# MCG-NKU/E2FGVI

Hardware: AMD Instinct MI355X
Metric: inpainted frames/sec at 432x240 T=10 (higher is better)
Workload: dtype f32; 1 GPU; BASELINE.json configs[1]: e2fgvi 432x240 T=10 l_t=10, 1 clip(s) per GPU per forward (1 in the job), random-init weights, torch.rand frames + box mask (SURVEY.md 8d); clips_per_gpu=1, precision=fp32, kernel_selection=e2fgvi_amd/tile_table.py (checked in, deterministic: ops.py), hip_graph=True, forwards_in_flight=2

## Files before the change

### e2fgvi_amd/build.py

```python
import os
import subprocess
import sys
from concurrent.futures import ThreadPoolExecutor

HERE = os.path.dirname(os.path.abspath(__file__))
CSRC = os.path.join(HERE, "csrc")
LIB = os.path.join(CSRC, "libe2fgvi_hip.so")
FLAGS = ["--offload-arch=gfx950", "-O3", "-std=c++17", "-fPIC", "-ffp-contract=fast"]
NOPK = ["-Xclang", "-target-feature", "-Xclang", "-packed-fp32-ops"]
UNITS = [("error.hip", "error.o", []), ("conv.hip", "conv.o", []), ("conv.hip", "conv_nopk.o", NOPK + ["-DE2_NOPK_VARIANT"]),
         ("conv_bf16x.hip", "conv_bf16x.o", NOPK), ("conv_wino.hip", "conv_wino.o", NOPK), ("conv_wino.hip", "conv_wino_x3.o", NOPK + ["-DE2_WINO_X3=1"]), ("conv_wino4.hip", "conv_wino4.o", NOPK), ("conv_tail.hip", "conv_tail.o", NOPK),
         ("mdcn.hip", "mdcn.o", NOPK), ("attention.hip", "attention.o", []),
         ("attention_bf16.hip", "attention_bf16.o", NOPK), ("attention_x3.hip", "attention_x3.o", NOPK), ("misc.hip", "misc.o", NOPK),
         ("video.hip", "video.o", NOPK), ("metrics.hip", "metrics.o", NOPK)]
NOPK_OBJECTS = ("conv_nopk.o", "conv_bf16x.o", "conv_wino.o", "conv_wino4.o", "conv_wino_x3.o", "conv_tail.o", "mdcn.o", "attention_bf16.o", "attention_x3.o", "misc.o", "video.o", "metrics.o")
OBJDUMP = "/opt/rocm/lib/llvm/bin/llvm-objdump"


def _hipcc():
    for c in (os.environ.get("HIPCC"), "/opt/rocm/bin/hipcc"):
        if c and os.path.exists(c):
            return c
    return "hipcc"


def _stale(out, deps):
    return (not os.path.exists(out)) or any(os.path.getmtime(d) > os.path.getmtime(out) for d in deps)


def build(force=False, verbose=False, nopk_all=False, lib=None, tag=None, defines=()):
    hipcc = _hipcc()
    if tag:
        nopk_all = False
    objdir = os.path.join(CSRC, ("build_" + tag) if tag else ("build_nopk" if nopk_all else "build"))
    os.makedirs(objdir, exist_ok=True)
    out = lib or (os.path.join(CSRC, "libe2fgvi_hip_%s.so" % tag) if tag else
                  os.path.join(CSRC, "libe2fgvi_hip_nopk.so") if nopk_all else LIB)
    headers = [os.path.join(CSRC, "common.h"), os.path.join(HERE, "..", "include", "e2fgvi_hip.h"), os.path.abspath(__file__)]
    jobs = []
    for src, obj, extra in UNITS:
        sp, op = os.path.join(CSRC, src), os.path.join(objdir, obj)
        if nopk_all and not any(f == "-packed-fp32-ops" for f in extra):
            extra = extra + NOPK
        if force or _stale(op, [sp] + headers):
            jobs.append([hipcc] + FLAGS + extra + list(defines) + ["-c", sp, "-o", op])

    def run(cmd):
        if verbose:
            print(" ".join(cmd), flush=True)
        subprocess.check_call(cmd)

    with ThreadPoolExecutor(max_workers=min(4, max(1, len(jobs)))) as ex:
        list(ex.map(run, jobs))
    objs = [os.path.join(objdir, obj) for _, obj, _ in UNITS]
    if force or jobs or _stale(out, objs):
        run([hipcc, "--offload-arch=gfx950", "-shared", "-fPIC", "-o", out] + objs)
    if jobs:
        verify_isa(objdir)
        if not nopk_all:
            verify_wino_waits(objdir)
            verify_exit_reuse(objdir)
            verify_no_scratch(objdir)
    return out


def build_variant(tag, *defines):
    return build(tag=tag, defines=defines)


def device_isa(obj):
    import shutil
    import tempfile
    d = tempfile.mkdtemp(prefix="e2isa")
    try:
        local = os.path.join(d, os.path.basename(obj))
        shutil.copy(obj, local)
        subprocess.run([OBJDUMP, "--offloading", os.path.basename(obj)], cwd=d, check=True, stdout=subprocess.DEVNULL,
                       stderr=subprocess.DEVNULL)
        dev = [f for f in os.listdir(d) if "gfx950" in f]
        if not dev:
            return ""
        return subprocess.run([OBJDUMP, "-d", os.path.join(d, dev[0])], check=True, capture_output=True, text=True).stdout
    finally:
        shutil.rmtree(d, ignore_errors=True)


def verify_isa(objdir=None):
    import re
    objdir = objdir or os.path.join(CSRC, "build")
    if not os.path.exists(OBJDUMP):
        return
    for obj in NOPK_OBJECTS:
        isa = device_isa(os.path.join(objdir, obj))
        bad = re.findall(r"v_pk_(?:mul|add|fma)_f32", isa)
        if bad or not isa:
            raise RuntimeError("%s: %s" % (obj, "%d packed-fp32 instructions in a unit that must have none" % len(bad) if isa
                                           else "no gfx950 code object found"))


def verify_no_scratch(objdir=None, obj="conv_bf16x.o", marker="ELb0ELi2ELb1EEE"):
    import re
    import shutil
    import tempfile
    objdir = objdir or os.path.join(CSRC, "build")
    readelf = os.path.join(os.path.dirname(OBJDUMP), "llvm-readelf")
    if not (os.path.exists(OBJDUMP) and os.path.exists(readelf)):
        return 0
    d = tempfile.mkdtemp(prefix="e2elf")
    try:
        shutil.copy(os.path.join(objdir, obj), os.path.join(d, obj))
        subprocess.run([OBJDUMP, "--offloading", obj], cwd=d, check=True, stdout=subprocess.DEVNULL, stderr=subprocess.DEVNULL)
        dev = [f for f in os.listdir(d) if "gfx950" in f]
        notes = subprocess.run([readelf, "--notes", os.path.join(d, dev[0])], check=True, capture_output=True, text=True).stdout if dev else ""
    finally:
        shutil.rmtree(d, ignore_errors=True)
    found = 0
    for block in notes.split("  - .agpr_count")[1:]:
        name = re.search(r"\.name:\s+(\S+)", block)
        if not name or marker not in name.group(1):
            continue
        found += 1
        priv = int(re.search(r"\.private_segment_fixed_size:\s+(\d+)", block).group(1))
        spill = int(re.search(r"\.vgpr_spill_count:\s+(\d+)", block).group(1))
        if priv or spill:
            raise RuntimeError("%s: %s: private segment %d bytes, %d spilled VGPRs in a ping-pong kernel" % (obj, name.group(1)[:70], priv, spill))
    if not found:
        raise RuntimeError("verify_no_scratch: no ping-pong instantiation found in %s (mangled-name marker changed?)" % obj)
    return found


def _kernels(isa):
    import re
    out, cur = {}, None
    for line in isa.splitlines():
        m = re.match(r"^[0-9a-f]+ <([^>]+)>:", line)
        if m:
            cur = out.setdefault(m.group(1), [])
            continue
        m = re.match(r"^\s+(\S+)\s*(.*?)\s*//\s*([0-9A-Fa-f]+):", line)
        if m and cur is not None:
            cur.append((int(m.group(3), 16), m.group(1), m.group(2)))
    return out


def check_kernel_waits(obj, name, ins):
# ... 223 lines not shown
```

### e2fgvi_amd/csrc/conv_bf16x.hip

```cpp
#include "common.h"

namespace {

typedef __bf16 bf16x8 __attribute__((ext_vector_type(8)));
typedef unsigned int u32x4 __attribute__((ext_vector_type(4)));
typedef __attribute__((address_space(3))) void lds_void;

struct ConvXParams {
    const void* src[E2FGVI_MAX_SRC];
    int ld[E2FGVI_MAX_SRC];
    int coff[E2FGVI_MAX_SRC];
    int cpg[E2FGVI_MAX_SRC];
    unsigned src_bytes[E2FGVI_MAX_SRC];
    int nsrc;
    int N, H, W, Ho, Wo, KH, KW, stride, pad;
    int padx;
    int osy, osx, opy, opx, oH, oW;
    int res_bcast;
    int Cout, Cout_g, Npad;
    int M;
    int tilesM, tilesN;
    int nsteps;
    unsigned wgroup_bytes;
    long long wgroup_elems;
    const void* w;
    const float* bias;
    const void* res;
    int res_ld, res_coff, res_bf16;
    void* dst;
    int dst_ld, dst_coff, dst_bf16, dst_nchw;
    __bf16* dst2;
    int dst2_ld, dst2_coff;
    int split_from;
    long long split_plane;
    int act;
    float slope;
    int tp_cq;
    unsigned tp_magic;
    unsigned tp_magic_cq;
    int dbg_noload;
};

__device__ __forceinline__ __amdgpu_buffer_rsrc_t make_rsrc(const void* base, unsigned bytes) {
    return __builtin_amdgcn_make_buffer_rsrc(const_cast<void*>(base), 0, (int)bytes, 0x00020000);
}

__device__ __forceinline__ float dcn_post(float v, int co, int C, const f32x4& fl, float max_residue) {
    const int noff = (C / 3) * 2;
    if (co >= noff) return e2_fast_sigmoid(v);
    const int which = (co * 2 >= noff) ? 2 : 0;
    return max_residue * e2_fast_tanh(v) + fl[which + ((co & 1) ? 0 : 1)];
}


__device__ __forceinline__ void split8(const f32x4& v0, const f32x4& v1, bf16x8& hi, bf16x8& mid, bf16x8& lo) {
    e2_split8(v0, v1, hi, mid, lo);
}

typedef int pp_i32x4 __attribute__((ext_vector_type(4)));
__device__ __forceinline__ pp_i32x4 pp_rsrc_words(const void* base, unsigned bytes) {
    const unsigned long long b = (unsigned long long)base;
    pp_i32x4 r;
    r[0] = __builtin_amdgcn_readfirstlane((int)(unsigned)b);
    r[1] = __builtin_amdgcn_readfirstlane((int)((unsigned)(b >> 32) & 0xFFFFu));
    r[2] = __builtin_amdgcn_readfirstlane((int)bytes);
    r[3] = 0x00020000;
    return r;
}
__device__ __forceinline__ void pp_dma16(pp_i32x4 rsrc, unsigned lds_dst, unsigned voff, unsigned soff) {
    unsigned keep;
    asm volatile("s_nop 4\n\ts_mov_b32 %0, m0\n\ts_mov_b32 m0, %3\n\ts_nop 0\n\tbuffer_load_dwordx4 %1, %2, %4 offen lds\n\ts_mov_b32 m0, %0"
                 : "=&s"(keep) : "v"(voff), "s"(rsrc), "s"(lds_dst), "s"(soff) : "memory");
}

template <int BM, int BN, int WGM, int WGN, bool S3, int MODE, bool PP = false>
__global__ __launch_bounds__(64 * WGM * WGN) void conv_bf16x_kernel(const ConvXParams p) {
#if defined(__HIP_DEVICE_COMPILE__)
    constexpr bool F32 = MODE == 1, X3 = MODE == 2, F16 = MODE == 3;
    typedef typename e2_h16<F16>::T E16;
    typedef typename e2_h16<F16>::V8 e16x8;
    static_assert(!PP || (X3 && !S3 && WGM * WGN == 8), "ping-pong halves: split-operand mode, 8 waves, no row-shift stages");
    constexpr int NT = 64 * WGM * WGN;
    constexpr int ESZ = (F32 || X3) ? 4 : 2;
    constexpr int CH = 16 / ESZ;
    constexpr int KC = 8 * CH;
    constexpr int TM = BM / (32 * WGM), TN = BN / (32 * WGN);
    constexpr int AR = S3 ? BM + 2 : BM;
    constexpr int B_CH = X3 ? 12 : 8;
    constexpr int A_BYTES = AR * 128, B_BYTES = BN * B_CH * 16;
    constexpr int A_IT = (AR * 8 + NT - 1) / NT, B_IT = (BN * B_CH + NT - 1) / NT;
    constexpr bool A_PART = (AR * 8) % NT != 0;
    constexpr bool B_PART = (BN * B_CH) % NT != 0;
    constexpr int R = TM * 32, CN = TN * 32;
    constexpr int ES = (WGM * WGN * R * (CN + 4) * 4 <= 150 * 1024) ? 1 : (TN % 2 == 0 ? 2 : TN);
    constexpr int TNH = TN / ES, CNH = CN / ES, LDE = CNH + 4;
    constexpr int EPI = WGM * WGN * R * LDE * 4;
    static_assert(TN % ES == 0 && EPI <= 160 * 1024, "epilogue region");
    constexpr int SMEM = 2 * (A_BYTES + B_BYTES) > EPI ? 2 * (A_BYTES + B_BYTES) : EPI;
    constexpr unsigned OOB = 0xFFFFFFFFu;
    static_assert(TM >= 1 && TN >= 1 && (BM * 8) % NT == 0 && (BN * B_CH) % 64 == 0 && SMEM <= 160 * 1024, "tile");

    __shared__ __attribute__((aligned(1024))) unsigned char smem[SMEM];

    const int tid = threadIdx.x;
    const int lane = tid & 63, wave = __builtin_amdgcn_readfirstlane(tid >> 6);
    const int wm = wave / WGN, wn = wave % WGN;
    const int g = blockIdx.y;
    const int logical = xcd_remap(blockIdx.x, p.tilesM * p.tilesN);
    const int tile_m = logical / p.tilesN, tile_n = logical - tile_m * p.tilesN;
    const int m0 = tile_m * BM, n0 = tile_n * BN;
    const int HoWo = p.Ho * p.Wo;

    int a_pix[A_IT];
    unsigned a_msk[A_IT];
    unsigned a_ch16[A_IT];
#pragma unroll
    for (int it = 0; it < A_IT; ++it) {
        const int item = tid + it * NT;
        const int row = item >> 3, slot = item & 7;
        a_ch16[it] = (unsigned)((slot ^ ((row >> 1) & 7)) * 16);
        const int m = S3 ? m0 + row - 1 : m0 + row;
        const bool ok = m >= 0 && m < p.M;
        const int mm = ok ? m : 0;
        const int img = mm / HoWo;
        const int rem = mm - img * HoWo;
        const int oy = rem / p.Wo, ox = rem - oy * p.Wo;
        const int by = oy * p.stride - p.pad;
        const int bx = S3 ? ox : ox * p.stride - p.padx;
        unsigned msk = 0;
        for (int k = 0; k < p.KH; ++k) msk |= ((unsigned)(by + k) < (unsigned)p.H ? 1u : 0u) << k;
        for (int k = 0; k < (S3 ? 1 : p.KW); ++k) msk |= ((unsigned)(bx + k) < (unsigned)p.W ? 1u : 0u) << (8 + k);
        a_msk[it] = ok ? msk : 0u;
        a_pix[it] = (img * p.H + by) * p.W + bx;
    }
    unsigned b_off[B_IT];
#pragma unroll
    for (int it = 0; it < B_IT; ++it) {
        const int item = tid + it * NT;
        const int koct = item / BN, n = item - koct * BN;
        b_off[it] = ((n0 + n) < p.Npad && koct < B_CH) ? (unsigned)((koct * p.Npad + n0 + n) * 16) : OOB;
    }
    const __amdgpu_buffer_rsrc_t wrsrc = make_rsrc(reinterpret_cast<const char*>(p.w) + (long long)g * p.wgroup_bytes, p.wgroup_bytes);
    const unsigned b_step = (unsigned)B_CH * (unsigned)p.Npad * 16u;

    const void* const sp0 = p.src[0]; const void* const sp1 = p.src[1]; const void* const sp2 = p.src[2]; const void* const sp3 = p.src[3];
    const unsigned sb0 = p.src_bytes[0], sb1 = p.src_bytes[1], sb2 = p.src_bytes[2], sb3 = p.src_bytes[3];
    const unsigned sl0 = (unsigned)p.ld[0] * ESZ, sl1 = (unsigned)p.ld[1] * ESZ, sl2 = (unsigned)p.ld[2] * ESZ, sl3 = (unsigned)p.ld[3] * ESZ;
    const unsigned sc0 = (unsigned)(p.coff[0] + g * p.cpg[0]) * ESZ, sc1 = (unsigned)(p.coff[1] + g * p.cpg[1]) * ESZ,
                   sc2 = (unsigned)(p.coff[2] + g * p.cpg[2]) * ESZ, sc3 = (unsigned)(p.coff[3] + g * p.cpg[3]) * ESZ;
    const int sg0 = p.cpg[0], sg1 = p.cpg[1], sg2 = p.cpg[2], sg3 = p.cpg[3];
    int ky = 0, kx = 0, s = 0, c0 = 0;
    int blk = 0;
    const void* cur_src = sp0;
    unsigned cur_bytes = sb0;
    unsigned cur_ld2 = sl0, cur_chan = sc0;
    int cur_cpg = sg0;
    unsigned a_off[A_IT];
    auto retarget = [&]() {
        if (p.nsrc > 1) {
            cur_src = s == 0 ? sp0 : s == 1 ? sp1 : s == 2 ? sp2 : sp3;
            cur_bytes = s == 0 ? sb0 : s == 1 ? sb1 : s == 2 ? sb2 : sb3;
            cur_ld2 = s == 0 ? sl0 : s == 1 ? sl1 : s == 2 ? sl2 : sl3;
            cur_chan = s == 0 ? sc0 : s == 1 ? sc1 : s == 2 ? sc2 : sc3;
            cur_cpg = s == 0 ? sg0 : s == 1 ? sg1 : s == 2 ? sg2 : sg3;
        }
        const int kxe = S3 ? 0 : kx;
        const int tap = ky * p.W + kxe;
#pragma unroll
        for (int it = 0; it < A_IT; ++it) {
            const bool ok = ((a_msk[it] >> ky) & (a_msk[it] >> (8 + kxe)) & 1u) != 0;
            a_off[it] = ok ? (unsigned)(a_pix[it] + tap) * cur_ld2 + cur_chan + a_ch16[it] : OOB;
        }
    };
    retarget();
    unsigned char* const smem_b = smem + 2 * A_BYTES;
    auto issue_a = [&](int stage) {
        if (p.dbg_noload & 16) return;
        unsigned char* sa = smem + stage * A_BYTES + wave * 1024;
        const __amdgpu_buffer_rsrc_t arsrc = make_rsrc(cur_src, cur_bytes);
        const unsigned soff = (unsigned)c0 * (unsigned)ESZ;
        if (c0 + KC <= cur_cpg) {
#pragma unroll
            for (int it = 0; it < A_IT; ++it)
                if (!A_PART || it + 1 < A_IT || tid + it * NT < AR * 8)
                    __builtin_amdgcn_raw_ptr_buffer_load_lds(arsrc, (lds_void*)(sa + it * NT * 16), 16, a_off[it], soff, 0, 0);
        } else {
#pragma unroll
            for (int it = 0; it < A_IT; ++it)
                if (!A_PART || it + 1 < A_IT || tid + it * NT < AR * 8)
                    __builtin_amdgcn_raw_ptr_buffer_load_lds(arsrc, (lds_void*)(sa + it * NT * 16), 16,
                                                             (c0 + (int)(a_ch16[it] / ESZ) < cur_cpg) ? a_off[it] : OOB, soff, 0, 0);
        }
    };
    auto issue_b = [&](int stage, int step) {
        if (p.dbg_noload & 32) return;
        unsigned char* sb = smem_b + stage * B_BYTES + wave * 1024;
        const unsigned soff = (unsigned)step * b_step;
#pragma unroll
        for (int it = 0; it < B_IT; ++it)
            if (!B_PART || it + 1 < B_IT || tid + it * NT < BN * B_CH)
                __builtin_amdgcn_raw_ptr_buffer_load_lds(wrsrc, (lds_void*)(sb + it * NT * 16), 16, b_off[it], soff, 0, 0);
    };
    auto advance = [&]() -> bool {
        c0 += KC;
        ++blk;
        if (c0 < cur_cpg) return false;
        c0 = 0;
        ++s;
        if (s == p.nsrc) {
            s = 0;
            blk = 0;
            if (S3) ++ky;
            else { ++kx; if (kx == p.KW) { kx = 0; ++ky; } }
        }
        return true;
    };

    f32x16 acc[TM][TN];
#pragma unroll
    for (int tm = 0; tm < TM; ++tm)
#pragma unroll
        for (int tn = 0; tn < TN; ++tn)
#pragma unroll
            for (int r = 0; r < 16; ++r) acc[tm][tn][r] = 0.f;

    const int i = lane & 31, h = lane >> 5;
    int a_row[TM], b_rd[TN];
    bool okl[TM], okr[TM];
#pragma unroll
    for (int tm = 0; tm < TM; ++tm) {
        a_row[tm] = (wm * TM + tm) * 32 + i;
        const int ox = (m0 + a_row[tm]) % p.Wo;
        okl[tm] = ox != 0;
        okr[tm] = ox != p.Wo - 1;
    }
#pragma unroll
    for (int tn = 0; tn < TN; ++tn) b_rd[tn] = ((wn * TN + tn) * 32 + i) * 16;

    auto compute = [&](const unsigned char* st, const unsigned char* stb, int kxs) {
        int a_rd[TM], a_key[TM];
        bool zero[TM];
#pragma unroll
        for (int tm = 0; tm < TM; ++tm) {
            const int row = a_row[tm] + (S3 ? kxs : 0);
            a_rd[tm] = row * 128;
            a_key[tm] = (row >> 1) & 7;
            zero[tm] = S3 && ((kxs == 0 && !okl[tm]) || (kxs == 2 && !okr[tm]));
        }
        if constexpr (X3) {
#pragma unroll
            for (int kk = 0; kk < 2; ++kk) {
                const int q = 2 * kk + h;
                bf16x8 ah[TM], am[TM], al[TM];
#pragma unroll
                for (int tm = 0; tm < TM; ++tm)
                    split8(*reinterpret_cast<const f32x4*>(st + a_rd[tm] + (((2 * q) ^ a_key[tm]) << 4)),
                           *reinterpret_cast<const f32x4*>(st + a_rd[tm] + (((2 * q + 1) ^ a_key[tm]) << 4)), ah[tm], am[tm], al[tm]);
#pragma unroll
                for (int tn = 0; tn < TN; ++tn) {
                    const bf16x8 bh = *reinterpret_cast<const bf16x8*>(stb + b_rd[tn] + q * (BN * 16));
                    const bf16x8 bm = *reinterpret_cast<const bf16x8*>(stb + b_rd[tn] + (4 + q) * (BN * 16));
                    const bf16x8 bl = *reinterpret_cast<const bf16x8*>(stb + b_rd[tn] + (8 + q) * (BN * 16));
#pragma unroll
                    for (int tm = 0; tm < TM; ++tm) acc[tm][tn] = __builtin_amdgcn_mfma_f32_32x32x16_bf16(al[tm], bh, acc[tm][tn], 0, 0, 0);
#pragma unroll
                    for (int tm = 0; tm < TM; ++tm) acc[tm][tn] = __builtin_amdgcn_mfma_f32_32x32x16_bf16(ah[tm], bl, acc[tm][tn], 0, 0, 0);
#pragma unroll
                    for (int tm = 0; tm < TM; ++tm) acc[tm][tn] = __builtin_amdgcn_mfma_f32_32x32x16_bf16(am[tm], bm, acc[tm][tn], 0, 0, 0);
#pragma unroll
                    for (int tm = 0; tm < TM; ++tm) acc[tm][tn] = __builtin_amdgcn_mfma_f32_32x32x16_bf16(am[tm], bh, acc[tm][tn], 0, 0, 0);
#pragma unroll
                    for (int tm = 0; tm < TM; ++tm) acc[tm][tn] = __builtin_amdgcn_mfma_f32_32x32x16_bf16(ah[tm], bm, acc[tm][tn], 0, 0, 0);
#pragma unroll
                    for (int tm = 0; tm < TM; ++tm) acc[tm][tn] = __builtin_amdgcn_mfma_f32_32x32x16_bf16(ah[tm], bh, acc[tm][tn], 0, 0, 0);
                }
            }
        } else {
#pragma unroll
        for (int kk = 0; kk < 4; ++kk) {
            if constexpr (F32) {
                f32x4 a[TM], b[TN];
#pragma unroll
                for (int tm = 0; tm < TM; ++tm)
                    a[tm] = *reinterpret_cast<const f32x4*>(st + a_rd[tm] + (((2 * kk + h) ^ a_key[tm]) << 4));
#pragma unroll
                for (int tn = 0; tn < TN; ++tn)
                    b[tn] = *reinterpret_cast<const f32x4*>(stb + b_rd[tn] + (2 * kk + h) * (BN * 16));
#pragma unroll
                for (int e = 0; e < 4; ++e)
#pragma unroll
                    for (int tm = 0; tm < TM; ++tm)
#pragma unroll
                        for (int tn = 0; tn < TN; ++tn)
                            acc[tm][tn] = __builtin_amdgcn_mfma_f32_32x32x2f32(a[tm][e], b[tn][e], acc[tm][tn], 0, 0, 0);
            } else {
                e16x8 a[TM], b[TN];
#pragma unroll
                for (int tm = 0; tm < TM; ++tm) {
                    a[tm] = *reinterpret_cast<const e16x8*>(st + a_rd[tm] + (((2 * kk + h) ^ a_key[tm]) << 4));
                    if (S3) {
                        u32x4 q = __builtin_bit_cast(u32x4, a[tm]);
#pragma unroll
                        for (int e = 0; e < 4; ++e) q[e] = zero[tm] ? 0u : q[e];
                        a[tm] = __builtin_bit_cast(e16x8, q);
                    }
                }
#pragma unroll
                for (int tn = 0; tn < TN; ++tn)
                    b[tn] = *reinterpret_cast<const e16x8*>(stb + b_rd[tn] + (2 * kk + h) * (BN * 16));
#pragma unroll
                for (int tm = 0; tm < TM; ++tm)
#pragma unroll
                    for (int tn = 0; tn < TN; ++tn)
                        acc[tm][tn] = e2_mfma16(a[tm], b[tn], acc[tm][tn]);
            }
        }
        }
    };
    const bool tap_packed = !S3 && p.tp_cq != 0;
    if (!tap_packed) issue_a(0);
    issue_b(0, 0);
    if (!tap_packed) {
        asm volatile("s_waitcnt vmcnt(0)" ::: "memory");
        __syncthreads();
    }
    if constexpr (PP) {
        const bool trail = wave >= 4;
        bf16x8 fa[TM][3];
        auto pp_bar = [&]() __attribute__((always_inline)) {
            __builtin_amdgcn_sched_barrier(0);
            asm volatile("s_waitcnt lgkmcnt(0)\n\ts_barrier" ::: "memory");
            __builtin_amdgcn_sched_barrier(0);
        };
        auto prep = [&](const unsigned char* st, const int kk) __attribute__((always_inline)) {
            const int q = 2 * kk + h;
#pragma unroll
            for (int tm = 0; tm < TM; ++tm) {
                const int row = a_row[tm];
                const int rd = row * 128, key = (row >> 1) & 7;
                split8(*reinterpret_cast<const f32x4*>(st + rd + (((2 * q) ^ key) << 4)),
                       *reinterpret_cast<const f32x4*>(st + rd + (((2 * q + 1) ^ key) << 4)), fa[tm][0], fa[tm][1], fa[tm][2]);
            }
        };
        auto mma = [&](const unsigned char* stb, const int kk) __attribute__((always_inline)) {
            const int q = 2 * kk + h;
            bf16x8 bq[2][3];
            auto rd = [&](int tn, bf16x8 (&b)[3]) __attribute__((always_inline)) {
                b[0] = *reinterpret_cast<const bf16x8*>(stb + b_rd[tn] + q * (BN * 16));
                b[1] = *reinterpret_cast<const bf16x8*>(stb + b_rd[tn] + (4 + q) * (BN * 16));
                b[2] = *reinterpret_cast<const bf16x8*>(stb + b_rd[tn] + (8 + q) * (BN * 16));
            };
            rd(0, bq[0]);
#pragma unroll
            for (int tn = 0; tn < TN; ++tn) {
                if (tn + 1 < TN) rd(tn + 1, bq[(tn + 1) & 1]);
                __builtin_amdgcn_sched_barrier(0);
                const bf16x8 bh = bq[tn & 1][0], bm = bq[tn & 1][1], bl = bq[tn & 1][2];
#pragma unroll
                for (int tm = 0; tm < TM; ++tm) acc[tm][tn] = __builtin_amdgcn_mfma_f32_32x32x16_bf16(fa[tm][2], bh, acc[tm][tn], 0, 0, 0);
#pragma unroll
                for (int tm = 0; tm < TM; ++tm) acc[tm][tn] = __builtin_amdgcn_mfma_f32_32x32x16_bf16(fa[tm][0], bl, acc[tm][tn], 0, 0, 0);
#pragma unroll
                for (int tm = 0; tm < TM; ++tm) acc[tm][tn] = __builtin_amdgcn_mfma_f32_32x32x16_bf16(fa[tm][1], bm, acc[tm][tn], 0, 0, 0);
#pragma unroll
                for (int tm = 0; tm < TM; ++tm) acc[tm][tn] = __builtin_amdgcn_mfma_f32_32x32x16_bf16(fa[tm][1], bh, acc[tm][tn], 0, 0, 0);
#pragma unroll
                for (int tm = 0; tm < TM; ++tm) acc[tm][tn] = __builtin_amdgcn_mfma_f32_32x32x16_bf16(fa[tm][0], bm, acc[tm][tn], 0, 0, 0);
#pragma unroll
                for (int tm = 0; tm < TM; ++tm) acc[tm][tn] = __builtin_amdgcn_mfma_f32_32x32x16_bf16(fa[tm][0], bh, acc[tm][tn], 0, 0, 0);
                __builtin_amdgcn_sched_barrier(0);
            }
        };
        const unsigned smem_lds = (unsigned)(unsigned long long)(lds_void*)smem;
        const pp_i32x4 wrsrc_w = pp_rsrc_words(reinterpret_cast<const char*>(p.w) + (long long)g * p.wgroup_bytes, p.wgroup_bytes);
        auto pp_issue = [&](int stage, int step) __attribute__((always_inline)) {
            const pp_i32x4 arsrc_w = pp_rsrc_words(cur_src, cur_bytes);
            const unsigned soff = (unsigned)__builtin_amdgcn_readfirstlane(c0 * ESZ);
            const unsigned la = smem_lds + (unsigned)(stage * A_BYTES + wave * 1024);
            const bool whole = c0 + KC <= cur_cpg;
#pragma unroll
            for (int it = 0; it < A_IT; ++it)
                pp_dma16(arsrc_w, (unsigned)__builtin_amdgcn_readfirstlane((int)(la + it * NT * 16)),
                         (whole || c0 + (int)(a_ch16[it] / ESZ) < cur_cpg) ? a_off[it] : OOB, soff);
            const unsigned lb = smem_lds + (unsigned)(2 * A_BYTES + stage * B_BYTES + wave * 1024);
            const unsigned sb = (unsigned)__builtin_amdgcn_readfirstlane((int)((unsigned)step * b_step));
#pragma unroll
            for (int it = 0; it < B_IT; ++it)
                if (!B_PART || it + 1 < B_IT || tid + it * NT < BN * B_CH)
                    pp_dma16(wrsrc_w, (unsigned)__builtin_amdgcn_readfirstlane((int)(lb + it * NT * 16)), b_off[it], sb);
        };
        if (trail) pp_bar();
        for (int step = 0; step < p.nsteps; ++step) {
            const int cur = step & 1;
            const unsigned char* const sA = smem + cur * A_BYTES;
            const unsigned char* const sB = smem_b + cur * B_BYTES;
            if (trail) { if (step + 1 < p.nsteps) { if (advance()) retarget(); pp_issue((step & 1) ^ 1, step + 1); } }
            prep(sA, 0);
            pp_bar();
            mma(sB, 0);
            pp_bar();
            prep(sA, 1);
            if (!trail) { if (step + 1 < p.nsteps) { if (advance()) retarget(); pp_issue((step & 1) ^ 1, step + 1); } }
            if (trail) asm volatile("s_waitcnt vmcnt(0)" ::: "memory");
            pp_bar();
            mma(sB, 1);
            if (!trail) asm volatile("s_waitcnt vmcnt(0)" ::: "memory");
            pp_bar();
        }
        if (!trail) pp_bar();
    } else
    if constexpr (!S3) {
        if (p.tp_cq) {
            const int cq = p.tp_cq, KK = p.KH * p.KW;
            int t_c[A_IT];
#pragma unroll
            for (int it = 0; it < A_IT; ++it) t_c[it] = (int)(a_ch16[it] >> 4);
            const __amdgpu_buffer_rsrc_t arsrc = make_rsrc(sp0, sb0);
            auto issue_a_packed = [&](int stage, int step) {
                unsigned char* sa = smem + stage * A_BYTES + wave * 1024;
#pragma unroll
                for (int it = 0; it < A_IT; ++it) {
                    const int L = 8 * step + t_c[it];
                    const int tap = cq == 1 ? L : (int)__umulhi((unsigned)L, p.tp_magic_cq);
                    const int cc = L - tap * cq;
                    const int tky = (int)__umulhi((unsigned)tap, p.tp_magic), tkx = tap - tky * p.KW;
                    const bool ok = tap < KK && ((a_msk[it] >> tky) & (a_msk[it] >> (8 + tkx)) & 1u) != 0;
                    const unsigned off = ok ? (unsigned)(a_pix[it] + tky * p.W + tkx) * sl0 + sc0 + (unsigned)cc * 16u : OOB;
                    __builtin_amdgcn_raw_ptr_buffer_load_lds(arsrc, (lds_void*)(sa + it * NT * 16), 16, off, 0, 0, 0);
                }
            };
            issue_a_packed(0, 0);
            asm volatile("s_waitcnt vmcnt(0)" ::: "memory");
            __syncthreads();
            for (int step = 0; step < p.nsteps; ++step) {
                const int cur = step & 1;
                if (step + 1 < p.nsteps) {
                    issue_a_packed(cur ^ 1, step + 1);
                    issue_b(cur ^ 1, step + 1);
                }
                compute(smem + cur * A_BYTES, smem_b + cur * B_BYTES, 0);
                asm volatile("s_waitcnt vmcnt(0)" ::: "memory");
                __syncthreads();
            }
        } else
        for (int step = 0; step < p.nsteps; ++step) {
            const int cur = step & 1;
            const bool more = step + 1 < p.nsteps && !(p.dbg_noload & 1);
            if (more) {
                if (advance()) retarget();
                issue_a(cur ^ 1);
                issue_b(cur ^ 1, step + 1);
            }
            compute(smem + cur * A_BYTES, smem_b + cur * B_BYTES, 0);
            asm volatile("s_waitcnt vmcnt(0)" ::: "memory");
            __syncthreads();
        }
    } else if constexpr (!S3) {
        for (int step = 0; step < p.nsteps; ++step) {
            const int cur = step & 1;
            const bool more = step + 1 < p.nsteps && !(p.dbg_noload & 1);
            if (more) {
                if (advance()) retarget();
                issue_a(cur ^ 1);
                issue_b(cur ^ 1, step + 1);
            }
            compute(smem + cur * A_BYTES, smem_b + cur * B_BYTES, 0);
            asm volatile("s_waitcnt vmcnt(0)" ::: "memory");
            __syncthreads();
        }
    } else {
        const int spt = p.nsteps / 9;
        int acur = 0, kxs = 0;
        for (int step = 0; step < p.nsteps; ++step) {
            const bool more = step + 1 < p.nsteps && !(p.dbg_noload & 1);
            int kxn = kxs + 1;
            bool newblk = false;
            if (kxn == 3) {
                kxn = 0;
                if (more) { if (advance()) retarget(); newblk = true; }
            }
            if (more) {
                if (newblk) issue_a(acur ^ 1);
                issue_b((step + 1) & 1, (ky * 3 + kxn) * spt + blk);
            }
            compute(smem + acur * A_BYTES, smem_b + (step & 1) * B_BYTES, kxs);
            asm volatile("s_waitcnt vmcnt(0)" ::: "memory");
            __syncthreads();
            if (kxn == 0) acur ^= 1;
            kxs = kxn;
        }
    }

    if (p.dbg_noload & 2) {
        float sacc = 0.f;
#pragma unroll
        for (int tm = 0; tm < TM; ++tm)
#pragma unroll
            for (int tn = 0; tn < TN; ++tn)
#pragma unroll
                for (int r = 0; r < 16; ++r) sacc += acc[tm][tn][r];
        if (sacc == 123.456f) reinterpret_cast<float*>(p.dst)[0] = sacc;
        return;
    }
    auto out_row = [&](long long m, long long& mr) -> long long {
        long long mo = m;
        mr = m;
        if (p.osy | p.res_bcast) {
            const int img = (int)(m / HoWo);
            const int rem = (int)(m - (long long)img * HoWo);
            if (p.osy) {
                const int oy = rem / p.Wo, ox = rem - oy * p.Wo;
// ... 204 lines not shown
    long long total, wgroup_elems;
};

bool geometry_x(int Cout, int groups, int KH, int KW, int nsrc, const int32_t* cpg, PackX* q, bool f32 = false) {
    q->kc = f32 ? 32 : 64;
    q->ch = f32 ? 4 : 8;
    q->tp_cq = 0;
    if (Cout <= 0 || groups <= 0 || Cout % groups || KH <= 0 || KW <= 0 || nsrc < 1 || nsrc > E2FGVI_MAX_SRC) return false;
    q->Cout = Cout; q->groups = groups; q->KH = KH; q->KW = KW; q->nsrc = nsrc;
    q->Cout_g = Cout / groups;
    q->Npad = round_up(q->Cout_g, 32);
    q->Cin_g = 0;
    q->steps_per_tap = 0;
    for (int s = 0; s < E2FGVI_MAX_SRC; ++s) q->cpg[s] = 0;
    for (int s = 0; s < nsrc; ++s) {
        if (cpg[s] <= 0 || cpg[s] % q->ch) return false;
        q->cpg[s] = cpg[s];
        q->Cin_g += cpg[s];
        q->steps_per_tap += cdiv(cpg[s], q->kc);
    }
    q->wgroup_elems = (long long)KH * KW * q->steps_per_tap * q->kc * q->Npad;
    q->total = q->wgroup_elems * groups;
    return true;
}

__device__ __forceinline__ float pack_value(const float* __restrict__ w, const PackX& p, int g, int step, int koct, int n, int e) {
    if (p.tp_cq) {
        const int L = 8 * step + koct;
        const int tapk = L / p.tp_cq;
        const int chk = (L - tapk * p.tp_cq) * p.ch + e;
        if (tapk < p.KH * p.KW && chk < p.cpg[0] && n < p.Cout_g)
            return w[((long long)n * p.Cin_g + chk) * (p.KH * p.KW) + tapk];
        return 0.f;
    }
    const int tap = step / p.steps_per_tap;
    int blk = step - tap * p.steps_per_tap;
    int s = 0, prefix = 0;
    while (blk >= (p.cpg[s] + p.kc - 1) / p.kc) { blk -= (p.cpg[s] + p.kc - 1) / p.kc; prefix += p.cpg[s]; ++s; }
    const int c = blk * p.kc + koct * p.ch + e;
    if (c < p.cpg[s] && n < p.Cout_g)
        return w[((long long)(g * p.Cout_g + n) * p.Cin_g + prefix + c) * (p.KH * p.KW) + tap];
    return 0.f;
}

template <typename T>
__global__ void pack_conv_weight_x_kernel(const float* __restrict__ w, T* __restrict__ wp, const PackX p) {
    const long long idx = (long long)blockIdx.x * blockDim.x + threadIdx.x;
    if (idx >= p.total) return;
    const int g = (int)(idx / p.wgroup_elems);
    long long rem = idx - (long long)g * p.wgroup_elems;
    const int e = (int)(rem % p.ch);
    rem /= p.ch;
    const int n = (int)(rem % p.Npad);
    rem /= p.Npad;
    const int koct = (int)(rem & 7);
    const int step = (int)(rem >> 3);
    wp[idx] = (T)pack_value(w, p, g, step, koct, n, e);
}

__global__ void pack_conv_weight_x3_kernel(const float* __restrict__ w, unsigned short* __restrict__ wp, const PackX p) {
    const long long idx = (long long)blockIdx.x * blockDim.x + threadIdx.x;
    if (idx >= p.total) return;
    const int g = (int)(idx / p.wgroup_elems);
    long long rem = idx - (long long)g * p.wgroup_elems;
    const int e = (int)(rem & 3);
    rem >>= 2;
    const int n = (int)(rem % p.Npad);
    rem /= p.Npad;
    const int koct = (int)(rem & 7);
    const int step = (int)(rem >> 3);
    const float v = pack_value(w, p, g, step, koct, n, e);
    const unsigned xb = __builtin_bit_cast(unsigned, v);
    const float r = v - __builtin_bit_cast(float, xb & 0xFFFF0000u);
    const unsigned rb = __builtin_bit_cast(unsigned, r);
    const float r2 = r - __builtin_bit_cast(float, rb & 0xFFFF0000u);
    const long long plane = 4LL * p.Npad * 8;
    unsigned short* o = wp + (long long)g * p.wgroup_elems * 3 + (long long)step * 3 * plane +
                        ((long long)(koct >> 1) * p.Npad + n) * 8 + (koct & 1) * 4 + e;
    o[0] = (unsigned short)(xb >> 16);
    o[plane] = (unsigned short)(rb >> 16);
    o[2 * plane] = (unsigned short)(__builtin_bit_cast(unsigned, r2) >> 16);
}

template <int BM, int BN, int WGM, int WGN, bool S3, bool PP = false>
int launch_x(ConvXParams& p, int groups, hipStream_t st, int mode = 0) {
    p.tilesM = cdiv(p.M, BM);
    p.tilesN = cdiv(p.Cout_g, BN);
    if constexpr (PP) {
        if (mode != 2 || p.tp_cq) {
            e2fgvi_set_error("conv2d_x: the ping-pong tiles (107, 108) are for the split-operand mode without tap-packed weights");
            return E2FGVI_EUNSUP;
        }
        hipLaunchKernelGGL((conv_bf16x_kernel<BM, BN, WGM, WGN, false, 2, true>), dim3(p.tilesM * p.tilesN, groups, 1), dim3(64 * WGM * WGN), 0, st, p);
        E2_LAUNCH_CHECK("conv2d_x");
        return 0;
    } else {
    if (S3 && !(p.KH == 3 && p.KW == 3 && p.stride == 1 && p.pad == 1)) {
        e2fgvi_set_error("conv2d_bf16x: the row-shift tiles (11..17) are for 3x3 stride-1 pad-1 layers");
        return E2FGVI_EINVAL;
    }
    if (mode == 1 || mode == 2) {
        if constexpr (!S3) {
            if (mode == 2)
                hipLaunchKernelGGL((conv_bf16x_kernel<BM, BN, WGM, WGN, false, 2>), dim3(p.tilesM * p.tilesN, groups, 1), dim3(64 * WGM * WGN), 0, st, p);
            else
                hipLaunchKernelGGL((conv_bf16x_kernel<BM, BN, WGM, WGN, false, 1>), dim3(p.tilesM * p.tilesN, groups, 1), dim3(64 * WGM * WGN), 0, st, p);
        } else {
            e2fgvi_set_error("conv2d_f32x: the row-shift tiles (11..18) take bf16 operands only");
            return E2FGVI_EUNSUP;
        }
    } else if (mode == 3) {
        hipLaunchKernelGGL((conv_bf16x_kernel<BM, BN, WGM, WGN, S3, 3>), dim3(p.tilesM * p.tilesN, groups, 1), dim3(64 * WGM * WGN), 0, st, p);
    } else {
        hipLaunchKernelGGL((conv_bf16x_kernel<BM, BN, WGM, WGN, S3, 0>), dim3(p.tilesM * p.tilesN, groups, 1), dim3(64 * WGM * WGN), 0, st, p);
    }
    E2_LAUNCH_CHECK("conv2d_x");
    return 0;
    }
}

}

extern "C" int64_t e2fgvi_packed_conv_weight_bf16x_size(int32_t Cout, int32_t groups, int32_t KH, int32_t KW, int32_t nsrc,
                                                        const int32_t* src_cpg) {
    PackX q;
    if (!src_cpg || !geometry_x(Cout, groups, KH, KW, nsrc, src_cpg, &q)) {
        e2fgvi_set_error("packed_conv_weight_bf16x_size: bad geometry (channels per source must be multiples of 8)");
        return E2FGVI_EINVAL;
    }
    return q.total;
}

extern "C" int e2fgvi_pack_conv_weight_bf16x(const float* w, void* wpacked, int32_t Cout, int32_t groups, int32_t KH,
                                             int32_t KW, int32_t nsrc, const int32_t* src_cpg, void* stream) {
    PackX q;
    E2_REQUIRE(w && wpacked && src_cpg, E2FGVI_EINVAL, "pack_conv_weight_bf16x: null pointer");
    E2_REQUIRE(geometry_x(Cout, groups, KH, KW, nsrc, src_cpg, &q), E2FGVI_EINVAL, "pack_conv_weight_bf16x: bad geometry");
    hipLaunchKernelGGL(pack_conv_weight_x_kernel<__bf16>, dim3((unsigned)cdiv64(q.total, 256)), dim3(256), 0, (hipStream_t)stream,
                       w, (__bf16*)wpacked, q);
    E2_LAUNCH_CHECK("pack_conv_weight_bf16x");
    return 0;
}

extern "C" int64_t e2fgvi_packed_conv_weight_f16x_size(int32_t Cout, int32_t groups, int32_t KH, int32_t KW, int32_t nsrc,
                                                       const int32_t* src_cpg) {
    return e2fgvi_packed_conv_weight_bf16x_size(Cout, groups, KH, KW, nsrc, src_cpg);
}
extern "C" int e2fgvi_pack_conv_weight_f16x(const float* w, void* wpacked, int32_t Cout, int32_t groups, int32_t KH,
                                            int32_t KW, int32_t nsrc, const int32_t* src_cpg, void* stream) {
    PackX q;
    E2_REQUIRE(w && wpacked && src_cpg, E2FGVI_EINVAL, "pack_conv_weight_f16x: null pointer");
    E2_REQUIRE(geometry_x(Cout, groups, KH, KW, nsrc, src_cpg, &q), E2FGVI_EINVAL, "pack_conv_weight_f16x: bad geometry");
    hipLaunchKernelGGL(pack_conv_weight_x_kernel<_Float16>, dim3((unsigned)cdiv64(q.total, 256)), dim3(256), 0, (hipStream_t)stream,
                       w, (_Float16*)wpacked, q);
    E2_LAUNCH_CHECK("pack_conv_weight_f16x");
    return 0;
}

extern "C" int64_t e2fgvi_packed_conv_weight_f32x_size(int32_t Cout, int32_t groups, int32_t KH, int32_t KW, int32_t nsrc,
                                                       const int32_t* src_cpg) {
    PackX q;
    if (!src_cpg || !geometry_x(Cout, groups, KH, KW, nsrc, src_cpg, &q, true)) {
        e2fgvi_set_error("packed_conv_weight_f32x_size: bad geometry (channels per source must be multiples of 4)");
        return E2FGVI_EINVAL;
    }
    return q.total;
}

extern "C" int e2fgvi_pack_conv_weight_f32x(const float* w, float* wpacked, int32_t Cout, int32_t groups, int32_t KH,
                                            int32_t KW, int32_t nsrc, const int32_t* src_cpg, void* stream) {
// ... 64 lines not shown
                                                 void* stream) {
    PackX q;
    E2_REQUIRE(w && wpacked, E2FGVI_EINVAL, "pack_conv_weight_f16x_taps: null pointer");
    E2_REQUIRE(geometry_taps(Cout, KH, KW, cin, &q), E2FGVI_EINVAL, "pack_conv_weight_f16x_taps: bad geometry");
    hipLaunchKernelGGL(pack_conv_weight_x_kernel<_Float16>, dim3((unsigned)cdiv64(q.total, 256)), dim3(256), 0, (hipStream_t)stream,
                       w, (_Float16*)wpacked, q);
    E2_LAUNCH_CHECK("pack_conv_weight_f16x_taps");
    return 0;
}

extern "C" int64_t e2fgvi_packed_conv_weight_f32x_taps_size(int32_t Cout, int32_t KH, int32_t KW, int32_t cin) {
    PackX q;
    if (!geometry_taps(Cout, KH, KW, cin, &q, true)) {
        e2fgvi_set_error("packed_conv_weight_f32x_taps_size: one source of 4 ... 56 channels (multiple of 4), KW >= 2");
        return E2FGVI_EINVAL;
    }
    return q.total;
}

extern "C" int e2fgvi_pack_conv_weight_f32x_taps(const float* w, float* wpacked, int32_t Cout, int32_t KH, int32_t KW, int32_t cin,
                                                 void* stream) {
    PackX q;
    E2_REQUIRE(w && wpacked, E2FGVI_EINVAL, "pack_conv_weight_f32x_taps: null pointer");
    E2_REQUIRE(geometry_taps(Cout, KH, KW, cin, &q, true), E2FGVI_EINVAL, "pack_conv_weight_f32x_taps: bad geometry");
    hipLaunchKernelGGL(pack_conv_weight_x_kernel<float>, dim3((unsigned)cdiv64(q.total, 256)), dim3(256), 0, (hipStream_t)stream,
                       w, wpacked, q);
    E2_LAUNCH_CHECK("pack_conv_weight_f32x_taps");
    return 0;
}

extern "C" int64_t e2fgvi_packed_conv_weight_f32x3_taps_size(int32_t Cout, int32_t KH, int32_t KW, int32_t cin) {
    PackX q;
    if (!geometry_taps(Cout, KH, KW, cin, &q, true)) {
        e2fgvi_set_error("packed_conv_weight_f32x3_taps_size: one source of 4 ... 56 channels (multiple of 4), KW >= 2");
        return E2FGVI_EINVAL;
    }
    return 3 * q.total;
}

extern "C" int e2fgvi_pack_conv_weight_f32x3_taps(const float* w, void* wpacked, int32_t Cout, int32_t KH, int32_t KW, int32_t cin,
                                                  void* stream) {
    PackX q;
    E2_REQUIRE(w && wpacked, E2FGVI_EINVAL, "pack_conv_weight_f32x3_taps: null pointer");
    E2_REQUIRE(geometry_taps(Cout, KH, KW, cin, &q, true), E2FGVI_EINVAL, "pack_conv_weight_f32x3_taps: bad geometry");
    hipLaunchKernelGGL(pack_conv_weight_x3_kernel, dim3((unsigned)cdiv64(q.total, 256)), dim3(256), 0, (hipStream_t)stream,
                       w, (unsigned short*)wpacked, q);
    E2_LAUNCH_CHECK("pack_conv_weight_f32x3_taps");
    return 0;
}

static int conv2d_x(const e2fgvi_convx_desc* d, void* stream, int mode) {
    const bool f32 = mode == 1 || mode == 2;
    const int dt16 = mode == 3 ? E2FGVI_F16 : E2FGVI_BF16;
    E2_REQUIRE(d, E2FGVI_EINVAL, "conv2d_bf16x: null descriptor");
    PackX q;
    const int esz = f32 ? 4 : 2;
    const int wbytes_num = mode == 2 ? 6 : esz;
    E2_REQUIRE(geometry_x(d->Cout, d->groups, d->KH, d->KW, d->nsrc, d->src_cpg, &q, f32), E2FGVI_EINVAL,
               "conv2d_bf16x: bad geometry (channels per source must be multiples of 8 bf16 / 4 fp32)");
    E2_REQUIRE(d->N > 0 && d->H > 0 && d->W > 0 && d->Ho > 0 && d->Wo > 0 && d->stride > 0 && d->pad >= 0, E2FGVI_EINVAL,
               "conv2d_bf16x: bad sizes");
    if (d->out_grid) {
        E2_REQUIRE(d->pad_left >= 0 && d->act != E2FGVI_ACT_DCNPOST && !d->dst_nchw && !d->tap_packed && (d->tile < 10 || d->tile > 20),
                   E2FGVI_EINVAL, "conv2d_bf16x: explicit output grids take plain NHWC tiles only");
        if (d->out_sy || d->out_sx)
            E2_REQUIRE(d->out_sy > 0 && d->out_sx > 0 && d->out_py >= 0 && d->out_px >= 0 && d->out_H > 0 && d->out_W > 0 &&
                       (d->Ho - 1) * d->out_sy + d->out_py < d->out_H && (d->Wo - 1) * d->out_sx + d->out_px < d->out_W &&
                       (long long)d->N * d->out_H * d->out_W < 2147483647LL,
                       E2FGVI_EINVAL, "conv2d_bf16x: the output scatter leaves the [N, out_H, out_W] image");
    } else {
        E2_REQUIRE(d->Ho == (d->H + 2 * d->pad - d->KH) / d->stride + 1 && d->Wo == (d->W + 2 * d->pad - d->KW) / d->stride + 1,
                   E2FGVI_EINVAL, "conv2d_bf16x: Ho/Wo inconsistent with H/W/k/stride/pad");
        E2_REQUIRE(!d->out_sy && !d->out_sx && !d->pad_left, E2FGVI_EINVAL, "conv2d_bf16x: pad_left / out_s* need out_grid = 1");
    }
    E2_REQUIRE(!d->res_bcast || (d->residual && d->act != E2FGVI_ACT_DCNPOST), E2FGVI_EINVAL, "conv2d_bf16x: res_bcast without a residual");
    E2_REQUIRE((long long)d->N * d->Ho * d->Wo < 2147483647LL, E2FGVI_EUNSUP, "conv2d_bf16x: more than 2^31 output pixels");
    E2_REQUIRE(d->KH <= 8 && d->KW <= 8, E2FGVI_EUNSUP, "conv2d_bf16x: kernels larger than 8x8 are not supported");
    E2_REQUIRE(d->wpacked && d->dst, E2FGVI_EINVAL, "conv2d_bf16x: null weight/dst");
    E2_REQUIRE((d->dst_dtype == E2FGVI_F32 || d->dst_dtype == dt16) && (d->res_dtype == E2FGVI_F32 || d->res_dtype == dt16),
               E2FGVI_EINVAL, mode == 3 ? "conv2d_f16x: dtype must be E2FGVI_F32 or E2FGVI_F16"
                                        : "conv2d_bf16x: dtype must be E2FGVI_F32 or E2FGVI_BF16");
    ConvXParams p;
    for (int s = 0; s < E2FGVI_MAX_SRC; ++s) { p.src[s] = nullptr; p.ld[s] = 0; p.coff[s] = 0; p.cpg[s] = 0; p.src_bytes[s] = 0; }
    for (int s = 0; s < d->nsrc; ++s) {
        E2_REQUIRE(d->src[s], E2FGVI_EINVAL, "conv2d_bf16x: null source %d", s);
        E2_REQUIRE(d->src_ld[s] % q.ch == 0 && d->src_coff[s] % q.ch == 0 && ((uintptr_t)d->src[s] & 15) == 0, E2FGVI_EINVAL,
                   "conv2d_bf16x: source %d not 16-byte addressable (ld / coff multiples of 8 bf16 / 4 fp32)", s);
        E2_REQUIRE(d->src_coff[s] + d->groups * d->src_cpg[s] <= d->src_ld[s], E2FGVI_EINVAL,
                   "conv2d_bf16x: source %d channel range exceeds its pixel stride", s);
        const long long bytes = (long long)d->N * d->H * d->W * d->src_ld[s] * esz;
        E2_REQUIRE(bytes < 4294967295LL, E2FGVI_EUNSUP, "conv2d_bf16x: source %d spans >= 4 GiB (split the batch)", s);
        p.src[s] = d->src[s]; p.ld[s] = d->src_ld[s]; p.coff[s] = d->src_coff[s]; p.cpg[s] = d->src_cpg[s];
        p.src_bytes[s] = (unsigned)bytes;
    }
    E2_REQUIRE(q.wgroup_elems * wbytes_num < 4294967295LL, E2FGVI_EUNSUP, "conv2d_bf16x: packed weight group >= 4 GiB");
    E2_REQUIRE(((uintptr_t)d->wpacked & 15) == 0, E2FGVI_EINVAL, "conv2d_bf16x: packed weight not 16-byte aligned");
    if (d->dst_nchw)
        E2_REQUIRE(d->dst_dtype == E2FGVI_F32 && !d->dst2, E2FGVI_EINVAL, "conv2d_bf16x: the NCHW destination is fp32, without a second copy");
    else
        E2_REQUIRE(d->dst_coff >= 0 && d->dst_coff + d->Cout <= d->dst_ld, E2FGVI_EINVAL, "conv2d_bf16x: dst slice exceeds dst_ld");
    E2_REQUIRE(((uintptr_t)d->dst & 15) == 0 && (!d->dst2 || ((uintptr_t)d->dst2 & 15) == 0) &&
               (!d->residual || ((uintptr_t)d->residual & 15) == 0), E2FGVI_EINVAL, "conv2d_bf16x: dst / dst2 / residual not 16-byte aligned");
    E2_REQUIRE(mode != 3 || !d->dst2_plane_stride, E2FGVI_EINVAL, "conv2d_f16x: no split planes (dst2 is an fp16 copy)");
    if (d->dst2_plane_stride) {
        E2_REQUIRE(d->dst2 && d->dst2_plane_stride > 0 && d->dst_dtype == E2FGVI_F32 && !d->dst_nchw && d->groups == 1 &&
                       !(d->out_grid && d->out_sy), E2FGVI_EINVAL,
                   "conv2d_bf16x: split planes need dst2, an fp32 NHWC dst, groups = 1 and no output scatter");
        E2_REQUIRE(d->Cout % 8 == 0 && d->dst2_split_from >= 0 && d->dst2_split_from <= d->Cout && d->dst2_split_from % 8 == 0 &&
                       d->dst2_ld % 8 == 0 && d->dst2_coff % 8 == 0 && d->dst2_plane_stride % 8 == 0 && d->dst2_coff >= 0 &&
                       d->dst2_coff + d->Cout - d->dst2_split_from <= d->dst2_ld, E2FGVI_EINVAL,
                   "conv2d_bf16x: split planes: Cout, dst2_split_from, dst2_ld, dst2_coff and dst2_plane_stride in multiples of 8, "
                   "the split channels inside dst2_ld");
    } else if (d->dst2)
        E2_REQUIRE(d->dst2_coff >= 0 && d->dst2_coff + d->Cout <= d->dst2_ld, E2FGVI_EINVAL, "conv2d_bf16x: dst2 slice exceeds dst2_ld");
    if (d->act == E2FGVI_ACT_DCNPOST)
        E2_REQUIRE(d->residual && d->res_dtype == E2FGVI_F32 && d->Cout % 3 == 0 && d->groups == 1, E2FGVI_EINVAL,
                   "conv2d_bf16x: ACT_DCNPOST needs the fp32 [pixel][4] flows as residual, Cout %% 3 == 0, groups == 1");
    p.nsrc = d->nsrc;
    p.N = d->N; p.H = d->H; p.W = d->W; p.Ho = d->Ho; p.Wo = d->Wo;
    p.KH = d->KH; p.KW = d->KW; p.stride = d->stride; p.pad = d->pad;
    p.padx = d->out_grid ? d->pad_left : d->pad;
    p.osy = d->out_grid ? d->out_sy : 0; p.osx = d->out_sx; p.opy = d->out_py; p.opx = d->out_px; p.oH = d->out_H; p.oW = d->out_W;
    p.res_bcast = d->res_bcast;
    p.Cout = d->Cout; p.Cout_g = q.Cout_g; p.Npad = q.Npad;
    p.M = d->N * d->Ho * d->Wo;
    p.nsteps = d->KH * d->KW * q.steps_per_tap;
    p.tp_cq = 0; p.tp_magic = 0; p.tp_magic_cq = 0;
    if (d->tap_packed) {
        PackX qt;
        E2_REQUIRE(d->nsrc == 1 && d->groups == 1 && geometry_taps(d->Cout, d->KH, d->KW, d->src_cpg[0], &qt, f32), E2FGVI_EINVAL,
                   "conv2d_bf16x: tap-packed weights are for one source of <= 56 channels, no groups, KW >= 2");
        E2_REQUIRE(d->tile < 10 || d->tile > 20, E2FGVI_EUNSUP, "conv2d_bf16x: the row-shift tiles do not take tap-packed weights");
        q.wgroup_elems = qt.wgroup_elems;
        p.tp_cq = qt.tp_cq;
        p.tp_magic = 0xFFFFFFFFu / (unsigned)d->KW + 1u;
        p.tp_magic_cq = qt.tp_cq > 1 ? 0xFFFFFFFFu / (unsigned)qt.tp_cq + 1u : 0u;
        p.nsteps = cdiv(d->KH * d->KW * qt.tp_cq, 8);
    }
    p.wgroup_elems = q.wgroup_elems; p.wgroup_bytes = (unsigned)(q.wgroup_elems * wbytes_num);
    p.w = d->wpacked; p.bias = d->bias;
    p.res = d->residual; p.res_ld = d->res_ld; p.res_coff = d->res_coff; p.res_bf16 = d->res_dtype == dt16;
    p.dst = d->dst; p.dst_ld = d->dst_ld; p.dst_coff = d->dst_coff; p.dst_bf16 = d->dst_dtype == dt16;
    p.dst_nchw = d->dst_nchw;
    p.dst2 = (__bf16*)d->dst2; p.dst2_ld = d->dst2_ld; p.dst2_coff = d->dst2_coff;
    p.split_from = d->dst2_split_from; p.split_plane = d->dst2_plane_stride;
    p.act = d->act; p.slope = d->slope;
    hipStream_t st = (hipStream_t)stream;
    int tile = d->tile;
    p.dbg_noload = 0;
    if (tile == 21 || tile == 24 || tile == 26 || tile == 27) { p.dbg_noload = 1; tile -= 20; }
    if (tile == 31 || tile == 34 || tile == 36) { p.dbg_noload = 2; tile -= 30; }
    if (tile == 41 || tile == 44 || tile == 46) { p.dbg_noload = 3; tile -= 40; }
    if (tile == 61 || tile == 66) { p.dbg_noload = 8; tile -= 60; }
    if (tile == 71 || tile == 74 || tile == 76 || tile == 77) { p.dbg_noload = 16; tile -= 70; }
    if (tile == 81 || tile == 84 || tile == 86 || tile == 87) { p.dbg_noload = 32; tile -= 80; }
    if (!tile) {
        if (p.Cout_g <= 32) tile = 3;
        else if (p.Cout_g <= 64) tile = 2;
        else tile = ((long long)cdiv(p.M, 128) * cdiv(p.Cout_g, 128) * d->groups >= 384) ? 1 : 4;
    }
    switch (tile) {
        case 1: return launch_x<128, 128, 2, 2, false>(p, d->groups, st, mode);
        case 2: return launch_x<128, 64, 2, 2, false>(p, d->groups, st, mode);
        case 3: return launch_x<128, 32, 4, 1, false>(p, d->groups, st, mode);
        case 4: return launch_x<64, 128, 2, 2, false>(p, d->groups, st, mode);
        case 5: return launch_x<64, 64, 2, 2, false>(p, d->groups, st, mode);
        case 6: return launch_x<256, 128, 4, 2, false>(p, d->groups, st, mode);
        case 7: return launch_x<256, 256, 4, 2, false>(p, d->groups, st, mode);
        case 8: return launch_x<256, 192, 4, 2, false>(p, d->groups, st, mode);
        case 107: return launch_x<256, 256, 4, 2, false, true>(p, d->groups, st, mode);
        case 108: return launch_x<256, 192, 4, 2, false, true>(p, d->groups, st, mode);
        case 11: return launch_x<128, 128, 2, 2, true>(p, d->groups, st, mode);
        case 12: return launch_x<128, 64, 2, 2, true>(p, d->groups, st, mode);
        case 13: return launch_x<128, 32, 4, 1, true>(p, d->groups, st, mode);
        case 14: return launch_x<64, 128, 2, 2, true>(p, d->groups, st, mode);
        case 16: return launch_x<256, 128, 4, 2, true>(p, d->groups, st, mode);
        case 17: return launch_x<256, 256, 4, 2, true>(p, d->groups, st, mode);
        case 18: return launch_x<256, 64, 4, 2, true>(p, d->groups, st, mode);
        default: break;
    }
    e2fgvi_set_error("conv2d_bf16x: unknown tile %d", tile);
    return E2FGVI_EINVAL;
}

extern "C" int e2fgvi_conv2d_bf16x(const e2fgvi_convx_desc* d, void* stream) { return conv2d_x(d, stream, 0); }
extern "C" int e2fgvi_conv2d_f32x(const e2fgvi_convx_desc* d, void* stream) { return conv2d_x(d, stream, 1); }
extern "C" int e2fgvi_conv2d_f32x3(const e2fgvi_convx_desc* d, void* stream) { return conv2d_x(d, stream, 2); }
extern "C" int e2fgvi_conv2d_f16x(const e2fgvi_convx_desc* d, void* stream) { return conv2d_x(d, stream, 3); }
```

### e2fgvi_amd/csrc/misc.hip

```cpp
#include "common.h"

#include <type_traits>

namespace {

constexpr int NTH = 256;

typedef unsigned int u32x2 __attribute__((ext_vector_type(2)));
typedef __bf16 bf16x4 __attribute__((ext_vector_type(4)));
typedef _Float16 f16x4 __attribute__((ext_vector_type(4)));
typedef _Float16 f16x8 __attribute__((ext_vector_type(8)));
template <typename T> __device__ __forceinline__ f32x4 ld4(const T* p);
template <> __device__ __forceinline__ f32x4 ld4<float>(const float* p) { return *reinterpret_cast<const f32x4*>(p); }
template <> __device__ __forceinline__ f32x4 ld4<__bf16>(const __bf16* p) {
    const u32x2 q = *reinterpret_cast<const u32x2*>(p);
    f32x4 v = {__builtin_bit_cast(float, q[0] << 16), __builtin_bit_cast(float, q[0] & 0xFFFF0000u),
               __builtin_bit_cast(float, q[1] << 16), __builtin_bit_cast(float, q[1] & 0xFFFF0000u)};
    return v;
}
template <> __device__ __forceinline__ f32x4 ld4<_Float16>(const _Float16* p) {
    const f16x4 h = *reinterpret_cast<const f16x4*>(p);
    f32x4 v = {(float)h[0], (float)h[1], (float)h[2], (float)h[3]};
    return v;
}
// ... 342 lines not shown
    stv(co + C + c4 * NV, c2);
    if (c4 == 0) {
        f32x4 fo = {f1.x, f1.y, fl2.x, fl2.y};
        *reinterpret_cast<f32x4*>(flows + pix * 4) = fo;
        if (flows8) {
            const f32x4 z4 = {0.f, 0.f, 0.f, 0.f};
            st4(flows8 + pix * 8, fo);
            st4(flows8 + pix * 8 + 4, z4);
        }
    }
}

template <int VPL, typename TO>
__global__ void layernorm_kernel(const float* __restrict__ x, const float* __restrict__ gamma,
                                 const float* __restrict__ beta, TO* __restrict__ y, long long rows, int C) {
    const long long row = (long long)blockIdx.x * (blockDim.x >> 6) + (threadIdx.x >> 6);
    if (row >= rows) return;
    const int lane = threadIdx.x & 63;
    const float* xr = x + row * C;
    f32x4 v[VPL];
    float s = 0.f;
#pragma unroll
    for (int i = 0; i < VPL; ++i) {
        v[i] = *reinterpret_cast<const f32x4*>(xr + (i * 64 + lane) * 4);
        s += v[i][0] + v[i][1] + v[i][2] + v[i][3];
    }
#pragma unroll
    for (int o = 32; o > 0; o >>= 1) s += __shfl_xor(s, o);
    const float mean = s / (float)C;
    float q = 0.f;
#pragma unroll
    for (int i = 0; i < VPL; ++i) {
        v[i] = v[i] - mean;
        q += v[i][0] * v[i][0] + v[i][1] * v[i][1] + v[i][2] * v[i][2] + v[i][3] * v[i][3];
    }
#pragma unroll
    for (int o = 32; o > 0; o >>= 1) q += __shfl_xor(q, o);
    const float rstd = 1.f / sqrtf(q / (float)C + 1e-5f);
    TO* yr = y + row * C;
#pragma unroll
    for (int i = 0; i < VPL; ++i) {
        const f32x4 g = *reinterpret_cast<const f32x4*>(gamma + (i * 64 + lane) * 4);
        const f32x4 bb = *reinterpret_cast<const f32x4*>(beta + (i * 64 + lane) * 4);
        st4(yr + (i * 64 + lane) * 4, v[i] * rstd * g + bb);
    }
}

template <typename T>
__global__ void window_pool_kernel(const T* __restrict__ x, const float* __restrict__ w45,
                                   const float* __restrict__ bias1, T* __restrict__ pooled, int BT, int fh, int fw,
                                   int C) {
    constexpr int NV = VT<T>::N, Q = VT<T>::Q;
    const int cq = C / NV;
    const int nWw = fw / 9, nWh = fh / 5;
    const long long idx = (long long)blockIdx.x * blockDim.x + threadIdx.x;
    if (idx >= (long long)BT * nWh * nWw * cq) return;
    FlatIdx fi(idx, (long long)BT * nWh * nWw * cq);
    const int c4 = fi.pop(cq);
    const int wx = fi.pop(nWw);
    const int wy = fi.pop(nWh);
    const long long bt = fi.rest();
    const float b = bias1[0];
    f32x4 acc[Q];
#pragma unroll
    for (int q = 0; q < Q; ++q) acc[q] = f32x4{b, b, b, b};
    for (int py = 0; py < 5; ++py)
        for (int px = 0; px < 9; ++px) {
            f32x4 v[Q];
            ldv(x + ((bt * fh + wy * 5 + py) * fw + wx * 9 + px) * C + c4 * NV, v);
#pragma unroll
            for (int q = 0; q < Q; ++q) acc[q] = acc[q] + v[q] * w45[py * 9 + px];
        }
    stv(pooled + idx * NV, acc);
}

__device__ __forceinline__ void fold_range(int Y, int L, int& l_lo, int& l_hi) {
    const int lo = Y - 3;
    l_lo = lo <= 0 ? 0 : (lo + 2) / 3;
    l_hi = min((Y + 3) / 3, L - 1);
}

__device__ __forceinline__ float gelu_exact(float x) { return 0.5f * x * (1.f + erff(x * 0.70710678118654752f)); }

template <bool NORMALISE, typename TE, typename TR, typename TD, bool GELU_OUT = false>
__global__ void fold_kernel(const TE* __restrict__ emb, const float* __restrict__ bias_hwc,
                            const TR* __restrict__ residual, TD* __restrict__ dst, int F, int fh, int fw, int H,
                            int W, int C) {
    static_assert(VT<TE>::N == VT<TD>::N && VT<TR>::N == VT<TD>::N, "fold: one element class per instantiation");
    constexpr int NV = VT<TD>::N, Q = VT<TD>::Q;
    const int cq = C / NV;
    const long long idx = (long long)blockIdx.x * blockDim.x + threadIdx.x;
    if (idx >= (long long)F * H * W * cq) return;
    FlatIdx fi(idx, (long long)F * H * W * cq);
    const int c4 = fi.pop(cq);
    const int X = fi.pop(W);
    const int Y = fi.pop(H);
    const long long f = fi.rest();
    int ly0, ly1, lx0, lx1;
    fold_range(Y, fh, ly0, ly1);
    fold_range(X, fw, lx0, lx1);
    f32x4 acc[Q];
#pragma unroll
    for (int q = 0; q < Q; ++q) acc[q] = f32x4{0.f, 0.f, 0.f, 0.f};
    const int row_len = 49 * C;
    for (int ly = ly0; ly <= ly1; ++ly) {
        const int ki = Y + 3 - 3 * ly;
        for (int lx = lx0; lx <= lx1; ++lx) {
            const int kj = X + 3 - 3 * lx;
            f32x4 v[Q];
            ldv(emb + ((f * fh + ly) * fw + lx) * row_len + (ki * 7 + kj) * C + c4 * NV, v);
#pragma unroll
            for (int q = 0; q < Q; ++q) acc[q] = acc[q] + v[q];
        }
    }
    if (NORMALISE) {
        const float cnt = (float)((ly1 - ly0 + 1) * (lx1 - lx0 + 1));
#pragma unroll
        for (int q = 0; q < Q; ++q) acc[q] = acc[q] / cnt;
    }
    if (GELU_OUT) {
#pragma unroll
        for (int q = 0; q < Q; ++q)
#pragma unroll
            for (int e = 0; e < 4; ++e) acc[q][e] = gelu_exact(acc[q][e]);
    }
    const long long o = ((f * H + Y) * W + X) * C + c4 * NV;
    if (bias_hwc) {
        f32x4 bq[Q];
        ldf<Q>(bias_hwc + ((long long)Y * W + X) * C + c4 * NV, bq);
#pragma unroll
        for (int q = 0; q < Q; ++q) acc[q] = acc[q] + bq[q];
    }
    if (residual) {
        f32x4 rq[Q];
        ldv(residual + o, rq);
#pragma unroll
        for (int q = 0; q < Q; ++q) acc[q] = acc[q] + rq[q];
    }
    stv(dst + o, acc);
}

template <typename T, bool GELU = true>
__global__ void unfold_gelu_kernel(const T* __restrict__ folded, T* __restrict__ out, int F, int fh, int fw,
                                   int H, int W, int C) {
    constexpr int NV = VT<T>::N, Q = VT<T>::Q;
    const int cq = C / NV;
    const long long idx = (long long)blockIdx.x * blockDim.x + threadIdx.x;
    if (idx >= (long long)F * fh * fw * 49 * cq) return;
    FlatIdx fi(idx, (long long)F * fh * fw * 49 * cq);
    const int c4 = fi.pop(cq);
    const int tap = fi.pop(49);
    const int lx = fi.pop(fw);
    const int ly = fi.pop(fh);
    const long long f = fi.rest();
    const int Y = 3 * ly - 3 + tap / 7, X = 3 * lx - 3 + tap % 7;
    f32x4 v[Q];
#pragma unroll
    for (int q = 0; q < Q; ++q) v[q] = f32x4{0.f, 0.f, 0.f, 0.f};
    if (Y >= 0 && Y < H && X >= 0 && X < W) {
        ldv(folded + ((f * H + Y) * W + X) * C + c4 * NV, v);
        if (GELU) {
#pragma unroll
            for (int q = 0; q < Q; ++q)
#pragma unroll
                for (int e = 0; e < 4; ++e) v[q][e] = gelu_exact(v[q][e]);
        }
    }
    stv(out + idx * NV, v);
}

template <typename TI, typename TO>
__global__ void cast_kernel(const TI* __restrict__ src, TO* __restrict__ dst, long long n4) {
    const long long idx = (long long)blockIdx.x * blockDim.x + threadIdx.x;
    if (idx < n4) st4(dst + idx * 4, ld4(src + idx * 4));
}

inline unsigned blocks_for(long long total) { return (unsigned)cdiv64(total, NTH); }

template <typename Fn> void with_dtype(int dt, Fn&& f) {
    if (dt == E2FGVI_BF16) f((__bf16*)nullptr);
    else if (dt == E2FGVI_F16) f((_Float16*)nullptr);
    else f((float*)nullptr);
}
#define E2_ELEM(z) std::remove_pointer_t<decltype(z)>

}

#define E2_DT_OK(dt) ((dt) == E2FGVI_F32 || (dt) == E2FGVI_BF16 || (dt) == E2FGVI_F16)
#define E2_DT16(dt) ((dt) == E2FGVI_BF16 || (dt) == E2FGVI_F16)

extern "C" int e2fgvi_nchw_to_nhwc_x(const float* src, void* dst, int32_t dst_dtype, int32_t N, int32_t C, int32_t H, int32_t W,
                                     int32_t ld, float scale, float shift, void* stream) {
    E2_REQUIRE(src && dst && N > 0 && C > 0 && H > 0 && W > 0 && ld >= C && E2_DT_OK(dst_dtype), E2FGVI_EINVAL,
               "nchw_to_nhwc: bad arguments");
    if (ld == 8 && C <= 8 && ((uintptr_t)dst & 15) == 0) {
        const long long total = (long long)N * H * W;
        with_dtype(dst_dtype, [&](auto z) {
            hipLaunchKernelGGL(nchw_small_to_nhwc8_kernel<E2_ELEM(z)>, dim3(blocks_for(total)), dim3(NTH), 0, (hipStream_t)stream, src,
                               (E2_ELEM(z)*)dst, C, H * W, scale, shift, total);
        });
        E2_LAUNCH_CHECK("nchw_to_nhwc8");
        return 0;
    }
    if (ld == 4 && C <= 4 && ((uintptr_t)dst & 15) == 0) {
        const long long total = (long long)N * H * W;
        with_dtype(dst_dtype, [&](auto z) {
            hipLaunchKernelGGL(nchw_small_to_nhwc4_kernel<E2_ELEM(z)>, dim3(blocks_for(total)), dim3(NTH), 0, (hipStream_t)stream, src,
                               (E2_ELEM(z)*)dst, C, H * W, scale, shift, total);
        });
        E2_LAUNCH_CHECK("nchw_to_nhwc4");
        return 0;
    }
    dim3 grid(cdiv(H * W, 32), cdiv(ld, 32), N), block(32, 8);
    with_dtype(dst_dtype, [&](auto z) {
        hipLaunchKernelGGL(nchw_to_nhwc_kernel<E2_ELEM(z)>, grid, block, 0, (hipStream_t)stream, src, (E2_ELEM(z)*)dst, C, H * W, ld,
                           scale, shift);
    });
    E2_LAUNCH_CHECK("nchw_to_nhwc");
    return 0;
}
extern "C" int e2fgvi_nchw_to_nhwc(const float* src, float* dst, int32_t N, int32_t C, int32_t H, int32_t W, int32_t ld,
// ... 188 lines not shown
                                void* stream) {
    return e2fgvi_layernorm_x(x, gamma, beta, y, E2FGVI_F32, rows, C, stream);
}

extern "C" int e2fgvi_window_pool_x(const void* x, int32_t dtype, const float* w45, const float* bias1, void* pooled,
                                    int32_t BT, int32_t fh, int32_t fw, int32_t C, void* stream) {
    E2_REQUIRE(x && w45 && bias1 && pooled && BT > 0 && fh > 0 && fw > 0 && fh % 5 == 0 && fw % 9 == 0 && C % 4 == 0 &&
                   E2_DT_OK(dtype),
               E2FGVI_EINVAL, "window_pool: bad arguments");
    E2_REQUIRE(dtype == E2FGVI_F32 || C % 8 == 0, E2FGVI_EINVAL, "window_pool: 16-bit needs C %% 8 == 0");
    const long long total = (long long)BT * (fh / 5) * (fw / 9) * (C / (E2_DT16(dtype) ? 8 : 4));
    with_dtype(dtype, [&](auto z) {
        using T = E2_ELEM(z);
        hipLaunchKernelGGL(window_pool_kernel<T>, dim3(blocks_for(total)), dim3(NTH), 0, (hipStream_t)stream,
                           (const T*)x, w45, bias1, (T*)pooled, BT, fh, fw, C);
    });
    E2_LAUNCH_CHECK("window_pool");
    return 0;
}
extern "C" int e2fgvi_window_pool(const float* x, const float* w45, const float* bias1, float* pooled, int32_t BT,
                                  int32_t fh, int32_t fw, int32_t C, void* stream) {
    return e2fgvi_window_pool_x(x, E2FGVI_F32, w45, bias1, pooled, BT, fh, fw, C, stream);
}

static int check_fold(const char* name, int F, int fh, int fw, int H, int W, int C) {
    E2_REQUIRE(F > 0 && C > 0 && C % 4 == 0, E2FGVI_EINVAL, "%s: bad arguments", name);
    E2_REQUIRE(fh == (H + 6 - 7) / 3 + 1 && fw == (W + 6 - 7) / 3 + 1, E2FGVI_EINVAL,
               "%s: token grid %dx%d inconsistent with %dx%d", name, fh, fw, H, W);
    return 0;
}

extern "C" int e2fgvi_ffn_fold_x(const void* hid, void* folded, int32_t dtype, int32_t F, int32_t fh, int32_t fw, int32_t H,
                                 int32_t W, int32_t C, void* stream) {
    E2_REQUIRE(hid && folded && E2_DT_OK(dtype), E2FGVI_EINVAL, "ffn_fold: bad arguments");
    if (int rc = check_fold("ffn_fold", F, fh, fw, H, W, C)) return rc;
    E2_REQUIRE(dtype == E2FGVI_F32 || C % 8 == 0, E2FGVI_EINVAL, "ffn_fold: 16-bit needs C %% 8 == 0");
    const long long total = (long long)F * H * W * (C / (E2_DT16(dtype) ? 8 : 4));
    with_dtype(dtype, [&](auto z) {
        using T = E2_ELEM(z);
        hipLaunchKernelGGL((fold_kernel<true, T, T, T>), dim3(blocks_for(total)), dim3(NTH), 0, (hipStream_t)stream,
                           (const T*)hid, (const float*)nullptr, (const T*)nullptr, (T*)folded, F, fh, fw, H, W, C);
    });
    E2_LAUNCH_CHECK("ffn_fold");
    return 0;
}
extern "C" int e2fgvi_ffn_fold(const float* hid, float* folded, int32_t F, int32_t fh, int32_t fw, int32_t H, int32_t W,
                               int32_t C, void* stream) {
    return e2fgvi_ffn_fold_x(hid, folded, E2FGVI_F32, F, fh, fw, H, W, C, stream);
}

extern "C" int e2fgvi_ffn_unfold_gelu_x(const void* folded, void* out, int32_t dtype, int32_t F, int32_t fh, int32_t fw,
                                        int32_t H, int32_t W, int32_t C, void* stream) {
    E2_REQUIRE(folded && out && E2_DT_OK(dtype), E2FGVI_EINVAL, "ffn_unfold_gelu: bad arguments");
    if (int rc = check_fold("ffn_unfold_gelu", F, fh, fw, H, W, C)) return rc;
    E2_REQUIRE(dtype == E2FGVI_F32 || C % 8 == 0, E2FGVI_EINVAL, "ffn_unfold_gelu: 16-bit needs C %% 8 == 0");
    const long long total = (long long)F * fh * fw * 49 * (C / (E2_DT16(dtype) ? 8 : 4));
    with_dtype(dtype, [&](auto z) {
        using T = E2_ELEM(z);
        hipLaunchKernelGGL(unfold_gelu_kernel<T>, dim3(blocks_for(total)), dim3(NTH), 0, (hipStream_t)stream,
                           (const T*)folded, (T*)out, F, fh, fw, H, W, C);
    });
    E2_LAUNCH_CHECK("ffn_unfold_gelu");
    return 0;
}
extern "C" int e2fgvi_ffn_unfold_gelu(const float* folded, float* out, int32_t F, int32_t fh, int32_t fw, int32_t H,
                                      int32_t W, int32_t C, void* stream) {
    return e2fgvi_ffn_unfold_gelu_x(folded, out, E2FGVI_F32, F, fh, fw, H, W, C, stream);
}

extern "C" int e2fgvi_ffn_fold_gelu_x(const void* hid, void* folded, int32_t dtype, int32_t F, int32_t fh, int32_t fw, int32_t H,
                                      int32_t W, int32_t C, void* stream) {
    E2_REQUIRE(hid && folded && E2_DT_OK(dtype), E2FGVI_EINVAL, "ffn_fold_gelu: bad arguments");
    if (int rc = check_fold("ffn_fold_gelu", F, fh, fw, H, W, C)) return rc;
    E2_REQUIRE(dtype == E2FGVI_F32 || C % 8 == 0, E2FGVI_EINVAL, "ffn_fold_gelu: 16-bit needs C %% 8 == 0");
    const long long total = (long long)F * H * W * (C / (E2_DT16(dtype) ? 8 : 4));
    with_dtype(dtype, [&](auto z) {
        using T = E2_ELEM(z);
        hipLaunchKernelGGL((fold_kernel<true, T, T, T, true>), dim3(blocks_for(total)), dim3(NTH), 0, (hipStream_t)stream,
                           (const T*)hid, (const float*)nullptr, (const T*)nullptr, (T*)folded, F, fh, fw, H, W, C);
    });
    E2_LAUNCH_CHECK("ffn_fold_gelu");
    return 0;
}
extern "C" int e2fgvi_ffn_unfold_x(const void* folded, void* out, int32_t dtype, int32_t F, int32_t fh, int32_t fw, int32_t H,
                                   int32_t W, int32_t C, void* stream) {
    E2_REQUIRE(folded && out && E2_DT_OK(dtype), E2FGVI_EINVAL, "ffn_unfold: bad arguments");
    if (int rc = check_fold("ffn_unfold", F, fh, fw, H, W, C)) return rc;
    E2_REQUIRE(dtype == E2FGVI_F32 || C % 8 == 0, E2FGVI_EINVAL, "ffn_unfold: 16-bit needs C %% 8 == 0");
    const long long total = (long long)F * fh * fw * 49 * (C / (E2_DT16(dtype) ? 8 : 4));
    with_dtype(dtype, [&](auto z) {
        using T = E2_ELEM(z);
        hipLaunchKernelGGL((unfold_gelu_kernel<T, false>), dim3(blocks_for(total)), dim3(NTH), 0, (hipStream_t)stream,
                           (const T*)folded, (T*)out, F, fh, fw, H, W, C);
    });
    E2_LAUNCH_CHECK("ffn_unfold");
    return 0;
}

extern "C" int e2fgvi_softcomp_fold(const float* emb, const float* bias_hwc, const float* residual, float* dst, int32_t F,
                                    int32_t fh, int32_t fw, int32_t H, int32_t W, int32_t C, void* stream) {
    E2_REQUIRE(emb && dst, E2FGVI_EINVAL, "softcomp_fold: null pointer");
    if (int rc = check_fold("softcomp_fold", F, fh, fw, H, W, C)) return rc;
    const long long total = (long long)F * H * W * (C / 4);
    hipLaunchKernelGGL((fold_kernel<false, float, float, float>), dim3(blocks_for(total)), dim3(NTH), 0, (hipStream_t)stream, emb,
                       bias_hwc, residual, dst, F, fh, fw, H, W, C);
    E2_LAUNCH_CHECK("softcomp_fold");
    return 0;
}
template <typename T>
static int softcomp_fold_16(const char* name, const void* emb, const float* bias_hwc, const void* residual, void* dst, int32_t F,
                            int32_t fh, int32_t fw, int32_t H, int32_t W, int32_t C, void* stream) {
    E2_REQUIRE(emb && dst, E2FGVI_EINVAL, "%s: null pointer", name);
    if (int rc = check_fold(name, F, fh, fw, H, W, C)) return rc;
    E2_REQUIRE(C % 8 == 0, E2FGVI_EINVAL, "%s: C %% 8 != 0", name);
    const long long total = (long long)F * H * W * (C / 8);
    hipLaunchKernelGGL((fold_kernel<false, T, T, T>), dim3(blocks_for(total)), dim3(NTH), 0, (hipStream_t)stream,
                       (const T*)emb, bias_hwc, (const T*)residual, (T*)dst, F, fh, fw, H, W, C);
    E2_LAUNCH_CHECK(name);
    return 0;
}
extern "C" int e2fgvi_softcomp_fold_bf16(const void* emb, const float* bias_hwc, const void* residual, void* dst, int32_t F,
                                         int32_t fh, int32_t fw, int32_t H, int32_t W, int32_t C, void* stream) {
    return softcomp_fold_16<__bf16>("softcomp_fold_bf16", emb, bias_hwc, residual, dst, F, fh, fw, H, W, C, stream);
}
extern "C" int e2fgvi_softcomp_fold_f16(const void* emb, const float* bias_hwc, const void* residual, void* dst, int32_t F,
                                        int32_t fh, int32_t fw, int32_t H, int32_t W, int32_t C, void* stream) {
    return softcomp_fold_16<_Float16>("softcomp_fold_f16", emb, bias_hwc, residual, dst, F, fh, fw, H, W, C, stream);
}

extern "C" int e2fgvi_cast(const void* src, int32_t src_dtype, void* dst, int32_t dst_dtype, int64_t n, void* stream) {
    E2_REQUIRE(src && dst && n > 0 && n % 4 == 0 && E2_DT_OK(src_dtype) && E2_DT_OK(dst_dtype) &&
                   (src_dtype == E2FGVI_F32) != (dst_dtype == E2FGVI_F32) && (((uintptr_t)src | (uintptr_t)dst) & 7) == 0,
               E2FGVI_EINVAL, "cast: bad arguments (n must be a multiple of 4, one side fp32, the other bf16 / fp16)");
    if (src_dtype == E2FGVI_F32)
        with_dtype(dst_dtype, [&](auto z) {
            using T = E2_ELEM(z);
            if constexpr (!std::is_same_v<T, float>)
                hipLaunchKernelGGL((cast_kernel<float, T>), dim3(blocks_for(n / 4)), dim3(NTH), 0, (hipStream_t)stream,
                                   (const float*)src, (T*)dst, (long long)(n / 4));
        });
    else
        with_dtype(src_dtype, [&](auto z) {
            using T = E2_ELEM(z);
            if constexpr (!std::is_same_v<T, float>)
                hipLaunchKernelGGL((cast_kernel<T, float>), dim3(blocks_for(n / 4)), dim3(NTH), 0, (hipStream_t)stream,
                                   (const T*)src, (float*)dst, (long long)(n / 4));
        });
    E2_LAUNCH_CHECK("cast");
    return 0;
}

namespace {
__global__ void nhwc_to_planar16_kernel(const uint4* __restrict__ src, uint4* __restrict__ dst, long long P, int C8) {
    const long long idx = (long long)blockIdx.x * blockDim.x + threadIdx.x;
    if (idx >= P * C8) return;
    const long long pix = idx / C8;
    const int o = (int)(idx - pix * C8);
    dst[((long long)(o >> 1) * P + pix) * 2 + (o & 1)] = src[idx];
}
}

extern "C" int e2fgvi_nhwc_to_planar16(const void* src, void* dst, int64_t P, int32_t C, void* stream) {
    E2_REQUIRE(src && dst, E2FGVI_EINVAL, "nhwc_to_planar16: null pointer");
    E2_REQUIRE(P > 0 && C > 0 && C % 16 == 0 && ((uintptr_t)src & 15) == 0 && ((uintptr_t)dst & 15) == 0, E2FGVI_EINVAL,
               "nhwc_to_planar16: C must be a multiple of 16, buffers 16-byte aligned");
    const long long n = (long long)P * (C / 8);
// ... 6 lines not shown
```

### e2fgvi_amd/engine.py

```python
import numpy as np
import os

import torch

from . import ops
from .ops import ACT_DCNPOST, ACT_LRELU, ACT_RELU, ACT_TANH, PackedConvX

BF16 = torch.bfloat16
F16 = torch.float16
FC2_CONV = ops.X3_ENABLED
WIN = (5, 9)
JOIN_AT = int(os.environ.get("E2FGVI_JOIN_AT", "0") or 0)
if JOIN_AT not in (0, 10, 12, 14, 16, 18):
    raise ValueError("E2FGVI_JOIN_AT=%d: the join sits in front of encoder.layers.10 / 12 / 14 / 16 or behind the encoder (18)" % JOIN_AT)
PROP_SPLIT = os.environ.get("E2FGVI_PROP_SPLIT", "1") != "0"


def token_grid(h, w):
    return (h + 6 - 7) // 3 + 1, (w + 6 - 7) // 3 + 1


def build_key_table(fh, fw, valid_ind_rolled):
    nwh, nww = fh // WIN[0], fw // WIN[1]
    ex = (WIN[0] // 2, WIN[1] // 2)
# ... 61 lines not shown
            return c

        cin0 = 8 if x16 else 4
        w0 = torch.zeros(64, cin0, 3, 3, device=self.device)
        w0[:, :3] = f("encoder.layers.0.weight")
        self.enc = [layer("encoder.layers.0", "encoder.layers.0", [cin0], w=w0, stride=2, pad=1)]
        for i, (cpg, g, s) in zip((2, 4, 6, 8, 10, 12, 14, 16),
                                  (([64], 1, 1), ([64], 1, 2), ([128], 1, 1), ([256], 1, 1), ([128, 192], 2, 1),
                                   ([64, 128], 4, 1), ([32, 48], 8, 1), ([256, 256], 1, 1))):
            self.enc.append(layer("encoder.layers.%d" % i, "encoder.layers.%d" % i, cpg, groups=g, stride=s, pad=1))

        self.dec = [layer(n, n, [c], pad=1) for n, c in (("decoder.0.conv", 128), ("decoder.2", 128), ("decoder.4.conv", 64))]
        tail = ops.PackedTailConv(f("decoder.6.weight"), f("decoder.6.bias"), dtype=self.dtype)
        tail.name = "decoder.6"
        if x16 and autotune:
            tail.tune = True
        self.dec.append(tail)

        self.prop = {}
        self.prop_split = {}
        for d, nparts in (("backward_", 2), ("forward_", 3)):
            p = "feat_prop_module.deform_align.%s." % d
            b = "feat_prop_module.backbone.%s." % d
            w_off0 = f(p + "conv_offset.0.weight")
            if x16:
                w_off0 = torch.cat([w_off0, w_off0.new_zeros(128, 4, 3, 3)], 1)
            off = [layer("deform_align.%sconv_offset.0" % d, p + "conv_offset.0", [128, 128, 128, 8 if x16 else 4], w=w_off0, pad=1)]
            off += [layer("deform_align.%sconv_offset.%d" % (d, k), p + "conv_offset.%d" % k, [128], pad=1) for k in (2, 4, 6)]
            dcn = ops.PackedDcn(f(p + "weight"), f(p + "bias"), 16, pad=1, mfma=precision if x16 else ("x3" if x3 else "fp32"))
            dcn.name = "deform_align.%sdcn" % d
            bb = [layer("backbone.%s0" % d, b + "0", [128] * nparts, pad=1), layer("backbone.%s2" % d, b + "2", [128], pad=1)]
            self.prop[d] = (off, dcn, bb)
            if PROP_SPLIT and not x16:
                ws = split_prop_weights(f(p + "conv_offset.0.weight"), f(b + "0.weight"))
                self.prop_split[d] = dict(
                    off_rec=layer("deform_align.%sconv_offset.0 (recurrent part)" % d, None, [128, 128, 4], w=ws["off_rec"],
                                  b=f(p + "conv_offset.0.bias"), pad=1),
                    off_cur=layer("deform_align.%sconv_offset.0 (current-frame part)" % d, None, [128], w=ws["off_cur"], pad=1),
                    bb_rec=layer("backbone.%s0 (recurrent part)" % d, None, [128], w=ws["bb_rec"], b=f(b + "0.bias"), pad=1),
                    bb_pre=layer("backbone.%s0 (non-recurrent part)" % d, None, [128] * (nparts - 1), w=ws["bb_pre"], pad=1))
        self.fusion = layer("fusion", "feat_prop_module.fusion", [128, 128], tune=True)

        self.ss = layer("ss.embedding", "ss.embedding", [128], w=f("ss.embedding.weight").view(512, 128, 7, 7), stride=3, pad=3,
                        tune=True)
        wsc = f("sc.embedding.weight").view(128, 49, 512).permute(1, 0, 2).reshape(6272, 512).contiguous()
        bsc = f("sc.embedding.bias").view(128, 49).t().reshape(6272).contiguous()
        self.sc = layer("sc.embedding", None, w=wsc, b=bsc, tune=True)
        self.sc_bias_conv = layer("sc.bias_conv", "sc.bias_conv", [128], pad=1) if self.hq else None
        self.sc_bias_hwc = None if self.hq else f("sc.bias").permute(1, 2, 0).contiguous()
        self.sc_gather = (ops.SoftCompGather(f("sc.embedding.weight"), f("sc.embedding.bias"), 128, dtype=self.dtype)
                          if x16 and self.hq else None)

        self.blocks = []
        for i in range(8):
            p = "transformer.%d." % i
            w1 = f(p + "mlp.conv1.0.weight").view(40, 49, 512).permute(1, 0, 2).reshape(1960, 512).contiguous()
            b1 = f(p + "mlp.conv1.0.bias").view(40, 49).t().reshape(1960).contiguous()
            if FC2_CONV or x16:
                fc2 = layer(p + "fc2", p + "mlp.conv2.1", [40], w=f(p + "mlp.conv2.1.weight").view(512, 40, 7, 7), stride=3, pad=3,
                            taps=True, tune=True)
            else:
                w2 = f(p + "mlp.conv2.1.weight").view(512, 40, 49).permute(0, 2, 1).reshape(512, 1960).contiguous()
                fc2 = layer(p + "fc2", p + "mlp.conv2.1", w=w2, tune=True)
            self.blocks.append(dict(
                pool_w=f(p + "pool_layers.0.weight").view(45), pool_b=f(p + "pool_layers.0.bias"),
                n1w=f(p + "norm1.weight"), n1b=f(p + "norm1.bias"), n2w=f(p + "norm2.weight"), n2b=f(p + "norm2.bias"),
                qkv=layer(p + "qkv", p + "attn.qkv", tune=True),
                proj=layer(p + "proj", p + "attn.proj", tune=True),
                fc1=layer(p + "fc1", None, w=w1, b=b1, tune=True),
                fc2=fc2,
                valid=sd[p + "attn.valid_ind_rolled"].cpu().tolist()))

        self.spy = [[layer("spynet.%d.%d" % (lv, j), "update_spynet.basic_module.%d.basic_module.%d.conv" % (lv, j), [cin], pad=3,
                           nopk=True)
                     for j, cin in enumerate((8, 32, 64, 32, 16))] for lv in range(6)]
        mean = f("update_spynet.mean").view(3)
        std = f("update_spynet.std").view(3)
        one = torch.ones(1, device=self.device)
        self.spy_scale = torch.cat([1.0 / std, one]).contiguous()
        self.spy_shift = torch.cat([-mean / std, 0 * one]).contiguous()
        self.half = torch.full((4,), 0.5, device=self.device)
        self._tables = {}
        self._zeros = {}
        self.overlap_flows = True
        self._side = None
        self._given = None
        torch.cuda.synchronize(self.device)

    def weight_bytes(self):
        seen, total = set(), 0

        def walk(o):
            nonlocal total
            if id(o) in seen:
                return
            seen.add(id(o))
            if isinstance(o, (list, tuple)):
                for v in o:
                    walk(v)
            elif isinstance(o, dict):
                for v in o.values():
                    walk(v)
            elif hasattr(o, "weight_bytes") and o is not self:
                total += o.weight_bytes()
            elif isinstance(getattr(o, "wpacked", None), torch.Tensor):
                total += o.wpacked.numel() * o.wpacked.element_size()
            elif hasattr(o, "__dict__") and type(o).__module__.startswith("e2fgvi_amd") and o is not self:
                walk(list(vars(o).values()))
        walk(list(vars(self).values()))
        return total

    def _fork_ok(self):
        return self.overlap_flows and not torch.cuda.is_current_stream_capturing()

    def _side_stream(self):
        if self._side is None:
            self._side = {}
        key = torch.cuda.current_stream(self.device).cuda_stream
        if key not in self._side:
            self._side[key] = torch.cuda.Stream(device=self.device)
        return self._side[key]

    def _zero(self, shape, dtype=torch.float32):
        key = (dtype,) + tuple(shape)
        if key not in self._zeros:
            self._zeros[key] = torch.zeros(tuple(shape), dtype=dtype, device=self.device)
        return self._zeros[key]

    def _table(self, fh, fw, blk):
        key = (fh, fw, tuple(blk["valid"]))
        if key not in self._tables:
            tab, nk = build_key_table(fh, fw, blk["valid"])
            self._tables[key] = (torch.from_numpy(tab).to(self.device), torch.from_numpy(nk).to(self.device))
        return self._tables[key]

    def flows(self, frames, l_t):
        b, t, c, H, W = frames.shape
        h, w = H // 4, W // 4
        local = frames[:, :l_t].reshape(b * l_t, c, H, W)
        if not local.is_contiguous():
            local = local.contiguous()
        small = ops.resize_bilinear(local, (h, w), True, src_nchw=True, out_ld=4, scale=self.half, shift=self.half)
        w_up = w if w % 32 == 0 else 32 * (w // 32 + 1)
        h_up = h if h % 32 == 0 else 32 * (h // 32 + 1)
        pyr = [ops.resize_bilinear(small, (h_up, w_up), False, channels=3, out_ld=4, scale=self.spy_scale,
                                   shift=self.spy_shift)]
        for _ in range(5):
            pyr.append(ops.avgpool2(pyr[-1]))
        pyr = pyr[::-1]
        nf = b * (l_t - 1)
        key = ("pairs", b, l_t, h, w)
        if key not in self._tables:
            ref, supp = [], []
            for bi in range(b):
                for i in range(l_t - 1):
                    ref.append(bi * l_t + i); supp.append(bi * l_t + i + 1)
            ref, supp = ref + supp, supp + ref
            self._tables[key] = (torch.tensor(ref, dtype=torch.int32, device=self.device),
                                 torch.tensor(supp, dtype=torch.int32, device=self.device),
                                 torch.tensor([float(w) / float(w_up), float(h) / float(h_up)], dtype=torch.float32,
                                              device=self.device))
        ref_idx, supp_idx, sc = self._tables[key]
        flow = None
        for lv in range(6):
            if self.x16:
                inp, x = ops.spynet_level_input(pyr[lv], ref_idx, supp_idx, flow, copy_dtype=self.dtype)
            else:
                inp = x = ops.spynet_level_input(pyr[lv], ref_idx, supp_idx, flow)
            cv = self.spy[lv]
            x = cv[0]([x], act=ACT_RELU)
            x = cv[1]([x], act=ACT_RELU)
            x = cv[2]([x], act=ACT_RELU)
            x = cv[3]([x], act=ACT_RELU)
            flow = cv[4]([x], out_dtype=torch.float32, residual=inp, res_coff=6)
        flow = ops.resize_bilinear(flow, (h, w), False, scale=sc)
        fwd = flow[:nf].view(b, l_t - 1, h, w, 2)
        bwd = flow[nf:].view(b, l_t - 1, h, w, 2)
        return fwd, bwd

    def encode(self, frames, join=None):
        b, t, c, H, W = frames.shape
        x = ops.nchw_to_nhwc(frames.reshape(b * t, c, H, W).contiguous(), ld=8 if self.x16 else 4, out_dtype=self.dtype)
        e = self.enc
        lr = dict(act=ACT_LRELU, slope=0.2)
        x = e[0]([x], **lr)
        x = e[1]([x], **lr)
        x = e[2]([x], **lr)
        x0 = e[3]([x], **lr)
        x = e[4]([x0], **lr)
        join_at = 18 if self.x16 else (JOIN_AT or (16 if b == 1 else 10))
        joined = join is None
        if not joined and join_at <= 10:
            join()
            joined = True
        for k in (5, 6, 7, 8):
            x = e[k]([x0, x], **lr)
            if not joined and (join_at <= 2 * k + 2 or k == 8):
                join()
                joined = True
        return x

    def propagate(self, loc, flows_a, flows_b, inplace=False):
        l_t, b, h, w, ch = loc.shape
        dev = loc.device
        x16 = self.x16
        feats = {}
        zero = self._zero((b, h, w, ch), self.dtype)
        zero_dcn = self._zero((ch // 16, b, h, w, 16), self.dtype) if x16 else zero
        lk = dict(act=ACT_LRELU, slope=0.1)
        split = bool(self.prop_split) and b == 1 and l_t >= 3
        main = torch.cuda.current_stream()
        side = self._side_stream() if (split and self._fork_ok()) else None
        pre, ready = {}, {}
        if split:
            n1 = (l_t - 1) * b
            for k in ("off backward_", "bb backward_", "off forward_", "bb forward_"):
                pre[k] = torch.empty((l_t - 1, b, h, w, ch), dtype=torch.float32, device=dev)
# ... 10 lines not shown
                    with torch.cuda.stream(side):
                        layer(srcs, out=flat(pre[key]))
                        ready[key] = torch.cuda.Event()
                        ready[key].record(side)
            sb, sf = self.prop_split["backward_"], self.prop_split["forward_"]
            beside([("off backward_", sb["off_cur"], [lb]), ("bb backward_", sb["bb_pre"], [lb]), ("off forward_", sf["off_cur"], [lf])])

        def partial(key, slot):
            ev = ready.pop(key, None)
            if ev is not None:
                main.wait_event(ev)
            return pre[key][slot]
        for name, flows in (("backward_", flows_a), ("forward_", flows_b)):
            off_convs, dcn, bb = self.prop[name]
            sp = self.prop_split.get(name) if split else None
            if sp is not None and name == "forward_":
                beside([("bb forward_", sp["bb_pre"], [lf, flat(feats["backward_"][1:])])])
            store = torch.empty((l_t, b, h, w, ch), dtype=self.dtype, device=dev)
            order = list(range(l_t))
            if name == "backward_":
                order = order[::-1]
            img_stride = (l_t - 1) * h * w * 2
            hist = []
            hist_dcn = [] if x16 else hist
            aligned = zero
            for i, idx in enumerate(order):
                cur = loc[idx]
                if i > 0:
                    flow_a = flows[0, i - 1]
                    flow_b = flows[0, i - 2] if i > 1 else None
                    feat_n2 = hist[-2] if i > 1 else None
                    if x16:
                        cond, fl, fl_src = ops.prop_cond(hist[-1], feat_n2, flow_a, flow_b, img_stride, cond_dtype=self.dtype, flows8=True)
                    else:
                        cond, fl = ops.prop_cond(hist[-1], feat_n2, flow_a, flow_b, img_stride)
                        fl_src = fl
                    if sp is not None:
                        slot = idx if name == "backward_" else idx - 1
                        x = sp["off_rec"]([(cond, 0), (cond, ch), fl], residual=partial("off " + name, slot), **lk)
                    else:
                        x = off_convs[0]([(cond, 0), cur, (cond, ch), fl_src], **lk)
                    x = off_convs[1]([x], **lk)
                    x = off_convs[2]([x], **lk)
                    offs = off_convs[3]([x], out_dtype=torch.float32, residual=fl, act=ACT_DCNPOST, slope=10.0)
                    aligned = dcn([hist_dcn[-1], hist_dcn[-2] if i > 1 else zero_dcn], offs, out_dtype=self.dtype, planar=x16)
                if sp is not None and i > 0:
                    y = sp["bb_rec"]([aligned], residual=partial("bb " + name, idx if name == "backward_" else idx - 1), **lk)
                else:
                    srcs = [cur, feats["backward_"][idx], aligned] if name == "forward_" else [cur, aligned]
                    y = bb[0](srcs, **lk)
                hist.append(bb[1]([y], residual=aligned, out=store[idx]))
                if x16 and i + 1 < l_t:
                    hist_dcn.append(ops.to_planar16(store[idx]))
            feats[name] = store
        out = self.fusion([feats["backward_"].view(l_t * b, h, w, ch), feats["forward_"].view(l_t * b, h, w, ch)],
                          residual=loc.view(l_t * b, h, w, ch), out=loc.view(l_t * b, h, w, ch) if inplace else None)
        return out.view(l_t, b, h, w, ch)

    def soft_split(self, feat):
        return self.ss([feat], out_dtype=torch.float32)

    def block(self, i, x, b, t, fh, fw, hw, out2=None):
        blk = self.blocks[i]
        H, W = hw
        tab, nk = self._table(fh, fw, blk)
        rows = x.shape[0]
        prow = b * t * (fh // 5) * (fw // 9)
        nbuf = torch.empty((rows + prow, 512), dtype=self.dtype, device=x.device)
        n1 = ops.layernorm(x, blk["n1w"], blk["n1b"], out=nbuf[:rows])
        ops.window_pool(n1, blk["pool_w"], blk["pool_b"], b * t, fh, fw, out=nbuf[rows:])
        if self.x16:
            both = blk["qkv"](nbuf)
            att = ops.focal_attention_bf16(both[:rows], both[rows:], tab, nk, b, t, fh, fw)
        elif ops.attention_x3_applies(b, t, fh, fw):
            planes = torch.empty((3, rows + prow, 1024), dtype=torch.bfloat16, device=x.device)
            both = blk["qkv"](nbuf, kv_planes=planes)
            att = ops.focal_attention_x3(both[:rows], planes, tab, nk, b, t, fh, fw)
        else:
            both = blk["qkv"](nbuf)
            att = ops.focal_attention(both[:rows], both[rows:], tab, nk, b, t, fh, fw)
        x1 = blk["proj"](att, out_dtype=torch.float32, residual=x)
        n2 = ops.layernorm(x1, blk["n2w"], blk["n2b"], out_dtype=self.dtype)
        hid = blk["fc1"](n2)
        folded = ops.ffn_fold_gelu(hid, b * t, fh, fw, H, W, 40)
        if isinstance(blk["fc2"], PackedConvX):
            y = torch.empty((rows, 512), dtype=torch.float32, device=x.device)
            blk["fc2"]([folded], out=y.view(b * t, fh, fw, 512), residual=x1.view(b * t, fh, fw, 512),
                       out2=None if out2 is None else out2.view(b * t, fh, fw, 512))
            return y, x1
        unf = ops.ffn_unfold(folded, fh, fw, out=hid)
        return blk["fc2"](unf, residual=x1), x1

    def compose(self, tokens, enc, b, t, fh, fw):
        _, h, w, ch = enc.shape
        if self.sc_gather is not None and (h, w) == (3 * fh, 3 * fw):
            folded = self.sc_gather(tokens.view(b * t, fh, fw, 512))
            return self.sc_bias_conv([folded], residual=enc)
        emb = self.sc(tokens)
        if self.hq:
            folded = ops.softcomp_fold(emb, b * t, fh, fw, h, w, ch)
            return self.sc_bias_conv([folded], residual=enc)
        return ops.softcomp_fold(emb, b * t, fh, fw, h, w, ch, bias_hwc=self.sc_bias_hwc, residual=enc)

    def decode(self, x):
        n, h, w, _ = x.shape
        lr = dict(act=ACT_LRELU, slope=0.2)
        d = self.dec
        x = ops.resize_bilinear(x, (2 * h, 2 * w), True)
        x = d[0]([x], **lr)
        x = d[1]([x], **lr)
        x = ops.resize_bilinear(x, (4 * h, 4 * w), True)
        x = d[2]([x], **lr)
        return d[3]([x], act=ACT_TANH, out_nchw=True)

    def forward(self, frames, l_t, trace=None):
        b, t, c, H, W = frames.shape
        if H % 4 or W % 4:
            raise ValueError("H and W must be multiples of 4")
        h, w = H // 4, W // 4
        fh, fw = token_grid(h, w)
        if fh % 5 or fw % 9:
            raise ValueError("token grid %dx%d is not a multiple of (5,9): pad H to a multiple of 60 and W to a "
                             "multiple of 108 (reference test.py:156-165)" % (fh, fw))
        if not self.hq and (h, w) != (60, 108):
            raise ValueError("model 'e2fgvi' is fixed to 432x240 inputs (sc.bias is [128,60,108]); use e2fgvi_hq")
        if not (1 <= l_t <= t):
            raise ValueError("num_local_frames must be in [1, t]")
        frames = ops._chk(frames.float().contiguous(), "masked_frames")
        if self._given is not None:
            (fwd, bwd), enc = self._given
        elif l_t == 1:
            fwd = bwd = torch.empty((b, 0, h, w, 2), dtype=torch.float32, device=frames.device)
            enc = self.encode(frames)
        elif self._fork_ok():
            main = torch.cuda.current_stream()
            side = self._side_stream()
            side.wait_stream(main)
            with torch.cuda.stream(side):
                fwd, bwd = self.flows(frames, l_t)
            enc = self.encode(frames, join=lambda: main.wait_stream(side))
        else:
            fwd, bwd = self.flows(frames, l_t)
            enc = self.encode(frames)
        ch = enc.shape[3]
        if trace is not None:
            trace["flow_fwd"], trace["flow_bwd"], trace["enc"] = fwd, bwd, enc.to(torch.float32, copy=True)
        enc5 = enc.view(b, t, h, w, ch)
        if b == 1:
            loc = enc5[0, :l_t].unsqueeze(1)
            inplace = not (ops.AUTOTUNE or self.x16)
            prop = self.propagate(loc, fwd, bwd, inplace=inplace)
            if not inplace:
                enc5[0, :l_t].copy_(prop[:, 0])
        else:
            loc = enc5[:, :l_t].permute(1, 0, 2, 3, 4).contiguous()
            prop = self.propagate(loc, fwd, bwd)
            enc5[:, :l_t].copy_(prop.permute(1, 0, 2, 3, 4))
        if trace is not None:
            trace["prop"] = enc.to(torch.float32, copy=True)
        tok = self.soft_split(enc).view(b * t * fh * fw, 512)
        if trace is not None:
            trace["tokens0"] = tok.clone()
        tok16 = None
        for i in range(8):
            if self.x16 and i == 7:
                tok16 = torch.empty((b * t * fh * fw, 512), dtype=self.dtype, device=tok.device)
            tok, x1 = self.block(i, tok, b, t, fh, fw, (h, w), out2=tok16)
# ... 14 lines not shown
```

### e2fgvi_amd/lib.py

```python
import ctypes as C
import os

_HERE = os.path.dirname(os.path.abspath(__file__))
LIB_PATH = os.environ.get("E2FGVI_LIB") or os.path.join(_HERE, "csrc", "libe2fgvi_hip.so")

ABI_VERSION = 8
MAX_SRC = 4
ACT_NONE, ACT_RELU, ACT_LRELU, ACT_TANH, ACT_DCNPOST = 0, 1, 2, 3, 4
DT_F32, DT_BF16 = 0, 1
DT_F16 = 3

_fp = C.c_void_p


class ConvDesc(C.Structure):
    _fields_ = [
        ("src", _fp * MAX_SRC), ("src_ld", C.c_int32 * MAX_SRC), ("src_coff", C.c_int32 * MAX_SRC),
        ("src_cpg", C.c_int32 * MAX_SRC), ("nsrc", C.c_int32),
        ("N", C.c_int32), ("H", C.c_int32), ("W", C.c_int32), ("Ho", C.c_int32), ("Wo", C.c_int32),
        ("KH", C.c_int32), ("KW", C.c_int32), ("stride", C.c_int32), ("pad", C.c_int32),
        ("groups", C.c_int32), ("Cout", C.c_int32), ("bk", C.c_int32),
        ("wpacked", _fp), ("bias", _fp), ("residual", _fp), ("res_ld", C.c_int32), ("res_coff", C.c_int32),
        ("dst", _fp), ("dst_ld", C.c_int32), ("dst_coff", C.c_int32), ("dst_nchw", C.c_int32),
        ("act", C.c_int32), ("slope", C.c_float), ("tile", C.c_int32),
# ... 37 lines not shown
SYMBOLS = {
    "e2fgvi_last_error": (C.c_char_p, []),
    "e2fgvi_abi_version": (C.c_int, []),
    "e2fgvi_nhwc_to_planar16": (C.c_int, [_fp, _fp, _i64, _i32, _fp]),
    "e2fgvi_conv2d_nhwc": (C.c_int, [C.POINTER(ConvDesc), _fp]),
    "e2fgvi_conv2d_nhwc_nopk": (C.c_int, [C.POINTER(ConvDesc), _fp]),
    "e2fgvi_packed_conv_weight_size": (_i64, [_i32, _i32, _i32, _i32, _i32, C.POINTER(_i32), _i32]),
    "e2fgvi_pack_conv_weight": (C.c_int, [_fp, _fp, _i32, _i32, _i32, _i32, _i32, C.POINTER(_i32), _i32, _fp]),
    "e2fgvi_conv2d_bf16x": (C.c_int, [C.POINTER(ConvXDesc), _fp]),
    "e2fgvi_packed_conv_weight_bf16x_size": (_i64, [_i32, _i32, _i32, _i32, _i32, C.POINTER(_i32)]),
    "e2fgvi_pack_conv_weight_bf16x": (C.c_int, [_fp, _fp, _i32, _i32, _i32, _i32, _i32, C.POINTER(_i32), _fp]),
    "e2fgvi_packed_conv_weight_bf16x_taps_size": (_i64, [_i32, _i32, _i32, _i32]),
    "e2fgvi_pack_conv_weight_bf16x_taps": (C.c_int, [_fp, _fp, _i32, _i32, _i32, _i32, _fp]),
    "e2fgvi_conv2d_f16x": (C.c_int, [C.POINTER(ConvXDesc), _fp]),
    "e2fgvi_packed_conv_weight_f16x_size": (_i64, [_i32, _i32, _i32, _i32, _i32, C.POINTER(_i32)]),
    "e2fgvi_pack_conv_weight_f16x": (C.c_int, [_fp, _fp, _i32, _i32, _i32, _i32, _i32, C.POINTER(_i32), _fp]),
    "e2fgvi_packed_conv_weight_f16x_taps_size": (_i64, [_i32, _i32, _i32, _i32]),
    "e2fgvi_pack_conv_weight_f16x_taps": (C.c_int, [_fp, _fp, _i32, _i32, _i32, _i32, _fp]),
    "e2fgvi_packed_conv_weight_f32x_taps_size": (_i64, [_i32, _i32, _i32, _i32]),
    "e2fgvi_pack_conv_weight_f32x_taps": (C.c_int, [_fp, _fp, _i32, _i32, _i32, _i32, _fp]),
    "e2fgvi_conv2d_f32x": (C.c_int, [C.POINTER(ConvXDesc), _fp]),
    "e2fgvi_packed_conv_weight_f32x_size": (_i64, [_i32, _i32, _i32, _i32, _i32, C.POINTER(_i32)]),
    "e2fgvi_pack_conv_weight_f32x": (C.c_int, [_fp, _fp, _i32, _i32, _i32, _i32, _i32, C.POINTER(_i32), _fp]),
    "e2fgvi_conv2d_f32x3": (C.c_int, [C.POINTER(ConvXDesc), _fp]),
    "e2fgvi_packed_conv_weight_f32x3_size": (_i64, [_i32, _i32, _i32, _i32, _i32, C.POINTER(_i32)]),
    "e2fgvi_pack_conv_weight_f32x3": (C.c_int, [_fp, _fp, _i32, _i32, _i32, _i32, _i32, C.POINTER(_i32), _fp]),
    "e2fgvi_packed_conv_weight_f32x3_taps_size": (_i64, [_i32, _i32, _i32, _i32]),
    "e2fgvi_pack_conv_weight_f32x3_taps": (C.c_int, [_fp, _fp, _i32, _i32, _i32, _i32, _fp]),
    "e2fgvi_packed_winograd_weight_size": (_i64, [_i32, _i32, _i32, C.POINTER(_i32)]),
    "e2fgvi_pack_winograd_weight": (C.c_int, [_fp, _fp, _i32, _i32, _i32, C.POINTER(_i32), _fp]),
    "e2fgvi_conv3x3_winograd": (C.c_int, [C.POINTER(ConvDesc), _fp]),
    "e2fgvi_packed_winograd_weight_x3_size": (_i64, [_i32, _i32, _i32, C.POINTER(_i32)]),
    "e2fgvi_pack_winograd_weight_x3": (C.c_int, [_fp, _fp, _i32, _i32, _i32, C.POINTER(_i32), _fp]),
    "e2fgvi_conv3x3_winograd_x3": (C.c_int, [C.POINTER(ConvDesc), _fp]),
    "e2fgvi_packed_winograd4_weight_size": (_i64, [_i32, _i32, _i32, C.POINTER(_i32), _i32]),
    "e2fgvi_pack_winograd4_weight": (C.c_int, [_fp, _fp, _i32, _i32, _i32, C.POINTER(_i32), _i32, _fp]),
    "e2fgvi_conv3x3_winograd4": (C.c_int, [C.POINTER(ConvDesc), _i32, _fp]),
    "e2fgvi_packed_tail_weight_size": (_i64, [_i32, _i32]),
    "e2fgvi_pack_tail_weight": (C.c_int, [_fp, _fp, _i32, _i32, _i32, _fp]),
    "e2fgvi_conv3x3_tail": (C.c_int, [_fp, _i32, _i32, _fp, _fp, _fp, _i32, _i32, _i32, _i32, C.c_float, _fp]),
    "e2fgvi_mdcn_nhwc": (C.c_int, [C.POINTER(MdcnDesc), _fp]),
    "e2fgvi_packed_dcn_weight_size": (_i64, [_i32, _i32, _i32, _i32]),
    "e2fgvi_pack_dcn_weight": (C.c_int, [_fp, _fp, _i32, _i32, _i32, _i32, _i32, _fp]),
    "e2fgvi_pack_dcn_weight_bf16": (C.c_int, [_fp, _fp, _i32, _i32, _i32, _i32, _i32, _fp]),
    "e2fgvi_pack_dcn_weight_f16": (C.c_int, [_fp, _fp, _i32, _i32, _i32, _i32, _i32, _fp]),
    "e2fgvi_pack_dcn_weight_x3": (C.c_int, [_fp, _fp, _i32, _i32, _i32, _i32, _i32, _fp]),
    "e2fgvi_focal_attention": (C.c_int, [_fp, _fp, _fp, _i32, _fp, _fp, _i32, _i32, _i32, _i32, _i32, _fp]),
    "e2fgvi_split3_kv": (C.c_int, [_fp, _fp, _i64, _fp]),
    "e2fgvi_focal_attention_x3": (C.c_int, [_fp, _fp, _fp, _i32, _fp, _fp, _i32, _i32, _i32, _i32, _i32, _fp]),
    "e2fgvi_nchw_to_nhwc": (C.c_int, [_fp, _fp, _i32, _i32, _i32, _i32, _i32, _f, _f, _fp]),
    "e2fgvi_nhwc_to_nchw": (C.c_int, [_fp, _i32, _fp, _i32, _i32, _i32, _i32, _fp]),
    "e2fgvi_resize_bilinear": (C.c_int, [_fp, _i32, _i32, _fp, _i32, _i32, _i32, _i32, _i32, _i32, _i32, _i32, _fp, _fp, _fp]),
    "e2fgvi_avgpool2_nhwc": (C.c_int, [_fp, _fp, _i32, _i32, _i32, _i32, _fp]),
    "e2fgvi_spynet_level_input": (C.c_int, [_fp, _fp, _fp, _fp, _fp, _i32, _i32, _i32, _fp]),
    "e2fgvi_prop_cond": (C.c_int, [_fp, _i32, _fp, _i32, _fp, _fp, _i64, _fp, _fp, _i32, _i32, _i32, _i32, _fp]),
    "e2fgvi_layernorm": (C.c_int, [_fp, _fp, _fp, _fp, _i64, _i32, _fp]),
    "e2fgvi_window_pool": (C.c_int, [_fp, _fp, _fp, _fp, _i32, _i32, _i32, _i32, _fp]),
    "e2fgvi_ffn_fold": (C.c_int, [_fp, _fp, _i32, _i32, _i32, _i32, _i32, _i32, _fp]),
    "e2fgvi_ffn_unfold_gelu": (C.c_int, [_fp, _fp, _i32, _i32, _i32, _i32, _i32, _i32, _fp]),
    "e2fgvi_mask_prepare": (C.c_int, [_fp, _i32, _i32, _i32, _fp, _fp, _fp, _i32, _i32, _i32, _fp]),
    "e2fgvi_masked_clip": (C.c_int, [_fp, _fp, _fp, _i32, _i32, _i32, _fp, _i32, _i32, _fp]),
    "e2fgvi_composite": (C.c_int, [_fp, _fp, _fp, _i32, _fp, _fp, _fp, _i32, _i32, _i32, _i32, _fp]),
    "e2fgvi_resample_u8": (C.c_int, [_fp, _fp, _i32, _i32, _i32, _i32, _i32, _fp, _fp, _i32, _fp]),
    "e2fgvi_float_to_u8": (C.c_int, [_fp, _fp, _i64, _fp]),
    "e2fgvi_pred_to_u8": (C.c_int, [_fp, _fp, _i32, _i32, _i32, _i32, _i32, _fp]),
    "e2fgvi_psnr_ssim_workspace": (_i64, [_i32, _i32, _i32]),
    "e2fgvi_psnr_ssim": (C.c_int, [_fp, _fp, _i32, _i32, _i32, _i32, _fp, _fp, _fp]),
    "e2fgvi_softcomp_fold": (C.c_int, [_fp, _fp, _fp, _fp, _i32, _i32, _i32, _i32, _i32, _i32, _fp]),
    "e2fgvi_focal_attention_bf16": (C.c_int, [_fp, _fp, _fp, _i32, _fp, _fp, _i32, _i32, _i32, _i32, _fp]),
    "e2fgvi_focal_attention_bf16_variant": (C.c_int, [C.c_int]),
    "e2fgvi_focal_attention_f16": (C.c_int, [_fp, _fp, _fp, _i32, _fp, _fp, _i32, _i32, _i32, _i32, _fp]),
    "e2fgvi_nchw_to_nhwc_x": (C.c_int, [_fp, _fp, _i32, _i32, _i32, _i32, _i32, _i32, _f, _f, _fp]),
    "e2fgvi_resize_bilinear_bf16": (C.c_int, [_fp, _i32, _fp, _i32, _i32, _i32, _i32, _i32, _i32, _i32, _i32, _fp]),
    "e2fgvi_resize_bilinear_f16": (C.c_int, [_fp, _i32, _fp, _i32, _i32, _i32, _i32, _i32, _i32, _i32, _i32, _fp]),
    "e2fgvi_prop_cond_x": (C.c_int, [_fp, _i32, _fp, _i32, _fp, _fp, _i64, _fp, _i32, _fp, _fp, _i32, _i32, _i32, _i32, _fp]),
    "e2fgvi_prop_cond_xs": (C.c_int, [_fp, _i32, _fp, _i32, _i32, _fp, _fp, _i64, _fp, _i32, _fp, _fp, _i32, _i32, _i32, _i32, _fp]),
    "e2fgvi_spynet_level_input_x": (C.c_int, [_fp, _fp, _fp, _fp, _fp, _fp, _i32, _i32, _i32, _fp]),
    "e2fgvi_spynet_level_input_x_f16": (C.c_int, [_fp, _fp, _fp, _fp, _fp, _fp, _i32, _i32, _i32, _fp]),
    "e2fgvi_layernorm_x": (C.c_int, [_fp, _fp, _fp, _fp, _i32, _i64, _i32, _fp]),
    "e2fgvi_window_pool_x": (C.c_int, [_fp, _i32, _fp, _fp, _fp, _i32, _i32, _i32, _i32, _fp]),
    "e2fgvi_ffn_fold_x": (C.c_int, [_fp, _fp, _i32, _i32, _i32, _i32, _i32, _i32, _i32, _fp]),
    "e2fgvi_ffn_unfold_gelu_x": (C.c_int, [_fp, _fp, _i32, _i32, _i32, _i32, _i32, _i32, _i32, _fp]),
    "e2fgvi_ffn_fold_gelu_x": (C.c_int, [_fp, _fp, _i32, _i32, _i32, _i32, _i32, _i32, _i32, _fp]),
    "e2fgvi_ffn_unfold_x": (C.c_int, [_fp, _fp, _i32, _i32, _i32, _i32, _i32, _i32, _i32, _fp]),
    "e2fgvi_softcomp_fold_bf16": (C.c_int, [_fp, _fp, _fp, _fp, _i32, _i32, _i32, _i32, _i32, _i32, _fp]),
    "e2fgvi_softcomp_fold_f16": (C.c_int, [_fp, _fp, _fp, _fp, _i32, _i32, _i32, _i32, _i32, _i32, _fp]),
    "e2fgvi_cast": (C.c_int, [_fp, _i32, _fp, _i32, _i64, _fp]),
}

_lib = None

TRACE = None
NEXT_META = None


X3_PIPE = 6 * 157.3 / 2500.0


def useful_macs(kernel, macs, issued):
    import re
    k = str(kernel)
    f = 1.0
    m = re.match(r"conv_wino4<F\((\d)x4\)", k)
    if m:
        fy = int(m.group(1))
        f = (fy + 2) * 6 / (fy * 4 * 9.0)
    elif k.startswith("conv_wino"):
        f = 16 / 36.0
    if "x3" in k:
        f *= X3_PIPE
    return min(int(issued), int(macs * f))


def annotate(**meta):
    global NEXT_META
    if TRACE is not None:
        if "macs" in meta and "issued" in meta and "useful" not in meta:
            meta["useful"] = useful_macs(meta.get("kernel", ""), meta["macs"], meta["issued"])
        NEXT_META = meta


def _traced(name, fn):
    def call(*args):
        global NEXT_META
        if TRACE is None:
            return fn(*args)
        import torch
        e0, e1 = torch.cuda.Event(enable_timing=True), torch.cuda.Event(enable_timing=True)
        e0.record()
        rc = fn(*args)
        e1.record()
        TRACE.append({"symbol": name, "e0": e0, "e1": e1, "meta": NEXT_META})
        NEXT_META = None
        return rc
    call.__name__ = name
    return call


class HipLibraryMissing(ImportError):
    pass


def load():
    global _lib
    if _lib is not None:
        return _lib
    if not os.path.exists(LIB_PATH):
        raise HipLibraryMissing(
            "libe2fgvi_hip.so not found at %s -- the MI355X kernels are mandatory (no CPU / eager "
            "fallback exists).  Build them: python -m e2fgvi_amd.build" % LIB_PATH)
    lib = C.CDLL(LIB_PATH)
    for name, (res, args) in SYMBOLS.items():
        fn = getattr(lib, name)
        fn.restype = res
        fn.argtypes = args
        if args and args[-1] is _fp and res is C.c_int:
            setattr(lib, name, _traced(name, fn))
    have = int(lib.e2fgvi_abi_version())
    if have != ABI_VERSION:
        raise HipLibraryMissing("%s implements ABI version %d, this binding is version %d: rebuild it (python -m e2fgvi_amd.build)"
                                % (LIB_PATH, have, ABI_VERSION))
    _lib = lib
    return lib


class HipError(RuntimeError):
# ... 17 lines not shown
```

### e2fgvi_amd/ops.py

```python
import ctypes as C
import math
import os

import torch

from . import lib as _L

ACT_NONE, ACT_RELU, ACT_LRELU, ACT_TANH, ACT_DCNPOST = _L.ACT_NONE, _L.ACT_RELU, _L.ACT_LRELU, _L.ACT_TANH, _L.ACT_DCNPOST


def _stream():
    return C.c_void_p(torch.cuda.current_stream().cuda_stream)


def _chk(t, name, dtype=torch.float32):
    if not isinstance(t, torch.Tensor) or not t.is_cuda:
        raise TypeError("%s must be a CUDA (ROCm) tensor -- the HIP path has no CPU fallback" % name)
    if t.dtype != dtype:
        raise TypeError("%s must be %s, got %s" % (name, dtype, t.dtype))
    if not t.is_contiguous():
        raise ValueError("%s must be contiguous" % name)
    return t


def _ptr(t):
    return C.c_void_p(t.data_ptr()) if t is not None else C.c_void_p(0)


def empty_nhwc(n, h, w, c, device):
    return torch.empty((n, h, w, c), dtype=torch.float32, device=device)


TUNE_CANDIDATES = (0, 213, 223, 211, 219, 216)
WINO_CANDIDATES = (64, 132, 164, 32)
W4_CODES = {2464: (2, 64)}
_W4_MINPIX = 20000
XTUNE_CANDIDATES = (1, 4, 6, 7, 8, 2, 5, 3, 107, 108)
XTUNE_ROWSHIFT = (11, 16, 17, 12, 13, 18)
X3_ENABLED = os.environ.get("E2FGVI_X3", "1") != "0"
X3_MARGIN = 0.97
X3_BASE = 30000
W3_BASE = 40000
W3_CANDIDATES = (132, 164, 32, 5132, 6064)
W3_WIDE = 6064
W3_WIDE_FALLBACK = 164
_TUNED = {}
AUTOTUNE = os.environ.get("E2FGVI_AUTOTUNE", "0") == "1"
TUNE_REPS = max(1, int(os.environ.get("E2FGVI_TUNE_REPS", "1") or 1))
TABLE_FORMAT = 2
_SIZE_FIELD = 8


def _default_tune_file():
    try:
        st = os.stat(_L.LIB_PATH)
        d = os.environ.get("E2FGVI_CACHE_DIR") or os.path.join(os.path.dirname(os.path.abspath(__file__)), ".tile_cache")
        os.makedirs(d, exist_ok=True)
        dev = "gpu"
        if torch.cuda.is_available():
            dev = "".join(ch for ch in torch.cuda.get_device_properties(0).gcnArchName.split(":")[0] if ch.isalnum())
        return os.path.join(d, "tiles_v%d_%s_%x_%x.txt" % (TABLE_FORMAT, dev, st.st_size, int(st.st_mtime)))
    except (OSError, RuntimeError):
        return None


_TUNE_FILE = None
if AUTOTUNE:
    _TUNE_FILE = os.environ.get("E2FGVI_TUNE_FILE")
    if _TUNE_FILE is None:
        _TUNE_FILE = _default_tune_file()
    elif _TUNE_FILE in ("", "0"):
        _TUNE_FILE = None
    if _TUNE_FILE and os.path.exists(_TUNE_FILE):
        import ast
        for _line in open(_TUNE_FILE):
            try:
                _k, _v = ast.literal_eval(_line)
                _TUNED[_k] = _v
            except Exception:
                pass
elif os.environ.get("E2FGVI_TILE_TABLE", "1") != "0":
    try:
        if os.environ.get("E2FGVI_TILE_TABLE", "1").endswith(".py"):
            import importlib.util
            _spec = importlib.util.spec_from_file_location("e2fgvi_tile_table_override", os.environ["E2FGVI_TILE_TABLE"])
            _tt = importlib.util.module_from_spec(_spec)
            _spec.loader.exec_module(_tt)
        else:
            from . import tile_table as _tt
        if getattr(_tt, "TABLE_FORMAT", None) == TABLE_FORMAT:
            _TUNED.update(_tt.TILES)
    except ImportError:
        pass


def _remember(key, tile):
    _TUNED[key] = tile
    if _TUNE_FILE:
        try:
            with open(_TUNE_FILE, "a") as fh:
                fh.write(repr((key, tile)) + "\n")
        except OSError:
            pass
    return tile


def _decision(key):
    best = _TUNED.get(key)
    if best is not None or AUTOTUNE:
        return best
    hit = _NEAREST.get(key)
    if hit is None:
        sc = key[_SIZE_FIELD]
        cands = [(abs(k[_SIZE_FIELD] - sc), k[_SIZE_FIELD], v) for k, v in _TUNED.items()
                 if len(k) == len(key) and k[:_SIZE_FIELD] == key[:_SIZE_FIELD] and k[_SIZE_FIELD + 1:] == key[_SIZE_FIELD + 1:]]
        hit = _NEAREST[key] = (min(cands)[2] if cands else -1)
    return None if hit < 0 else hit


_NEAREST = {}


def sync_tile_decisions(group=None, src=0):
    import torch.distributed as dist
# ... 327 lines not shown
                        for _ in range(3):
                            launch()
                        e1.record()
                        e1.synchronize()
                        t = min(t, e0.elapsed_time(e1) / 3)
                    return t
                if self.tune and not use_wino and not self.nopk and self._alt() is not None:
                    d.tile = best
                    mine = time_mine()
                    res = self.alt._time_tiles(self.alt._desc(srcs, out, out_coff, residual, res_coff, act, slope, None, out_nchw))
                    if res and min(res.values()) < mine:
                        best, mine = 2000 + min(res, key=res.get), min(res.values())
                if x3 and self._alt3() is not None:
                    if mine is None:
                        d.tile = best
                        mine = time_mine()
                    d3 = self.alt3._desc(srcs, out, out_coff, residual, res_coff, act, slope, None, out_nchw)
                    if kv_planes is not None:
                        self.alt3._set_planes(d3, kv_planes, self.Cout - kv_planes.shape[2], N * Ho * Wo)
                    res = self.alt3._time_tiles(d3)
                    if res and min(res.values()) < X3_MARGIN * mine:
                        best, mine = X3_BASE + min(res, key=res.get), min(res.values())
                if x3 and use_wino and self._wino_x3() is not None:
                    w3 = {}
                    for shape in W3_CANDIDATES:
                        if launch_w3(shape)[0] != 0:
                            continue
                        e0, e1 = torch.cuda.Event(enable_timing=True), torch.cuda.Event(enable_timing=True)
                        w3[shape] = float("inf")
                        for _ in range(TUNE_REPS):
                            e0.record()
                            for _ in range(3):
                                launch_w3(shape)
                            e1.record()
                            e1.synchronize()
                            w3[shape] = min(w3[shape], e0.elapsed_time(e1) / 3)
                    if w3 and min(w3.values()) < X3_MARGIN * mine:
                        best, mine = W3_BASE + min(w3, key=w3.get), min(w3.values())
                best = _remember(key, best)
            try:
                if best and best >= W3_BASE and self._wino_x3() is not None:
                    w3_tile = best - W3_BASE
                elif best and X3_BASE <= best < W3_BASE and self._alt3() is not None:
                    return self.alt3(srcs, out=out, out_coff=out_coff, residual=residual, res_coff=res_coff, act=act, slope=slope,
                                     tile=best - X3_BASE, out_nchw=out_nchw, planes=kv_planes,
                                     split_from=(self.Cout - kv_planes.shape[2]) if kv_planes is not None else 0)
                elif best and self.tune and 2000 <= best < 2100 and self._alt() is not None:
                    r = self.alt(srcs, out=out, out_coff=out_coff, residual=residual, res_coff=res_coff, act=act, slope=slope,
                                 tile=best - 2000, out_nchw=out_nchw)
                    if kv_planes is not None:
                        split3_kv(out.view(-1, out.shape[-1]), out=kv_planes)
                    return r
                elif self.tune and best is not None and best < 2000:
                    d.tile = best
            except _L.HipError:
                if not from_table:
                    raise
                w3_tile = None
        if _L.TRACE is not None:
            _L.annotate(**self._work(N, H, W, Ho, Wo, use_wino, d.tile if w3_tile is None else W3_BASE + w3_tile))
        rc, what = launch()
        if rc != 0 and (w3_tile is not None or d.tile != tile0):
            w3_tile, d.tile = None, tile0
            rc, what = launch()
        _L.check(rc, what)
        if kv_planes is not None:
            split3_kv(out.view(-1, out.shape[-1]), out=kv_planes)
        return out


HALF16 = (torch.bfloat16, torch.float16)


def _dt(t):
    if t.dtype == torch.float32:
        return _L.DT_F32
    if t.dtype == torch.bfloat16:
        return _L.DT_BF16
    if t.dtype == torch.float16:
        return _L.DT_F16
    raise TypeError("tensor must be float32, bfloat16 or float16, got %s" % t.dtype)


def _dt_key(t):
    return _L.DT_BF16 if t.dtype == torch.float16 else _dt(t)


def _chk_any(t, name):
    if not isinstance(t, torch.Tensor) or not t.is_cuda:
        raise TypeError("%s must be a CUDA (ROCm) tensor -- the HIP path has no CPU fallback" % name)
    if not t.is_contiguous():
        raise ValueError("%s must be contiguous" % name)
    _dt(t)
    return t


class PackedConvX:

    def __init__(self, weight, bias, cpg, groups=1, stride=1, pad=0, dtype=torch.bfloat16, taps=None, x3=False):
        lib = _L.load()
        if weight.dim() == 2:
            weight = weight[:, :, None, None]
        w = _chk(weight.detach().float().contiguous(), "weight")
        self.Cout, cin_g, self.KH, self.KW = w.shape
        self.cpg = [int(c) for c in cpg]
        if sum(self.cpg) != cin_g:
            raise ValueError("sum(cpg)=%d != weight input channels %d" % (sum(self.cpg), cin_g))
        self.groups, self.stride, self.pad = groups, stride, pad
        self.dtype = dtype
        self.f32 = dtype == torch.float32
        self.x3 = bool(x3)
        if self.x3 and not self.f32:
            raise ValueError("x3 splitting is for fp32 sources")
        self.f16 = dtype == torch.float16
        if not self.f32 and dtype not in HALF16:
            raise TypeError("PackedConvX: dtype must be float32, bfloat16 or float16")
        self._fn = ((lib.e2fgvi_conv2d_f32x3 if self.x3 else lib.e2fgvi_conv2d_f32x) if self.f32 else
                    lib.e2fgvi_conv2d_f16x if self.f16 else lib.e2fgvi_conv2d_bf16x)
        wdtype = torch.bfloat16 if self.x3 else dtype
        self.name = "conv"
        self.tune = False
        self.try_x3 = False
        self.alt3 = None
        self._w_raw = w if (self.f32 and not self.x3) else None
        self._taps_arg = taps
        arr = (C.c_int32 * len(self.cpg))(*self.cpg)
        self.taps = (len(self.cpg) == 1 and groups == 1 and self.cpg[0] <= 56 and self.KW > 1
                     and (taps is True if self.f32 else taps is not False))
        self._wdtype = wdtype
        self._wp = None
        self.bias = None if bias is None else _chk(bias.detach().float().contiguous(), "bias")
        if self._w_raw is None:
            self._wp = self._pack(w)
        else:
            self._pack(w, dry=True)

    @property
    def wpacked(self):
        if self._wp is None:
            _no_capture(self.name + " (LDS-DMA GEMM weights)")
            self._wp = self._pack(self._w_raw)
        return self._wp

    def weight_bytes(self):
        return (0 if self._wp is None else self._wp.numel() * self._wp.element_size()) + (self.alt3.weight_bytes() if self.alt3 is not None else 0)

    def _pack(self, w, dry=False):
        lib = _L.load()
        wdtype = self._wdtype
        arr = (C.c_int32 * len(self.cpg))(*self.cpg)
        if self.taps:
            size_fn = ((lib.e2fgvi_packed_conv_weight_f32x3_taps_size if self.x3 else lib.e2fgvi_packed_conv_weight_f32x_taps_size)
                       if self.f32 else lib.e2fgvi_packed_conv_weight_f16x_taps_size if self.f16
                       else lib.e2fgvi_packed_conv_weight_bf16x_taps_size)
            pack_fn = ((lib.e2fgvi_pack_conv_weight_f32x3_taps if self.x3 else lib.e2fgvi_pack_conv_weight_f32x_taps)
                       if self.f32 else lib.e2fgvi_pack_conv_weight_f16x_taps if self.f16 else lib.e2fgvi_pack_conv_weight_bf16x_taps)
            n = size_fn(self.Cout, self.KH, self.KW, self.cpg[0])
            if n < 0:
                _L.check(int(n), "packed_conv_weight_x_taps_size")
            if dry:
                return None
            t = torch.empty(int(n), dtype=wdtype, device=w.device)
            _L.check(pack_fn(_ptr(w), _ptr(t), self.Cout, self.KH, self.KW, self.cpg[0], _stream()),
                     "pack_conv_weight_x_taps")
        else:
            size_fn = ((lib.e2fgvi_packed_conv_weight_f32x3_size if self.x3 else lib.e2fgvi_packed_conv_weight_f32x_size)
                       if self.f32 else lib.e2fgvi_packed_conv_weight_f16x_size if self.f16 else lib.e2fgvi_packed_conv_weight_bf16x_size)
            pack_fn = ((lib.e2fgvi_pack_conv_weight_f32x3 if self.x3 else lib.e2fgvi_pack_conv_weight_f32x)
                       if self.f32 else lib.e2fgvi_pack_conv_weight_f16x if self.f16 else lib.e2fgvi_pack_conv_weight_bf16x)
            n = size_fn(self.Cout, self.groups, self.KH, self.KW, len(self.cpg), arr)
            if n < 0:
                _L.check(int(n), "packed_conv_weight_x_size")
            if dry:
                return None
            t = torch.empty(int(n), dtype=wdtype, device=w.device)
            _L.check(pack_fn(_ptr(w), _ptr(t), self.Cout, self.groups, self.KH, self.KW, len(self.cpg), arr, _stream()),
                     "pack_conv_weight_x")
        return t

    def out_hw(self, H, W):
        return ((H + 2 * self.pad - self.KH) // self.stride + 1, (W + 2 * self.pad - self.KW) // self.stride + 1)

    def _alt3(self):
        if self.alt3 is None and self._w_raw is not None:
            _no_capture(self.name + " (split-operand GEMM alternative)")
            self.alt3 = PackedConvX(self._w_raw, self.bias, self.cpg, groups=self.groups, stride=self.stride, pad=self.pad,
                                    dtype=torch.float32, taps=self._taps_arg, x3=True)
            self.alt3.name = self.name
        return self.alt3

    def _desc(self, srcs, out, out_coff, residual, res_coff, act, slope, out2, out_nchw):
        d = _L.ConvXDesc()
        N, H, W, _ = srcs[0][0].shape
        Ho, Wo = self.out_hw(H, W)
        for i, (t, coff) in enumerate(srcs):
            _chk(t, "source %d" % i, self.dtype)
            if t.dim() != 4 or tuple(t.shape[:3]) != (N, H, W):
                raise ValueError("source %d shape %s does not match [%d,%d,%d,*]" % (i, tuple(t.shape), N, H, W))
            d.src[i], d.src_ld[i], d.src_coff[i], d.src_cpg[i] = t.data_ptr(), t.shape[3], coff, self.cpg[i]
        d.nsrc = len(srcs)
        d.N, d.H, d.W, d.Ho, d.Wo = N, H, W, Ho, Wo
        d.KH, d.KW, d.stride, d.pad = self.KH, self.KW, self.stride, self.pad
        d.groups, d.Cout = self.groups, self.Cout
        d.wpacked = None if self._wp is None else self._wp.data_ptr()
        d.bias = self.bias.data_ptr() if self.bias is not None else None
        _chk_any(out, "out")
        if out_nchw:
            if tuple(out.shape) != (N, self.Cout, Ho, Wo) or out.dtype != torch.float32:
                raise ValueError("NCHW out must be fp32 %s" % ((N, self.Cout, Ho, Wo),))
            d.dst, d.dst_ld, d.dst_coff, d.dst_dtype, d.dst_nchw = out.data_ptr(), 0, 0, _L.DT_F32, 1
        else:
            if out.dim() != 4 or tuple(out.shape[:3]) != (N, Ho, Wo):
                raise ValueError("out shape %s != [%d,%d,%d,*]" % (tuple(out.shape), N, Ho, Wo))
            d.dst, d.dst_ld, d.dst_coff, d.dst_dtype = out.data_ptr(), out.shape[3], out_coff, _dt(out)
        if out2 is not None:
            _chk(out2, "out2", torch.float16 if self.f16 else torch.bfloat16)
            if out2.dim() != 4 or tuple(out2.shape[:3]) != (N, Ho, Wo):
                raise ValueError("out2 shape %s != [%d,%d,%d,*]" % (tuple(out2.shape), N, Ho, Wo))
            d.dst2, d.dst2_ld, d.dst2_coff = out2.data_ptr(), out2.shape[3], 0
        if residual is not None:
            _chk_any(residual, "residual")
            if residual.dim() != 4 or tuple(residual.shape[:3]) != (N, Ho, Wo):
                raise ValueError("residual shape %s != [%d,%d,%d,*]" % (tuple(residual.shape), N, Ho, Wo))
            d.residual, d.res_ld, d.res_coff, d.res_dtype = residual.data_ptr(), residual.shape[3], res_coff, _dt(residual)
        d.act, d.slope, d.tile = act, slope, 0
        d.tap_packed = 1 if self.taps else 0
        return d

    @staticmethod
    def _set_planes(d, planes, split_from, rows):
        _chk(planes, "planes", torch.bfloat16)
        if planes.dim() != 3 or planes.shape[0] != 3 or planes.shape[1] != rows or planes.shape[2] != d.Cout - split_from:
            raise ValueError("planes must be [3, %d, %d] bf16, got %s" % (rows, d.Cout - split_from, tuple(planes.shape)))
        d.dst2, d.dst2_ld, d.dst2_coff = planes.data_ptr(), planes.shape[2], 0
        d.dst2_split_from, d.dst2_plane_stride = split_from, planes.shape[1] * planes.shape[2]

    def __call__(self, sources, out=None, out_dtype=None, out_coff=0, residual=None, res_coff=0, act=ACT_NONE,
                 slope=0.0, out2=None, tile=0, out_nchw=False, planes=None, split_from=0):
        if out_dtype is None:
            out_dtype = self.dtype
        srcs = [(s, 0) if isinstance(s, torch.Tensor) else s for s in sources]
        if len(srcs) != len(self.cpg):
            raise ValueError("expected %d sources, got %d" % (len(self.cpg), len(srcs)))
        N, H, W, _ = srcs[0][0].shape
        Ho, Wo = self.out_hw(H, W)
        dev = srcs[0][0].device
        if out is None:
            out = (torch.empty((N, self.Cout, Ho, Wo), dtype=torch.float32, device=dev) if out_nchw else
                   torch.empty((N, Ho, Wo, self.Cout), dtype=out_dtype, device=dev))
        per_img = max(H * W * t.shape[3] * (4 if self.f32 else 2) for t, _ in srcs)
        if N > 1 and N * per_img >= (1 << 32) - 1:
            if planes is not None:
                raise ValueError("split planes: the batch spans >= 4 GiB (call in chunks)")
            step = max(1, ((1 << 32) - 2) // per_img)
            for n0 in range(0, N, step):
                n1 = min(N, n0 + step)
                self([(t[n0:n1], c) for t, c in srcs], out=out[n0:n1], out_coff=out_coff,
                     residual=None if residual is None else residual[n0:n1], res_coff=res_coff, act=act, slope=slope,
                     out2=None if out2 is None else out2[n0:n1], tile=tile, out_nchw=out_nchw)
            return out
        d = self._desc(srcs, out, out_coff, residual, res_coff, act, slope, out2, out_nchw)
        if planes is not None:
            self._set_planes(d, planes, split_from, N * Ho * Wo)
        d.tile = tile
        x3 = self.try_x3 and X3_ENABLED and self.f32 and not self.x3
        if tile == 0 and self.tune and N * Ho * Wo >= 2048:
            key = (("x3" if self.x3 else ("x32+3" if x3 else "x32")) if self.f32 else "x", self.Cout, tuple(self.cpg), self.KH, self.KW, self.stride, self.pad, self.groups,
                   int(4.0 * math.log2(N * Ho * Wo)), _dt_key(out), out_nchw, self.taps)
            best = _decision(key)
            if best is None and AUTOTUNE and not torch.cuda.is_current_stream_capturing() and (
                    residual is None or residual.data_ptr() != out.data_ptr()):
                res = self._time_tiles(d)
                best = min(res, key=res.get) if res else 0
                if x3 and self._alt3() is not None:
                    res3 = self.alt3._time_tiles(self.alt3._desc(srcs, out, out_coff, residual, res_coff, act, slope, out2, out_nchw))
                    if res3 and (not res or min(res3.values()) < X3_MARGIN * min(res.values())):
                        best = X3_BASE + min(res3, key=res3.get)
                best = _remember(key, best)
            if best and best >= X3_BASE and self._alt3() is not None:
                try:
                    return self.alt3(srcs, out=out, out_dtype=out_dtype, out_coff=out_coff, residual=residual, res_coff=res_coff, act=act,
                                     slope=slope, out2=out2, tile=best - X3_BASE, out_nchw=out_nchw, planes=planes, split_from=split_from)
                except _L.HipError:
                    best = 0
            d.tile = tile = (best or 0) if (best or 0) < X3_BASE else 0
        if _L.TRACE is not None:
            cin_g, cout_g, K2 = sum(self.cpg), self.Cout // self.groups, self.KH * self.KW
            kc = 32 if self.f32 else 64
            cin_p = sum(-(-c // kc) * kc for c in self.cpg)
            if self.taps:
                cin_p = -(-K2 * (self.cpg[0] // (4 if self.f32 else 8)) // 8) * kc / K2
            _L.annotate(layer=self.name, kernel="conv_%s tile=%d%s" % (("f32x3" if self.x3 else "f32x") if self.f32 else
                                                                      "f16x" if self.f16 else "bf16x", tile,
                                                                      " taps" if self.taps else ""),
                        shape="N%d %dx%d %d->%d k%d s%d g%d" % (N, H, W, cin_g * self.groups, self.Cout, self.KH, self.stride, self.groups),
                        macs=N * Ho * Wo * self.Cout * cin_g * K2,
                        issued=int(N * Ho * Wo * (-(-cout_g // 32) * 32) * self.groups * cin_p * K2 * (6 * 157.3 / 2500.0 if self.x3 else 1)))
        d.wpacked = self.wpacked.data_ptr()
        rc = self._fn(C.byref(d), _stream())
        if rc != 0 and d.tile and self.tune:
            d.tile = 0
            rc = self._fn(C.byref(d), _stream())
        _L.check(rc, "conv2d_x")
        return out

    def _time_tiles(self, d, reps=3, rounds=2):
        st = _stream()
        res = {}
        d.tile = 0
        d.wpacked = self.wpacked.data_ptr()
        for _ in range(2):
            self._fn(C.byref(d), st)
        for _ in range(rounds * TUNE_REPS):
            rowshift = (self.KH, self.KW, self.stride, self.pad) == (3, 3, 1, 1) and not self.f32 and not self.taps
            for code in XTUNE_CANDIDATES + (XTUNE_ROWSHIFT if rowshift else ()):
                if code % 10 == 3 and self.Cout // self.groups > 64:
                    continue
                if code in (12, 18) and self.Cout // self.groups > 64:
                    continue
                d.tile = code
                if self._fn(C.byref(d), st) != 0:
                    continue
                e0, e1 = torch.cuda.Event(enable_timing=True), torch.cuda.Event(enable_timing=True)
                e0.record()
                for _ in range(reps):
                    self._fn(C.byref(d), st)
                e1.record()
                e1.synchronize()
                res[code] = min(res.get(code, float("inf")), e0.elapsed_time(e1) / reps)
        d.tile = 0
        return res


class SoftCompGather:

    def __init__(self, weight, bias, channels=128, dtype=torch.bfloat16):
        w = _chk(weight.detach().float().contiguous(), "weight")
        if w.dim() != 2 or w.shape[0] != 49 * channels:
            raise ValueError("SoftComp embedding weight must be [%d, hidden]" % (49 * channels))
        self.C, self.hidden, self.dtype = channels, w.shape[1], dtype
        w4 = w.view(channels, 7, 7, self.hidden)
        self.phases = []
        for py in range(3):
            ky_taps = [6, 3, 0] if py == 0 else [py + 3, py]
            for px in range(3):
                kx_taps = [6, 3, 0] if px == 0 else [px + 3, px]
                wp = w4[:, ky_taps][:, :, kx_taps].permute(0, 3, 1, 2).contiguous()
                layer = PackedConvX(wp, None, [self.hidden], dtype=dtype)
                layer.name = "sc.embedding phase (%d,%d)" % (py, px)
                self.phases.append((py, px, 1 if py == 0 else 0, 1 if px == 0 else 0, layer))
        self.bias = None if bias is None else _chk(bias.detach().float().contiguous(), "bias")
        self._bias_img = {}
        self.tile = 0

    def bias_image(self, fh, fw):
        key = (fh, fw)
        if key not in self._bias_img and self.bias is not None:
            rows = self.bias.view(self.C, 49).t().reshape(1, 49 * self.C).expand(fh * fw, 49 * self.C).contiguous()
            self._bias_img[key] = softcomp_fold(rows, 1, fh, fw, 3 * fh, 3 * fw, self.C)[0].contiguous()
        return self._bias_img.get(key)

    def __call__(self, tokens, out=None, out_dtype=None):
        _chk(tokens, "tokens", self.dtype)
        F_, fh, fw, hid = tokens.shape
        if hid != self.hidden:
            raise ValueError("tokens must be [F, fh, fw, %d]" % self.hidden)
        H, W = 3 * fh, 3 * fw
        if out is None:
            out = torch.empty((F_, H, W, self.C), dtype=out_dtype or self.dtype, device=tokens.device)
        if tuple(out.shape) != (F_, H, W, self.C):
            raise ValueError("out must be [%d,%d,%d,%d]" % (F_, H, W, self.C))
        per_img = fh * fw * hid * tokens.element_size()
        if F_ > 1 and F_ * per_img >= (1 << 32) - 1:
            step = max(1, ((1 << 32) - 2) // per_img)
            for n0 in range(0, F_, step):
                self(tokens[n0:n0 + step], out=out[n0:n0 + step])
            return out
        bimg = self.bias_image(fh, fw)
        for py, px, pad_y, pad_x, layer in self.phases:
            d = _L.ConvXDesc()
            d.src[0], d.src_ld[0], d.src_coff[0], d.src_cpg[0], d.nsrc = tokens.data_ptr(), hid, 0, hid, 1
            d.N, d.H, d.W, d.Ho, d.Wo = F_, fh, fw, fh, fw
            d.KH, d.KW, d.stride, d.pad = layer.KH, layer.KW, 1, pad_y
            d.groups, d.Cout = 1, self.C
            d.wpacked = layer.wpacked.data_ptr()
            d.dst, d.dst_ld, d.dst_coff, d.dst_dtype = out.data_ptr(), self.C, 0, _dt(out)
            if bimg is not None:
# ... 392 lines not shown
    _chk_any(feat_prop, "feat_prop")
    N, H, W, Cc = feat_prop.shape
    if cond is None:
        cond = torch.empty((N, H, W, 2 * Cc), dtype=cond_dtype, device=feat_prop.device)
    if flows is None:
        flows = empty_nhwc(N, H, W, 4, feat_prop.device)
    fl8 = (torch.empty((N, H, W, 8), dtype=cond.dtype if cond.dtype == torch.float16 else torch.bfloat16, device=feat_prop.device)
           if flows8 else None)
    f2_ld = 0
    if flow_b is not None:
        _chk(feat_n2, "feat_n2", feat_prop.dtype)
        f2_ld = feat_n2.shape[3]
    _L.check(lib.e2fgvi_prop_cond_xs(_ptr(feat_prop), Cc, _ptr(feat_n2) if flow_b is not None else None, f2_ld, _dt(feat_prop),
                                    C.c_void_p(flow_a.data_ptr()),
                                    C.c_void_p(flow_b.data_ptr()) if flow_b is not None else None,
                                    flow_img_stride, _ptr(cond), _dt(cond), _ptr(flows), _ptr(fl8), N, H, W, Cc, _stream()),
             "prop_cond")
    return (cond, flows, fl8) if flows8 else (cond, flows)


def layernorm(x, gamma, beta, out=None, out_dtype=torch.float32):
    lib = _L.load()
    _chk(x, "x"); _chk(gamma, "gamma"); _chk(beta, "beta")
    Cc = x.shape[-1]
    rows = x.numel() // Cc
    if out is None:
        out = torch.empty(x.shape, dtype=out_dtype, device=x.device)
    _chk_any(out, "out")
    _L.check(lib.e2fgvi_layernorm_x(_ptr(x), _ptr(gamma), _ptr(beta), _ptr(out), _dt(out), rows, Cc, _stream()), "layernorm")
    return out


def window_pool(x, w45, bias1, BT, fh, fw, out=None):
    lib = _L.load()
    _chk_any(x, "x"); _chk(w45, "w45"); _chk(bias1, "bias1")
    Cc = x.shape[-1]
    rows = BT * (fh // 5) * (fw // 9)
    if out is None:
        out = torch.empty((rows, Cc), dtype=x.dtype, device=x.device)
    elif tuple(_chk(out, "out", x.dtype).shape) != (rows, Cc):
        raise ValueError("window_pool out must be [%d,%d]" % (rows, Cc))
    _L.check(lib.e2fgvi_window_pool_x(_ptr(x), _dt(x), _ptr(w45), _ptr(bias1), _ptr(out), BT, fh, fw, Cc, _stream()), "window_pool")
    return out


def ffn_fold(hid, F_, fh, fw, H, W, Cc):
    lib = _L.load()
    _chk_any(hid, "hid")
    out = torch.empty((F_, H, W, Cc), dtype=hid.dtype, device=hid.device)
    _L.check(lib.e2fgvi_ffn_fold_x(_ptr(hid), _ptr(out), _dt(hid), F_, fh, fw, H, W, Cc, _stream()), "ffn_fold")
    return out


def to_planar16(x, out=None):
    dt = x.dtype if isinstance(x, torch.Tensor) and x.dtype == torch.float16 else torch.bfloat16
    _chk(x, "x", dt)
    N, H, W, Cc = x.shape
    if out is None:
        out = torch.empty((Cc // 16, N, H, W, 16), dtype=dt, device=x.device)
    _chk(out, "out", dt)
    _L.check(_L.load().e2fgvi_nhwc_to_planar16(_ptr(x), _ptr(out), N * H * W, Cc, _stream()), "nhwc_to_planar16")
    return out


def ffn_unfold_gelu(folded, fh, fw, out=None):
    lib = _L.load()
    _chk_any(folded, "folded")
    F_, H, W, Cc = folded.shape
    if out is None:
        out = torch.empty((F_ * fh * fw, 49 * Cc), dtype=folded.dtype, device=folded.device)
    _chk(out, "out", folded.dtype)
    _L.check(lib.e2fgvi_ffn_unfold_gelu_x(_ptr(folded), _ptr(out), _dt(folded), F_, fh, fw, H, W, Cc, _stream()), "ffn_unfold_gelu")
    return out


def ffn_fold_gelu(hid, F_, fh, fw, H, W, Cc):
    lib = _L.load()
    _chk_any(hid, "hid")
    out = torch.empty((F_, H, W, Cc), dtype=hid.dtype, device=hid.device)
    _L.check(lib.e2fgvi_ffn_fold_gelu_x(_ptr(hid), _ptr(out), _dt(hid), F_, fh, fw, H, W, Cc, _stream()), "ffn_fold_gelu")
    return out


def ffn_unfold(folded, fh, fw, out=None):
    lib = _L.load()
    _chk_any(folded, "folded")
    F_, H, W, Cc = folded.shape
    if out is None:
        out = torch.empty((F_ * fh * fw, 49 * Cc), dtype=folded.dtype, device=folded.device)
    _chk(out, "out", folded.dtype)
    _L.check(lib.e2fgvi_ffn_unfold_x(_ptr(folded), _ptr(out), _dt(folded), F_, fh, fw, H, W, Cc, _stream()), "ffn_unfold")
    return out


def softcomp_fold(emb, F_, fh, fw, H, W, Cc, bias_hwc=None, residual=None):
    lib = _L.load()
    if isinstance(emb, torch.Tensor) and emb.dtype in HALF16:
        _chk(emb, "emb", emb.dtype)
        out = torch.empty((F_, H, W, Cc), dtype=emb.dtype, device=emb.device)
        if bias_hwc is not None:
            _chk(bias_hwc, "bias_hwc")
        if residual is not None:
            _chk(residual, "residual", emb.dtype)
        fn = lib.e2fgvi_softcomp_fold_f16 if emb.dtype == torch.float16 else lib.e2fgvi_softcomp_fold_bf16
        _L.check(fn(_ptr(emb), _ptr(bias_hwc), _ptr(residual), _ptr(out), F_, fh, fw, H, W, Cc, _stream()), "softcomp_fold_16")
        return out
    _chk(emb, "emb")
    out = empty_nhwc(F_, H, W, Cc, emb.device)
    if bias_hwc is not None:
        _chk(bias_hwc, "bias_hwc")
    if residual is not None:
        _chk(residual, "residual")
    _L.check(lib.e2fgvi_softcomp_fold(_ptr(emb), _ptr(bias_hwc), _ptr(residual), _ptr(out), F_, fh, fw, H, W, Cc,
                                      _stream()), "softcomp_fold")
    return out


def _u8(t, name):
    return _chk(t, name, torch.uint8)


def mask_prepare(masks_u8, ytab, xtab, H, W, iterations=4):
    lib = _L.load()
    _u8(masks_u8, "masks")
    _chk(ytab, "ytab", torch.int32); _chk(xtab, "xtab", torch.int32)
    L, Hin, Win = masks_u8.shape
    if ytab.numel() != H or xtab.numel() != W:
        raise ValueError("ytab / xtab must have H / W entries")
    out = torch.empty((L, H, W), dtype=torch.uint8, device=masks_u8.device)
    _L.check(lib.e2fgvi_mask_prepare(_ptr(masks_u8), L, Hin, Win, _ptr(ytab), _ptr(xtab), _ptr(out), H, W, iterations, _stream()),
             "mask_prepare")
    return out


def masked_clip(frames_u8, masks01, ids, Hp, Wp):
    lib = _L.load()
    _u8(frames_u8, "frames"); _u8(masks01, "masks"); _chk(ids, "ids", torch.int32)
    L, H, W, _ = frames_u8.shape
    t = ids.numel()
    out = torch.empty((1, t, 3, Hp, Wp), dtype=torch.float32, device=frames_u8.device)
    _L.check(lib.e2fgvi_masked_clip(_ptr(frames_u8), _ptr(masks01), _ptr(ids), t, H, W, _ptr(out), Hp, Wp, _stream()), "masked_clip")
    return out


def composite(pred, ids, first, frames_u8, masks01, comp):
    lib = _L.load()
    _chk(pred, "pred"); _chk(ids, "ids", torch.int32); _u8(first, "first"); _u8(frames_u8, "frames"); _u8(masks01, "masks")
    _chk(comp, "comp")
    L, H, W, _ = frames_u8.shape
    n = ids.numel()
    if pred.shape[0] < n or pred.shape[1] != 3:
        raise ValueError("pred must hold at least %d frames of 3 channels" % n)
    _L.check(lib.e2fgvi_composite(_ptr(pred), _ptr(ids), _ptr(first), n, _ptr(frames_u8), _ptr(masks01), _ptr(comp), H, W,
                                  pred.shape[2], pred.shape[3], _stream()), "composite")
    return comp


def resample_u8(frames_u8, n_out, axis, bounds, coeffs):
    lib = _L.load()
    _u8(frames_u8, "frames"); _chk(bounds, "bounds", torch.int32); _chk(coeffs, "coeffs", torch.int32)
    if frames_u8.dim() != 4 or frames_u8.shape[3] != 3:
        raise ValueError("frames must be [L,H,W,3], got %s" % (tuple(frames_u8.shape),))
    if axis not in (1, 2):
        raise ValueError("axis must be 1 (H) or 2 (W), got %r" % (axis,))
    if bounds.device != frames_u8.device or coeffs.device != frames_u8.device:
        raise ValueError("frames, bounds and coeffs must be on one device")
# ... 33 lines not shown
```

### e2fgvi_amd/tile_table.py

```python
TABLE_FORMAT = 2
TILES = {
    ('x', 128, (128, 128), 1, 1, 1, 0, 1, 63, 1, False, False): 1,
    ('x', 128, (128, 128), 1, 1, 1, 0, 1, 76, 1, False, False): 4,
    ('x', 128, (128, 128), 1, 1, 1, 0, 1, 85, 1, False, False): 4,
    ('x', 128, (128, 128), 3, 3, 1, 1, 1, 50, 1, False, False): 5,
    ('x', 128, (128, 128), 3, 3, 1, 1, 1, 63, 1, False, False): 1,
    ('x', 128, (128, 128), 3, 3, 1, 1, 1, 68, 1, False, False): 4,
    ('x', 128, (128, 128, 128), 3, 3, 1, 1, 1, 50, 1, False, False): 5,
    ('x', 128, (128, 128, 128), 3, 3, 1, 1, 1, 63, 1, False, False): 11,
    ('x', 128, (128, 128, 128), 3, 3, 1, 1, 1, 68, 1, False, False): 4,
    ('x', 128, (128, 128, 128, 8), 3, 3, 1, 1, 1, 50, 1, False, False): 5,
    ('x', 128, (128, 128, 128, 8), 3, 3, 1, 1, 1, 63, 1, False, False): 11,
    ('x', 128, (128, 128, 128, 8), 3, 3, 1, 1, 1, 68, 1, False, False): 11,
    ('x', 128, (128,), 3, 3, 1, 1, 1, 50, 1, False, False): 5,
    ('x', 128, (128,), 3, 3, 1, 1, 1, 63, 1, False, False): 6,
    ('x', 128, (128,), 3, 3, 1, 1, 1, 68, 1, False, False): 4,
    ('x', 128, (128,), 3, 3, 1, 1, 1, 71, 1, False, False): 1,
    ('x', 128, (128,), 3, 3, 1, 1, 1, 76, 1, False, False): 1,
    ('x', 128, (128,), 3, 3, 1, 1, 1, 84, 1, False, False): 1,
    ('x', 128, (128,), 3, 3, 1, 1, 1, 85, 1, False, False): 6,
    ('x', 128, (128,), 3, 3, 1, 1, 1, 93, 1, False, False): 6,
    ('x', 128, (256, 256), 3, 3, 1, 1, 1, 63, 1, False, False): 16,
    ('x', 128, (256, 256), 3, 3, 1, 1, 1, 76, 1, False, False): 11,
    ('x', 128, (256, 256), 3, 3, 1, 1, 1, 85, 1, False, False): 11,
# ... 42 lines not shown
    ('x', 256, (32, 48), 3, 3, 1, 1, 8, 63, 1, False, False): 13,
    ('x', 256, (32, 48), 3, 3, 1, 1, 8, 76, 1, False, False): 13,
    ('x', 256, (32, 48), 3, 3, 1, 1, 8, 85, 1, False, False): 13,
    ('x', 32, (64,), 7, 7, 1, 3, 1, 44, 1, False, False): 5,
    ('x', 32, (64,), 7, 7, 1, 3, 1, 48, 1, False, False): 5,
    ('x', 32, (64,), 7, 7, 1, 3, 1, 49, 1, False, False): 5,
    ('x', 32, (64,), 7, 7, 1, 3, 1, 52, 1, False, False): 5,
    ('x', 32, (64,), 7, 7, 1, 3, 1, 56, 1, False, False): 5,
    ('x', 32, (64,), 7, 7, 1, 3, 1, 57, 1, False, False): 5,
    ('x', 32, (64,), 7, 7, 1, 3, 1, 60, 1, False, False): 3,
    ('x', 32, (64,), 7, 7, 1, 3, 1, 64, 1, False, False): 3,
    ('x', 32, (64,), 7, 7, 1, 3, 1, 65, 1, False, False): 3,
    ('x', 32, (64,), 7, 7, 1, 3, 1, 68, 1, False, False): 3,
    ('x', 32, (64,), 7, 7, 1, 3, 1, 72, 1, False, False): 3,
    ('x', 32, (64,), 7, 7, 1, 3, 1, 73, 1, False, False): 3,
    ('x', 32, (64,), 7, 7, 1, 3, 1, 80, 1, False, False): 3,
    ('x', 32, (64,), 7, 7, 1, 3, 1, 81, 1, False, False): 3,
    ('x', 32, (64,), 7, 7, 1, 3, 1, 89, 1, False, False): 3,
    ('x', 32, (8,), 7, 7, 1, 3, 1, 44, 1, False, True): 5,
    ('x', 32, (8,), 7, 7, 1, 3, 1, 48, 1, False, True): 5,
    ('x', 32, (8,), 7, 7, 1, 3, 1, 49, 1, False, True): 5,
    ('x', 32, (8,), 7, 7, 1, 3, 1, 52, 1, False, True): 5,
    ('x', 32, (8,), 7, 7, 1, 3, 1, 56, 1, False, True): 5,
    ('x', 32, (8,), 7, 7, 1, 3, 1, 57, 1, False, True): 5,
    ('x', 32, (8,), 7, 7, 1, 3, 1, 60, 1, False, True): 5,
    ('x', 32, (8,), 7, 7, 1, 3, 1, 64, 1, False, True): 3,
    ('x', 32, (8,), 7, 7, 1, 3, 1, 65, 1, False, True): 3,
    ('x', 32, (8,), 7, 7, 1, 3, 1, 68, 1, False, True): 3,
    ('x', 32, (8,), 7, 7, 1, 3, 1, 72, 1, False, True): 3,
    ('x', 32, (8,), 7, 7, 1, 3, 1, 73, 1, False, True): 3,
    ('x', 32, (8,), 7, 7, 1, 3, 1, 80, 1, False, True): 3,
    ('x', 32, (8,), 7, 7, 1, 3, 1, 81, 1, False, True): 3,
    ('x', 32, (8,), 7, 7, 1, 3, 1, 89, 1, False, True): 3,
    ('x', 384, (256,), 3, 3, 1, 1, 1, 63, 1, False, False): 8,
    ('x', 384, (256,), 3, 3, 1, 1, 1, 76, 1, False, False): 8,
    ('x', 384, (256,), 3, 3, 1, 1, 1, 85, 1, False, False): 8,
    ('x', 384, (64, 128), 3, 3, 1, 1, 4, 63, 1, False, False): 11,
    ('x', 384, (64, 128), 3, 3, 1, 1, 4, 76, 1, False, False): 11,
    ('x', 384, (64, 128), 3, 3, 1, 1, 4, 85, 1, False, False): 11,
    ('x', 432, (128,), 3, 3, 1, 1, 1, 50, 0, False, False): 5,
    ('x', 432, (128,), 3, 3, 1, 1, 1, 63, 0, False, False): 2,
    ('x', 432, (128,), 3, 3, 1, 1, 1, 68, 0, False, False): 2,
    ('x', 512, (128, 192), 3, 3, 1, 1, 2, 63, 1, False, False): 7,
    ('x', 512, (128, 192), 3, 3, 1, 1, 2, 76, 1, False, False): 17,
    ('x', 512, (128, 192), 3, 3, 1, 1, 2, 85, 1, False, False): 7,
    ('x', 512, (128,), 7, 7, 3, 3, 1, 51, 0, False, False): 4,
    ('x', 512, (128,), 7, 7, 3, 3, 1, 63, 0, False, False): 7,
    ('x', 512, (128,), 7, 7, 3, 3, 1, 72, 0, False, False): 7,
    ('x', 512, (40,), 7, 7, 3, 3, 1, 51, 0, False, True): 4,
    ('x', 512, (40,), 7, 7, 3, 3, 1, 63, 0, False, True): 7,
    ('x', 512, (40,), 7, 7, 3, 3, 1, 72, 0, False, True): 7,
    ('x', 512, (512,), 1, 1, 1, 0, 1, 51, 0, False, False): 4,
    ('x', 512, (512,), 1, 1, 1, 0, 1, 63, 0, False, False): 7,
    ('x', 512, (512,), 1, 1, 1, 0, 1, 72, 0, False, False): 7,
    ('x', 6272, (512,), 1, 1, 1, 0, 1, 51, 1, False, False): 7,
    ('x', 64, (128,), 3, 3, 1, 1, 1, 71, 1, False, False): 2,
    ('x', 64, (128,), 3, 3, 1, 1, 1, 84, 1, False, False): 2,
    ('x', 64, (128,), 3, 3, 1, 1, 1, 93, 1, False, False): 2,
    ('x', 64, (32,), 7, 7, 1, 3, 1, 44, 1, False, True): 5,
    ('x', 64, (32,), 7, 7, 1, 3, 1, 48, 1, False, True): 5,
    ('x', 64, (32,), 7, 7, 1, 3, 1, 49, 1, False, True): 5,
    ('x', 64, (32,), 7, 7, 1, 3, 1, 52, 1, False, True): 5,
    ('x', 64, (32,), 7, 7, 1, 3, 1, 56, 1, False, True): 5,
    ('x', 64, (32,), 7, 7, 1, 3, 1, 57, 1, False, True): 5,
    ('x', 64, (32,), 7, 7, 1, 3, 1, 60, 1, False, True): 5,
    ('x', 64, (32,), 7, 7, 1, 3, 1, 64, 1, False, True): 2,
    ('x', 64, (32,), 7, 7, 1, 3, 1, 65, 1, False, True): 2,
    ('x', 64, (32,), 7, 7, 1, 3, 1, 68, 1, False, True): 5,
    ('x', 64, (32,), 7, 7, 1, 3, 1, 72, 1, False, True): 2,
    ('x', 64, (32,), 7, 7, 1, 3, 1, 73, 1, False, True): 2,
    ('x', 64, (32,), 7, 7, 1, 3, 1, 80, 1, False, True): 2,
    ('x', 64, (32,), 7, 7, 1, 3, 1, 81, 1, False, True): 2,
    ('x', 64, (32,), 7, 7, 1, 3, 1, 89, 1, False, True): 2,
    ('x', 64, (64,), 3, 3, 1, 1, 1, 71, 1, False, False): 2,
    ('x', 64, (64,), 3, 3, 1, 1, 1, 79, 1, False, False): 2,
    ('x', 64, (64,), 3, 3, 1, 1, 1, 84, 1, False, False): 2,
    ('x', 64, (64,), 3, 3, 1, 1, 1, 92, 1, False, False): 2,
    ('x', 64, (64,), 3, 3, 1, 1, 1, 93, 1, False, False): 2,
    ('x', 64, (64,), 3, 3, 1, 1, 1, 99, 1, False, False): 2,
    ('x', 64, (8,), 3, 3, 2, 1, 1, 71, 1, False, True): 2,
    ('x', 64, (8,), 3, 3, 2, 1, 1, 84, 1, False, True): 2,
    ('x', 64, (8,), 3, 3, 2, 1, 1, 93, 1, False, True): 2,
    ('x32+3', 512, (40,), 7, 7, 3, 3, 1, 47, 0, False, True): 30005,
    ('x32+3', 512, (40,), 7, 7, 3, 3, 1, 51, 0, False, True): 30004,
    ('x32+3', 512, (40,), 7, 7, 3, 3, 1, 54, 0, False, True): 30001,
    ('x32+3', 512, (40,), 7, 7, 3, 3, 1, 55, 0, False, True): 30001,
    ('x32+3', 512, (40,), 7, 7, 3, 3, 1, 63, 0, False, True): 30007,
    (128, (128, 128), 1, 1, 1, 0, 1, 32, 59, True, 0, False, True, 0): 2005,
    (128, (128, 128), 1, 1, 1, 0, 1, 32, 59, True, 0, False, True, 0, 'x3'): 30005,
    (128, (128, 128), 1, 1, 1, 0, 1, 32, 63, True, 0, False, True, 0): 2005,
    (128, (128, 128), 1, 1, 1, 0, 1, 32, 63, True, 0, False, True, 0, 'x3'): 30001,
    (128, (128, 128), 1, 1, 1, 0, 1, 32, 64, True, 0, False, True, 0): 2005,
    (128, (128, 128), 1, 1, 1, 0, 1, 32, 64, True, 0, False, True, 0, 'x3'): 30005,
    (128, (128, 128), 1, 1, 1, 0, 1, 32, 67, True, 0, False, True, 0): 2005,
    (128, (128, 128), 1, 1, 1, 0, 1, 32, 67, True, 0, False, True, 0, 'x3'): 30005,
    (128, (128, 128), 1, 1, 1, 0, 1, 32, 68, True, 0, False, True, 0): 2005,
    (128, (128, 128), 1, 1, 1, 0, 1, 32, 68, True, 0, False, True, 0, 'x3'): 30005,
    (128, (128, 128), 1, 1, 1, 0, 1, 32, 75, True, 0, False, True, 0): 2002,
    (128, (128, 128), 1, 1, 1, 0, 1, 32, 75, True, 0, False, True, 0, 'x3'): 30005,
    (128, (128, 128), 3, 3, 1, 1, 1, 32, 50, False, 2, True, False, 0, 'x3'): 40132,
    (128, (128, 128), 3, 3, 1, 1, 1, 32, 54, False, 2, True, False, 0, 'x3'): 40164,
    (128, (128, 128), 3, 3, 1, 1, 1, 32, 55, False, 2, True, False, 0, 'x3'): 46064,
    (128, (128, 128), 3, 3, 1, 1, 1, 32, 58, False, 0, True, False, 0, 'x3'): 46064,
    (128, (128, 128), 3, 3, 1, 1, 1, 32, 62, False, 2, True, False, 0, 'x3'): 46064,
    (128, (128, 128), 3, 3, 1, 1, 1, 32, 63, False, 0, True, False, 0, 'x3'): 46064,
    (128, (128, 128), 3, 3, 1, 1, 1, 32, 68, False, 0, True, False, 0, 'x3'): 46064,
    (128, (128, 128, 128), 3, 3, 1, 1, 1, 32, 50, False, 2, True, False, 0, 'x3'): 40132,
    (128, (128, 128, 128), 3, 3, 1, 1, 1, 32, 54, False, 2, True, False, 0, 'x3'): 40164,
    (128, (128, 128, 128), 3, 3, 1, 1, 1, 32, 55, False, 2, True, False, 0, 'x3'): 46064,
    (128, (128, 128, 128), 3, 3, 1, 1, 1, 32, 62, False, 2, True, False, 0, 'x3'): 46064,
    (128, (128, 128, 128, 4), 3, 3, 1, 1, 1, 32, 54, False, 2, True, False, 0, 'x3'): 40164,
    (128, (128, 128, 128, 4), 3, 3, 1, 1, 1, 32, 62, False, 2, True, False, 0, 'x3'): 46064,
    (128, (128, 128, 4), 3, 3, 1, 1, 1, 16, 50, True, 2, True, False, 0, 'x3'): 40132,
    (128, (128, 128, 4), 3, 3, 1, 1, 1, 16, 55, True, 2, True, False, 0, 'x3'): 46064,
    (128, (128,), 3, 3, 1, 1, 1, 32, 50, False, 2, True, False, 0, 'x3'): 40132,
    (128, (128,), 3, 3, 1, 1, 1, 32, 50, True, 0, True, False, 0, 'x3'): 40132,
    (128, (128,), 3, 3, 1, 1, 1, 32, 50, True, 2, True, False, 0, 'x3'): 40132,
    (128, (128,), 3, 3, 1, 1, 1, 32, 54, False, 2, True, False, 0, 'x3'): 40164,
    (128, (128,), 3, 3, 1, 1, 1, 32, 54, True, 0, True, False, 0, 'x3'): 45132,
    (128, (128,), 3, 3, 1, 1, 1, 32, 55, False, 2, True, False, 0, 'x3'): 46064,
    (128, (128,), 3, 3, 1, 1, 1, 32, 55, True, 0, True, False, 0, 'x3'): 46064,
    (128, (128,), 3, 3, 1, 1, 1, 32, 55, True, 2, True, False, 0, 'x3'): 46064,
    (128, (128,), 3, 3, 1, 1, 1, 32, 58, False, 0, True, False, 0, 'x3'): 46064,
    (128, (128,), 3, 3, 1, 1, 1, 32, 62, False, 2, True, False, 0, 'x3'): 46064,
    (128, (128,), 3, 3, 1, 1, 1, 32, 62, True, 0, True, False, 0, 'x3'): 46064,
    (128, (128,), 3, 3, 1, 1, 1, 32, 63, False, 0, True, False, 0, 'x3'): 46064,
    (128, (128,), 3, 3, 1, 1, 1, 32, 63, True, 0, True, False, 0, 'x3'): 45132,
    (128, (128,), 3, 3, 1, 1, 1, 32, 67, False, 2, True, False, 0, 'x3'): 46064,
    (128, (128,), 3, 3, 1, 1, 1, 32, 68, False, 0, True, False, 0, 'x3'): 46064,
    (128, (128,), 3, 3, 1, 1, 1, 32, 68, True, 0, True, False, 0, 'x3'): 46064,
    (128, (128,), 3, 3, 1, 1, 1, 32, 71, False, 2, True, False, 0, 'x3'): 46064,
    (128, (128,), 3, 3, 1, 1, 1, 32, 75, False, 2, True, False, 0, 'x3'): 46064,
    (128, (128,), 3, 3, 1, 1, 1, 32, 76, False, 2, True, False, 0, 'x3'): 46064,
    (128, (128,), 3, 3, 1, 1, 1, 32, 83, False, 2, True, False, 0, 'x3'): 46064,
    (128, (256, 256), 3, 3, 1, 1, 1, 32, 59, False, 2, True, False, 0, 'x3'): 45132,
    (128, (256, 256), 3, 3, 1, 1, 1, 32, 63, False, 2, True, False, 0, 'x3'): 46064,
    (128, (256, 256), 3, 3, 1, 1, 1, 32, 67, False, 2, True, False, 0, 'x3'): 46064,
    (128, (256, 256), 3, 3, 1, 1, 1, 32, 68, False, 2, True, False, 0, 'x3'): 46064,
    (128, (256, 256), 3, 3, 1, 1, 1, 32, 75, False, 2, True, False, 0, 'x3'): 46064,
    (128, (64,), 3, 3, 2, 1, 1, 32, 59, False, 2, False, False, 0, 'x3'): 30004,
    (128, (64,), 3, 3, 2, 1, 1, 32, 63, False, 2, False, False, 0, 'x3'): 30001,
    (128, (64,), 3, 3, 2, 1, 1, 32, 67, False, 2, False, False, 0, 'x3'): 30001,
    (128, (64,), 3, 3, 2, 1, 1, 32, 68, False, 2, False, False, 0, 'x3'): 30001,
    (128, (64,), 3, 3, 2, 1, 1, 32, 75, False, 2, False, False, 0, 'x3'): 30001,
    (1536, (512,), 1, 1, 1, 0, 1, 32, 47, False, 0, False, True, 0): 2004,
    (1536, (512,), 1, 1, 1, 0, 1, 32, 47, False, 0, False, True, 0, 'x3'): 30001,
    (1536, (512,), 1, 1, 1, 0, 1, 32, 51, False, 0, False, True, 0): 2005,
    (1536, (512,), 1, 1, 1, 0, 1, 32, 51, False, 0, False, True, 0, 'x3'): 30108,
    (1536, (512,), 1, 1, 1, 0, 1, 32, 54, False, 0, False, True, 0): 2004,
    (1536, (512,), 1, 1, 1, 0, 1, 32, 54, False, 0, False, True, 0, 'x3'): 30001,
    (1536, (512,), 1, 1, 1, 0, 1, 32, 55, False, 0, False, True, 0): 2004,
    (1536, (512,), 1, 1, 1, 0, 1, 32, 55, False, 0, False, True, 0, 'x3'): 30108,
    (1536, (512,), 1, 1, 1, 0, 1, 32, 56, False, 0, False, True, 0): 2005,
    (1536, (512,), 1, 1, 1, 0, 1, 32, 56, False, 0, False, True, 0, 'x3'): 30107,
    (1536, (512,), 1, 1, 1, 0, 1, 32, 63, False, 0, False, True, 0): 2004,
    (1536, (512,), 1, 1, 1, 0, 1, 32, 63, False, 0, False, True, 0, 'x3'): 30107,
    (16, (32,), 7, 7, 1, 3, 1, 32, 44, False, 1, False, False, 0, 'x3'): 0,
    (16, (32,), 7, 7, 1, 3, 1, 32, 45, False, 1, False, False, 0, 'x3'): 0,
    (16, (32,), 7, 7, 1, 3, 1, 32, 48, False, 1, False, False, 0, 'x3'): 0,
    (16, (32,), 7, 7, 1, 3, 1, 32, 49, False, 1, False, False, 0, 'x3'): 0,
    (16, (32,), 7, 7, 1, 3, 1, 32, 52, False, 1, False, False, 0, 'x3'): 0,
    (16, (32,), 7, 7, 1, 3, 1, 32, 53, False, 1, False, False, 0, 'x3'): 0,
    (16, (32,), 7, 7, 1, 3, 1, 32, 56, False, 1, False, False, 0, 'x3'): 0,
    (16, (32,), 7, 7, 1, 3, 1, 32, 57, False, 1, False, False, 0, 'x3'): 0,
    (16, (32,), 7, 7, 1, 3, 1, 32, 60, False, 1, False, False, 0, 'x3'): 0,
    (16, (32,), 7, 7, 1, 3, 1, 32, 61, False, 1, False, False, 0, 'x3'): 0,
    (16, (32,), 7, 7, 1, 3, 1, 32, 64, False, 1, False, False, 0, 'x3'): 0,
# ... 168 lines not shown
```

### include/e2fgvi_hip.h

```cpp
#ifndef E2FGVI_HIP_H
#define E2FGVI_HIP_H

#include <stdint.h>

#ifdef __cplusplus
extern "C" {
#endif

#define E2FGVI_EINVAL (-1)
#define E2FGVI_EUNSUP (-2)

#define E2FGVI_ACT_NONE 0
#define E2FGVI_ACT_RELU 1
#define E2FGVI_ACT_LRELU 2
#define E2FGVI_ACT_TANH 3
int e2fgvi_mask_prepare(const uint8_t* masks, int32_t L, int32_t Hin, int32_t Win, const int32_t* ytab, const int32_t* xtab,
                        uint8_t* out, int32_t H, int32_t W, int32_t iterations, void* stream);
int e2fgvi_masked_clip(const uint8_t* frames, const uint8_t* masks, const int32_t* ids, int32_t t, int32_t H, int32_t W,
                       float* clip, int32_t Hp, int32_t Wp, void* stream);
int e2fgvi_composite(const float* pred, const int32_t* ids, const uint8_t* first, int32_t n, const uint8_t* frames,
                     const uint8_t* masks, float* comp, int32_t H, int32_t W, int32_t Hp, int32_t Wp, void* stream);
int e2fgvi_resample_u8(const uint8_t* src, uint8_t* dst, int32_t L, int32_t H, int32_t W, int32_t n_out, int32_t axis,
                       const int32_t* bounds, const int32_t* coeffs, int32_t ksize, void* stream);
int e2fgvi_float_to_u8(const float* src, uint8_t* dst, int64_t n, void* stream);
// ... 168 lines not shown
    int32_t res_bcast;
    int32_t dst2_split_from;
    int64_t dst2_plane_stride;
} e2fgvi_convx_desc;

int e2fgvi_conv2d_bf16x(const e2fgvi_convx_desc* d, void* stream);
int64_t e2fgvi_packed_conv_weight_bf16x_size(int32_t Cout, int32_t groups, int32_t KH, int32_t KW, int32_t nsrc,
                                             const int32_t* src_cpg);
int e2fgvi_pack_conv_weight_bf16x(const float* w, void* wpacked, int32_t Cout, int32_t groups, int32_t KH, int32_t KW,
                                  int32_t nsrc, const int32_t* src_cpg, void* stream);

int64_t e2fgvi_packed_conv_weight_bf16x_taps_size(int32_t Cout, int32_t KH, int32_t KW, int32_t cin);
int e2fgvi_pack_conv_weight_bf16x_taps(const float* w, void* wpacked, int32_t Cout, int32_t KH, int32_t KW, int32_t cin,
                                       void* stream);
int e2fgvi_conv2d_f16x(const e2fgvi_convx_desc* d, void* stream);
int64_t e2fgvi_packed_conv_weight_f16x_size(int32_t Cout, int32_t groups, int32_t KH, int32_t KW, int32_t nsrc,
                                            const int32_t* src_cpg);
int e2fgvi_pack_conv_weight_f16x(const float* w, void* wpacked, int32_t Cout, int32_t groups, int32_t KH, int32_t KW,
                                 int32_t nsrc, const int32_t* src_cpg, void* stream);
int64_t e2fgvi_packed_conv_weight_f16x_taps_size(int32_t Cout, int32_t KH, int32_t KW, int32_t cin);
int e2fgvi_pack_conv_weight_f16x_taps(const float* w, void* wpacked, int32_t Cout, int32_t KH, int32_t KW, int32_t cin,
                                      void* stream);
int64_t e2fgvi_packed_conv_weight_f32x_taps_size(int32_t Cout, int32_t KH, int32_t KW, int32_t cin);
int e2fgvi_pack_conv_weight_f32x_taps(const float* w, float* wpacked, int32_t Cout, int32_t KH, int32_t KW, int32_t cin,
                                      void* stream);

int e2fgvi_conv2d_f32x(const e2fgvi_convx_desc* d, void* stream);
int64_t e2fgvi_packed_conv_weight_f32x_size(int32_t Cout, int32_t groups, int32_t KH, int32_t KW, int32_t nsrc,
                                            const int32_t* src_cpg);
int e2fgvi_pack_conv_weight_f32x(const float* w, float* wpacked, int32_t Cout, int32_t groups, int32_t KH, int32_t KW,
                                 int32_t nsrc, const int32_t* src_cpg, void* stream);

int e2fgvi_conv2d_f32x3(const e2fgvi_convx_desc* d, void* stream);
int64_t e2fgvi_packed_conv_weight_f32x3_size(int32_t Cout, int32_t groups, int32_t KH, int32_t KW, int32_t nsrc,
                                             const int32_t* src_cpg);
int e2fgvi_pack_conv_weight_f32x3(const float* w, void* wpacked, int32_t Cout, int32_t groups, int32_t KH, int32_t KW,
                                  int32_t nsrc, const int32_t* src_cpg, void* stream);
int e2fgvi_conv3x3_winograd_x3(const e2fgvi_conv_desc* d, void* stream);
int64_t e2fgvi_packed_winograd_weight_x3_size(int32_t Cout, int32_t groups, int32_t nsrc, const int32_t* src_cpg);
int e2fgvi_pack_winograd_weight_x3(const float* w, void* wpacked, int32_t Cout, int32_t groups, int32_t nsrc,
                                   const int32_t* src_cpg, void* stream);
int64_t e2fgvi_packed_conv_weight_f32x3_taps_size(int32_t Cout, int32_t KH, int32_t KW, int32_t cin);
int e2fgvi_pack_conv_weight_f32x3_taps(const float* w, void* wpacked, int32_t Cout, int32_t KH, int32_t KW, int32_t cin,
                                       void* stream);

int e2fgvi_split3_kv(const float* qkv_rows, void* planes, int64_t rows, void* stream);
int e2fgvi_focal_attention_x3(const float* qkv, const void* planes, const int32_t* key_tab, int32_t tab_ld, const int32_t* nkeys,
                              float* out, int32_t B, int32_t T, int32_t fh, int32_t fw, int32_t waves, void* stream);

int e2fgvi_focal_attention_bf16(const void* qkv, const void* kv_pool, const int32_t* key_tab, int32_t tab_ld,
                                const int32_t* nkeys, void* out, int32_t B, int32_t T, int32_t fh, int32_t fw,
                                void* stream);
int e2fgvi_focal_attention_bf16_variant(int variant);
int e2fgvi_focal_attention_f16(const void* qkv, const void* kv_pool, const int32_t* key_tab, int32_t tab_ld,
                               const int32_t* nkeys, void* out, int32_t B, int32_t T, int32_t fh, int32_t fw,
                               void* stream);

int e2fgvi_nchw_to_nhwc_x(const float* src, void* dst, int32_t dst_dtype, int32_t N, int32_t C, int32_t H, int32_t W,
                          int32_t ld, float scale, float shift, void* stream);
int e2fgvi_resize_bilinear_bf16(const void* src, int32_t src_ld, void* dst, int32_t dst_ld, int32_t N, int32_t C, int32_t H,
                                int32_t W, int32_t Ho, int32_t Wo, int32_t align_corners, void* stream);
int e2fgvi_resize_bilinear_f16(const void* src, int32_t src_ld, void* dst, int32_t dst_ld, int32_t N, int32_t C, int32_t H,
                               int32_t W, int32_t Ho, int32_t Wo, int32_t align_corners, void* stream);
int e2fgvi_prop_cond_x(const float* feat_prop, int32_t fp_ld, const float* feat_n2, int32_t f2_ld, const float* flow_a,
                       const float* flow_b, int64_t flow_img_stride, void* cond, int32_t cond_dtype, float* flows,
                       void* flows8_bf16, int32_t N, int32_t H, int32_t W, int32_t C, void* stream);
int e2fgvi_prop_cond_xs(const void* feat_prop, int32_t fp_ld, const void* feat_n2, int32_t f2_ld, int32_t src_dtype,
                        const float* flow_a, const float* flow_b, int64_t flow_img_stride, void* cond, int32_t cond_dtype,
                        float* flows, void* flows8_bf16, int32_t N, int32_t H, int32_t W, int32_t C, void* stream);
int e2fgvi_spynet_level_input_x(const float* pyr, const int32_t* ref_idx, const int32_t* supp_idx, const float* flow_prev,
                                float* out, void* out_bf16, int32_t Np, int32_t h, int32_t w, void* stream);
int e2fgvi_spynet_level_input_x_f16(const float* pyr, const int32_t* ref_idx, const int32_t* supp_idx, const float* flow_prev,
                                    float* out, void* out_f16, int32_t Np, int32_t h, int32_t w, void* stream);
int e2fgvi_layernorm_x(const float* x, const float* gamma, const float* beta, void* y, int32_t y_dtype, int64_t rows,
                       int32_t C, void* stream);
int e2fgvi_window_pool_x(const void* x, int32_t dtype, const float* w45, const float* bias1, void* pooled, int32_t BT,
                         int32_t fh, int32_t fw, int32_t C, void* stream);
int e2fgvi_ffn_fold_x(const void* hid, void* folded, int32_t dtype, int32_t F, int32_t fh, int32_t fw, int32_t H, int32_t W,
                      int32_t C, void* stream);
int e2fgvi_ffn_unfold_gelu_x(const void* folded, void* out, int32_t dtype, int32_t F, int32_t fh, int32_t fw, int32_t H,
                             int32_t W, int32_t C, void* stream);
int e2fgvi_ffn_fold_gelu_x(const void* hid, void* folded, int32_t dtype, int32_t F, int32_t fh, int32_t fw, int32_t H, int32_t W,
                           int32_t C, void* stream);
int e2fgvi_ffn_unfold_x(const void* folded, void* out, int32_t dtype, int32_t F, int32_t fh, int32_t fw, int32_t H, int32_t W,
                        int32_t C, void* stream);
int e2fgvi_softcomp_fold_bf16(const void* emb, const float* bias_hwc, const void* residual, void* dst, int32_t F, int32_t fh,
                              int32_t fw, int32_t H, int32_t W, int32_t C, void* stream);
int e2fgvi_softcomp_fold_f16(const void* emb, const float* bias_hwc, const void* residual, void* dst, int32_t F, int32_t fh,
                             int32_t fw, int32_t H, int32_t W, int32_t C, void* stream);
int e2fgvi_cast(const void* src, int32_t src_dtype, void* dst, int32_t dst_dtype, int64_t n, void* stream);

#ifdef __cplusplus
}
#endif
#endif
```

Baseline: 921.9 frames/s.

## Emit bf16x3 split planes from FFN fold and read them directly in fc2 conv

The FFN fold+GELU kernel can now write its fp32 output as three bf16 planes (hi/mid/lo), and a new conv tile (204) in the split-operand bf16x3 kernel loads A straight from those planes. The in-loop split of fp32 A tiles into three bf16 parts is skipped. The tile table switches the fc2 7x7 layer at this size to the new planes tile. This removes per-tile splitting arithmetic and LDS swizzle work, at the cost of 1.5x A-operand bytes and a third, plane-split layout for the fold output.

New measurement: 925.1 frames/s, median of 6. Within noise of the previous version (+0.3%).

```diff
diff --git a/e2fgvi_amd/build.py b/e2fgvi_amd/build.py
--- a/e2fgvi_amd/build.py
+++ b/e2fgvi_amd/build.py
@@ -61,6 +61,7 @@
             verify_wino_waits(objdir)
             verify_exit_reuse(objdir)
             verify_no_scratch(objdir)
+            verify_no_scratch(objdir, marker="ELb0ELi4ELb0EEE")
     return out
 
 
diff --git a/e2fgvi_amd/csrc/conv_bf16x.hip b/e2fgvi_amd/csrc/conv_bf16x.hip
--- a/e2fgvi_amd/csrc/conv_bf16x.hip
+++ b/e2fgvi_amd/csrc/conv_bf16x.hip
@@ -76,20 +76,24 @@
 template <int BM, int BN, int WGM, int WGN, bool S3, int MODE, bool PP = false>
 __global__ __launch_bounds__(64 * WGM * WGN) void conv_bf16x_kernel(const ConvXParams p) {
 #if defined(__HIP_DEVICE_COMPILE__)
-    constexpr bool F32 = MODE == 1, X3 = MODE == 2, F16 = MODE == 3;
+    constexpr bool F32 = MODE == 1, X3 = MODE == 2 || MODE == 4, F16 = MODE == 3;
+    constexpr bool APL = MODE == 4;
     typedef typename e2_h16<F16>::T E16;
     typedef typename e2_h16<F16>::V8 e16x8;
     static_assert(!PP || (X3 && !S3 && WGM * WGN == 8), "ping-pong halves: split-operand mode, 8 waves, no row-shift stages");
+    static_assert(!APL || (X3 && !S3 && !PP && BM % 64 == 0), "A from planes: split-operand mode, plain stages");
     constexpr int NT = 64 * WGM * WGN;
     constexpr int ESZ = (F32 || X3) ? 4 : 2;
+    constexpr int AESZ = APL ? 2 : ESZ;
     constexpr int CH = 16 / ESZ;
     constexpr int KC = 8 * CH;
     constexpr int TM = BM / (32 * WGM), TN = BN / (32 * WGN);
     constexpr int AR = S3 ? BM + 2 : BM;
     constexpr int B_CH = X3 ? 12 : 8;
-    constexpr int A_BYTES = AR * 128, B_BYTES = BN * B_CH * 16;
-    constexpr int A_IT = (AR * 8 + NT - 1) / NT, B_IT = (BN * B_CH + NT - 1) / NT;
-    constexpr bool A_PART = (AR * 8) % NT != 0;
+    constexpr int A_CH = APL ? 12 : 8;
+    constexpr int A_BYTES = AR * A_CH * 16, B_BYTES = BN * B_CH * 16;
+    constexpr int A_IT = (AR * A_CH + NT - 1) / NT, B_IT = (BN * B_CH + NT - 1) / NT;
+    constexpr bool A_PART = (AR * A_CH) % NT != 0;
     constexpr bool B_PART = (BN * B_CH) % NT != 0;
     constexpr int R = TM * 32, CN = TN * 32;
     constexpr int ES = (WGM * WGN * R * (CN + 4) * 4 <= 150 * 1024) ? 1 : (TN % 2 == 0 ? 2 : TN);
@@ -98,7 +102,7 @@
     static_assert(TN % ES == 0 && EPI <= 160 * 1024, "epilogue region");
     constexpr int SMEM = 2 * (A_BYTES + B_BYTES) > EPI ? 2 * (A_BYTES + B_BYTES) : EPI;
     constexpr unsigned OOB = 0xFFFFFFFFu;
-    static_assert(TM >= 1 && TN >= 1 && (BM * 8) % NT == 0 && (BN * B_CH) % 64 == 0 && SMEM <= 160 * 1024, "tile");
+    static_assert(TM >= 1 && TN >= 1 && (BM * A_CH) % NT == 0 && (BN * B_CH) % 64 == 0 && SMEM <= 160 * 1024, "tile");
 
     __shared__ __attribute__((aligned(1024))) unsigned char smem[SMEM];
 
@@ -117,8 +121,8 @@
 #pragma unroll
     for (int it = 0; it < A_IT; ++it) {
         const int item = tid + it * NT;
-        const int row = item >> 3, slot = item & 7;
-        a_ch16[it] = (unsigned)((slot ^ ((row >> 1) & 7)) * 16);
+        const int row = APL ? item % BM : item >> 3, slot = item & 7;
+        a_ch16[it] = APL ? (unsigned)(((item / BM) & 3) * 16) : (unsigned)((slot ^ ((row >> 1) & 7)) * 16);
         const int m = S3 ? m0 + row - 1 : m0 + row;
         const bool ok = m >= 0 && m < p.M;
         const int mm = ok ? m : 0;
@@ -145,9 +149,9 @@
 
     const void* const sp0 = p.src[0]; const void* const sp1 = p.src[1]; const void* const sp2 = p.src[2]; const void* const sp3 = p.src[3];
     const unsigned sb0 = p.src_bytes[0], sb1 = p.src_bytes[1], sb2 = p.src_bytes[2], sb3 = p.src_bytes[3];
-    const unsigned sl0 = (unsigned)p.ld[0] * ESZ, sl1 = (unsigned)p.ld[1] * ESZ, sl2 = (unsigned)p.ld[2] * ESZ, sl3 = (unsigned)p.ld[3] * ESZ;
-    const unsigned sc0 = (unsigned)(p.coff[0] + g * p.cpg[0]) * ESZ, sc1 = (unsigned)(p.coff[1] + g * p.cpg[1]) * ESZ,
-                   sc2 = (unsigned)(p.coff[2] + g * p.cpg[2]) * ESZ, sc3 = (unsigned)(p.coff[3] + g * p.cpg[3]) * ESZ;
+    const unsigned sl0 = (unsigned)p.ld[0] * AESZ, sl1 = (unsigned)p.ld[1] * AESZ, sl2 = (unsigned)p.ld[2] * AESZ, sl3 = (unsigned)p.ld[3] * AESZ;
+    const unsigned sc0 = (unsigned)(p.coff[0] + g * p.cpg[0]) * AESZ, sc1 = (unsigned)(p.coff[1] + g * p.cpg[1]) * AESZ,
+                   sc2 = (unsigned)(p.coff[2] + g * p.cpg[2]) * AESZ, sc3 = (unsigned)(p.coff[3] + g * p.cpg[3]) * AESZ;
     const int sg0 = p.cpg[0], sg1 = p.cpg[1], sg2 = p.cpg[2], sg3 = p.cpg[3];
     int ky = 0, kx = 0, s = 0, c0 = 0;
     int blk = 0;
@@ -174,22 +178,30 @@
     };
     retarget();
     unsigned char* const smem_b = smem + 2 * A_BYTES;
+    __amdgpu_buffer_rsrc_t a_rs[APL ? A_IT : 1];
+    if constexpr (APL) {
+#pragma unroll
+        for (int it = 0; it < A_IT; ++it) {
+            const int pl = __builtin_amdgcn_readfirstlane((tid + it * NT) / BM) >> 2;
+            a_rs[it] = make_rsrc(pl == 0 ? sp0 : pl == 1 ? sp1 : sp2, pl == 0 ? sb0 : pl == 1 ? sb1 : sb2);
+        }
+    }
     auto issue_a = [&](int stage) {
         if (p.dbg_noload & 16) return;
         unsigned char* sa = smem + stage * A_BYTES + wave * 1024;
         const __amdgpu_buffer_rsrc_t arsrc = make_rsrc(cur_src, cur_bytes);
-        const unsigned soff = (unsigned)c0 * (unsigned)ESZ;
+        const unsigned soff = (unsigned)c0 * (unsigned)AESZ;
         if (c0 + KC <= cur_cpg) {
 #pragma unroll
             for (int it = 0; it < A_IT; ++it)
-                if (!A_PART || it + 1 < A_IT || tid + it * NT < AR * 8)
-                    __builtin_amdgcn_raw_ptr_buffer_load_lds(arsrc, (lds_void*)(sa + it * NT * 16), 16, a_off[it], soff, 0, 0);
+                if (!A_PART || it + 1 < A_IT || tid + it * NT < AR * A_CH)
+                    __builtin_amdgcn_raw_ptr_buffer_load_lds(APL ? a_rs[it] : arsrc, (lds_void*)(sa + it * NT * 16), 16, a_off[it], soff, 0, 0);
         } else {
 #pragma unroll
             for (int it = 0; it < A_IT; ++it)
-                if (!A_PART || it + 1 < A_IT || tid + it * NT < AR * 8)
-                    __builtin_amdgcn_raw_ptr_buffer_load_lds(arsrc, (lds_void*)(sa + it * NT * 16), 16,
-                                                             (c0 + (int)(a_ch16[it] / ESZ) < cur_cpg) ? a_off[it] : OOB, soff, 0, 0);
+                if (!A_PART || it + 1 < A_IT || tid + it * NT < AR * A_CH)
+                    __builtin_amdgcn_raw_ptr_buffer_load_lds(APL ? a_rs[it] : arsrc, (lds_void*)(sa + it * NT * 16), 16,
+                                                             (c0 + (int)(a_ch16[it] / AESZ) < cur_cpg) ? a_off[it] : OOB, soff, 0, 0);
         }
     };
     auto issue_b = [&](int stage, int step) {
@@ -254,6 +266,11 @@
                 bf16x8 ah[TM], am[TM], al[TM];
 #pragma unroll
                 for (int tm = 0; tm < TM; ++tm)
+                    if constexpr (APL) {
+                        ah[tm] = *reinterpret_cast<const bf16x8*>(st + (q * BM + a_row[tm]) * 16);
+                        am[tm] = *reinterpret_cast<const bf16x8*>(st + ((4 + q) * BM + a_row[tm]) * 16);
+                        al[tm] = *reinterpret_cast<const bf16x8*>(st + ((8 + q) * BM + a_row[tm]) * 16);
+                    } else
                     split8(*reinterpret_cast<const f32x4*>(st + a_rd[tm] + (((2 * q) ^ a_key[tm]) << 4)),
                            *reinterpret_cast<const f32x4*>(st + a_rd[tm] + (((2 * q + 1) ^ a_key[tm]) << 4)), ah[tm], am[tm], al[tm]);
 #pragma unroll
@@ -420,13 +437,13 @@
                 unsigned char* sa = smem + stage * A_BYTES + wave * 1024;
 #pragma unroll
                 for (int it = 0; it < A_IT; ++it) {
-                    const int L = 8 * step + t_c[it];
+                    const int L = 8 * step + (APL ? 2 * t_c[it] : t_c[it]);
                     const int tap = cq == 1 ? L : (int)__umulhi((unsigned)L, p.tp_magic_cq);
                     const int cc = L - tap * cq;
                     const int tky = (int)__umulhi((unsigned)tap, p.tp_magic), tkx = tap - tky * p.KW;
                     const bool ok = tap < KK && ((a_msk[it] >> tky) & (a_msk[it] >> (8 + tkx)) & 1u) != 0;
-                    const unsigned off = ok ? (unsigned)(a_pix[it] + tky * p.W + tkx) * sl0 + sc0 + (unsigned)cc * 16u : OOB;
-                    __builtin_amdgcn_raw_ptr_buffer_load_lds(arsrc, (lds_void*)(sa + it * NT * 16), 16, off, 0, 0, 0);
+                    const unsigned off = ok ? (unsigned)(a_pix[it] + tky * p.W + tkx) * sl0 + sc0 + (unsigned)cc * (unsigned)(CH * AESZ) : OOB;
+                    __builtin_amdgcn_raw_ptr_buffer_load_lds(APL ? a_rs[it] : arsrc, (lds_void*)(sa + it * NT * 16), 16, off, 0, 0, 0);
                 }
             };
             issue_a_packed(0, 0);
@@ -797,10 +814,15 @@
     o[2 * plane] = (unsigned short)(__builtin_bit_cast(unsigned, r2) >> 16);
 }
 
-template <int BM, int BN, int WGM, int WGN, bool S3, bool PP = false>
+template <int BM, int BN, int WGM, int WGN, bool S3, bool PP = false, bool APL = false>
 int launch_x(ConvXParams& p, int groups, hipStream_t st, int mode = 0) {
     p.tilesM = cdiv(p.M, BM);
     p.tilesN = cdiv(p.Cout_g, BN);
+    if constexpr (APL) {
+        hipLaunchKernelGGL((conv_bf16x_kernel<BM, BN, WGM, WGN, false, 4>), dim3(p.tilesM * p.tilesN, groups, 1), dim3(64 * WGM * WGN), 0, st, p);
+        E2_LAUNCH_CHECK("conv2d_x");
+        return 0;
+    } else
     if constexpr (PP) {
         if (mode != 2 || p.tp_cq) {
             e2fgvi_set_error("conv2d_x: the ping-pong tiles (107, 108) are for the split-operand mode without tap-packed weights");
@@ -1031,7 +1053,22 @@
                                         : "conv2d_bf16x: dtype must be E2FGVI_F32 or E2FGVI_BF16");
     ConvXParams p;
     for (int s = 0; s < E2FGVI_MAX_SRC; ++s) { p.src[s] = nullptr; p.ld[s] = 0; p.coff[s] = 0; p.cpg[s] = 0; p.src_bytes[s] = 0; }
-    for (int s = 0; s < d->nsrc; ++s) {
+    const bool planes = d->tile > 200 && d->tile < 300;
+    if (planes) {
+        E2_REQUIRE(mode == 2, E2FGVI_EUNSUP, "conv2d_bf16x: the A-from-planes tiles (200 + tile) are for the split-operand mode");
+        E2_REQUIRE(d->nsrc == 1 && d->groups == 1 && d->src[1] && d->src[2] && d->src_ld[0] % 8 == 0 && d->src_coff[0] % 8 == 0 &&
+                       d->src_cpg[0] % 8 == 0, E2FGVI_EINVAL,
+                   "conv2d_f32x3: A from planes: one source as three bf16 planes src[0..2], no groups, ld / coff / channels in multiples of 8");
+        const long long bytes = (long long)d->N * d->H * d->W * d->src_ld[0] * 2;
+        E2_REQUIRE(bytes < 4294967295LL, E2FGVI_EUNSUP, "conv2d_f32x3: a plane spans >= 4 GiB (split the batch)");
+        E2_REQUIRE(d->src_coff[0] + d->src_cpg[0] <= d->src_ld[0], E2FGVI_EINVAL, "conv2d_f32x3: plane channel range exceeds its pixel stride");
+        for (int s = 0; s < 3; ++s) {
+            E2_REQUIRE(((uintptr_t)d->src[s] & 15) == 0, E2FGVI_EINVAL, "conv2d_f32x3: plane %d not 16-byte aligned", s);
+            p.src[s] = d->src[s]; p.ld[s] = d->src_ld[0]; p.coff[s] = d->src_coff[0]; p.cpg[s] = d->src_cpg[0];
+            p.src_bytes[s] = (unsigned)bytes;
+        }
+    }
+    for (int s = 0; s < (planes ? 0 : d->nsrc); ++s) {
         E2_REQUIRE(d->src[s], E2FGVI_EINVAL, "conv2d_bf16x: null source %d", s);
         E2_REQUIRE(d->src_ld[s] % q.ch == 0 && d->src_coff[s] % q.ch == 0 && ((uintptr_t)d->src[s] & 15) == 0, E2FGVI_EINVAL,
                    "conv2d_bf16x: source %d not 16-byte addressable (ld / coff multiples of 8 bf16 / 4 fp32)", s);
@@ -1119,6 +1156,7 @@
         case 8: return launch_x<256, 192, 4, 2, false>(p, d->groups, st, mode);
         case 107: return launch_x<256, 256, 4, 2, false, true>(p, d->groups, st, mode);
         case 108: return launch_x<256, 192, 4, 2, false, true>(p, d->groups, st, mode);
+        case 204: return launch_x<64, 128, 2, 2, false, false, true>(p, d->groups, st, mode);
         case 11: return launch_x<128, 128, 2, 2, true>(p, d->groups, st, mode);
         case 12: return launch_x<128, 64, 2, 2, true>(p, d->groups, st, mode);
         case 13: return launch_x<128, 32, 4, 1, true>(p, d->groups, st, mode);
diff --git a/e2fgvi_amd/csrc/misc.hip b/e2fgvi_amd/csrc/misc.hip
--- a/e2fgvi_amd/csrc/misc.hip
+++ b/e2fgvi_amd/csrc/misc.hip
@@ -448,10 +448,10 @@
 
 __device__ __forceinline__ float gelu_exact(float x) { return 0.5f * x * (1.f + erff(x * 0.70710678118654752f)); }
 
-template <bool NORMALISE, typename TE, typename TR, typename TD, bool GELU_OUT = false>
+template <bool NORMALISE, typename TE, typename TR, typename TD, bool GELU_OUT = false, bool PLANES = false>
 __global__ void fold_kernel(const TE* __restrict__ emb, const float* __restrict__ bias_hwc,
                             const TR* __restrict__ residual, TD* __restrict__ dst, int F, int fh, int fw, int H,
-                            int W, int C) {
+                            int W, int C, unsigned short* __restrict__ planes = nullptr, long long plane_stride = 0) {
     static_assert(VT<TE>::N == VT<TD>::N && VT<TR>::N == VT<TD>::N, "fold: one element class per instantiation");
     constexpr int NV = VT<TD>::N, Q = VT<TD>::Q;
     const int cq = C / NV;
@@ -503,6 +503,16 @@
 #pragma unroll
         for (int q = 0; q < Q; ++q) acc[q] = acc[q] + rq[q];
     }
+    if constexpr (PLANES) {
+        static_assert(NV == 4, "planes: fp32 folds");
+        unsigned hi[2], mid[2], lo[2];
+        e2_split2(acc[0][0], acc[0][1], hi[0], mid[0], lo[0]);
+        e2_split2(acc[0][2], acc[0][3], hi[1], mid[1], lo[1]);
+        typedef unsigned int u32x2 __attribute__((ext_vector_type(2)));
+        *reinterpret_cast<u32x2*>(planes + o) = u32x2{hi[0], hi[1]};
+        *reinterpret_cast<u32x2*>(planes + plane_stride + o) = u32x2{mid[0], mid[1]};
+        *reinterpret_cast<u32x2*>(planes + 2 * plane_stride + o) = u32x2{lo[0], lo[1]};
+    } else
     stv(dst + o, acc);
 }
 
@@ -857,6 +867,17 @@
     E2_LAUNCH_CHECK("ffn_fold_gelu");
     return 0;
 }
+extern "C" int e2fgvi_ffn_fold_gelu_x3(const float* hid, void* planes, int32_t F, int32_t fh, int32_t fw, int32_t H, int32_t W,
+                                       int32_t C, void* stream) {
+    E2_REQUIRE(hid && planes && ((uintptr_t)planes & 7) == 0, E2FGVI_EINVAL, "ffn_fold_gelu_x3: bad arguments");
+    if (int rc = check_fold("ffn_fold_gelu_x3", F, fh, fw, H, W, C)) return rc;
+    const long long total = (long long)F * H * W * (C / 4);
+    hipLaunchKernelGGL((fold_kernel<true, float, float, float, true, true>), dim3(blocks_for(total)), dim3(NTH), 0, (hipStream_t)stream,
+                       hid, (const float*)nullptr, (const float*)nullptr, (float*)nullptr, F, fh, fw, H, W, C,
+                       (unsigned short*)planes, (long long)F * H * W * C);
+    E2_LAUNCH_CHECK("ffn_fold_gelu_x3");
+    return 0;
+}
 extern "C" int e2fgvi_ffn_unfold_x(const void* folded, void* out, int32_t dtype, int32_t F, int32_t fh, int32_t fw, int32_t H,
                                    int32_t W, int32_t C, void* stream) {
     E2_REQUIRE(folded && out && E2_DT_OK(dtype), E2FGVI_EINVAL, "ffn_unfold: bad arguments");
diff --git a/e2fgvi_amd/engine.py b/e2fgvi_amd/engine.py
--- a/e2fgvi_amd/engine.py
+++ b/e2fgvi_amd/engine.py
@@ -167,6 +167,7 @@
         self.half = torch.full((4,), 0.5, device=self.device)
         self._tables = {}
         self._zeros = {}
+        self._fc2_planes = {}
         self.overlap_flows = True
         self._side = None
         self._given = None
@@ -218,6 +219,12 @@
             tab, nk = build_key_table(fh, fw, blk["valid"])
             self._tables[key] = (torch.from_numpy(tab).to(self.device), torch.from_numpy(nk).to(self.device))
         return self._tables[key]
+
+    def _fc2_reads_planes(self, fc2, n, H, W):
+        key = (n, H, W)
+        if key not in self._fc2_planes:
+            self._fc2_planes[key] = not self.x16 and fc2.wants_planes(n, H, W)
+        return self._fc2_planes[key]
 
     def flows(self, frames, l_t):
         b, t, c, H, W = frames.shape
@@ -394,7 +401,10 @@
         x1 = blk["proj"](att, out_dtype=torch.float32, residual=x)
         n2 = ops.layernorm(x1, blk["n2w"], blk["n2b"], out_dtype=self.dtype)
         hid = blk["fc1"](n2)
-        folded = ops.ffn_fold_gelu(hid, b * t, fh, fw, H, W, 40)
+        if isinstance(blk["fc2"], PackedConvX) and self._fc2_reads_planes(blk["fc2"], b * t, H, W):
+            folded = ops.ffn_fold_gelu_planes(hid, b * t, fh, fw, H, W, 40)
+        else:
+            folded = ops.ffn_fold_gelu(hid, b * t, fh, fw, H, W, 40)
         if isinstance(blk["fc2"], PackedConvX):
             y = torch.empty((rows, 512), dtype=torch.float32, device=x.device)
             blk["fc2"]([folded], out=y.view(b * t, fh, fw, 512), residual=x1.view(b * t, fh, fw, 512),
diff --git a/e2fgvi_amd/lib.py b/e2fgvi_amd/lib.py
--- a/e2fgvi_amd/lib.py
+++ b/e2fgvi_amd/lib.py
@@ -143,6 +143,7 @@
     "e2fgvi_ffn_fold_x": (C.c_int, [_fp, _fp, _i32, _i32, _i32, _i32, _i32, _i32, _i32, _fp]),
     "e2fgvi_ffn_unfold_gelu_x": (C.c_int, [_fp, _fp, _i32, _i32, _i32, _i32, _i32, _i32, _i32, _fp]),
     "e2fgvi_ffn_fold_gelu_x": (C.c_int, [_fp, _fp, _i32, _i32, _i32, _i32, _i32, _i32, _i32, _fp]),
+    "e2fgvi_ffn_fold_gelu_x3": (C.c_int, [_fp, _fp, _i32, _i32, _i32, _i32, _i32, _i32, _fp]),
     "e2fgvi_ffn_unfold_x": (C.c_int, [_fp, _fp, _i32, _i32, _i32, _i32, _i32, _i32, _i32, _fp]),
     "e2fgvi_softcomp_fold_bf16": (C.c_int, [_fp, _fp, _fp, _fp, _i32, _i32, _i32, _i32, _i32, _i32, _fp]),
     "e2fgvi_softcomp_fold_f16": (C.c_int, [_fp, _fp, _fp, _fp, _i32, _i32, _i32, _i32, _i32, _i32, _fp]),
diff --git a/e2fgvi_amd/ops.py b/e2fgvi_amd/ops.py
--- a/e2fgvi_amd/ops.py
+++ b/e2fgvi_amd/ops.py
@@ -35,11 +35,12 @@
 WINO_CANDIDATES = (64, 132, 164, 32)
 W4_CODES = {2464: (2, 64)}
 _W4_MINPIX = 20000
-XTUNE_CANDIDATES = (1, 4, 6, 7, 8, 2, 5, 3, 107, 108)
+XTUNE_CANDIDATES = (1, 4, 6, 7, 8, 2, 5, 3, 107, 108, 204)
 XTUNE_ROWSHIFT = (11, 16, 17, 12, 13, 18)
 X3_ENABLED = os.environ.get("E2FGVI_X3", "1") != "0"
 X3_MARGIN = 0.97
 X3_BASE = 30000
+APL_BASE = 200
 W3_BASE = 40000
 W3_CANDIDATES = (132, 164, 32, 5132, 6064)
 W3_WIDE = 6064
@@ -533,6 +534,10 @@
     raise TypeError("tensor must be float32, bfloat16 or float16, got %s" % t.dtype)
 
 
+def is_planes(t):
+    return isinstance(t, torch.Tensor) and t.dim() == 5 and t.shape[0] == 3 and t.dtype == torch.bfloat16
+
+
 def _dt_key(t):
     return _L.DT_BF16 if t.dtype == torch.float16 else _dt(t)
 
@@ -642,13 +647,24 @@
 
     def _desc(self, srcs, out, out_coff, residual, res_coff, act, slope, out2, out_nchw):
         d = _L.ConvXDesc()
-        N, H, W, _ = srcs[0][0].shape
+        if is_planes(srcs[0][0]):
+            t, coff = srcs[0]
+            if not self.x3 or len(srcs) != 1:
+                raise ValueError("%s: a source as bf16 planes is for one-source split-operand layers" % self.name)
+            _chk(t, "source planes", torch.bfloat16)
+            N, H, W = t.shape[1:4]
+            for i in range(3):
+                d.src[i] = t[i].data_ptr()
+            d.src_ld[0], d.src_coff[0], d.src_cpg[0] = t.shape[4], coff, self.cpg[0]
+            srcs = srcs[:1]
+        else:
+            N, H, W, _ = srcs[0][0].shape
+            for i, (t, coff) in enumerate(srcs):
+                _chk(t, "source %d" % i, self.dtype)
+                if t.dim() != 4 or tuple(t.shape[:3]) != (N, H, W):
+                    raise ValueError("source %d shape %s does not match [%d,%d,%d,*]" % (i, tuple(t.shape), N, H, W))
+                d.src[i], d.src_ld[i], d.src_coff[i], d.src_cpg[i] = t.data_ptr(), t.shape[3], coff, self.cpg[i]
         Ho, Wo = self.out_hw(H, W)
-        for i, (t, coff) in enumerate(srcs):
-            _chk(t, "source %d" % i, self.dtype)
-            if t.dim() != 4 or tuple(t.shape[:3]) != (N, H, W):
-                raise ValueError("source %d shape %s does not match [%d,%d,%d,*]" % (i, tuple(t.shape), N, H, W))
-            d.src[i], d.src_ld[i], d.src_coff[i], d.src_cpg[i] = t.data_ptr(), t.shape[3], coff, self.cpg[i]
         d.nsrc = len(srcs)
         d.N, d.H, d.W, d.Ho, d.Wo = N, H, W, Ho, Wo
         d.KH, d.KW, d.stride, d.pad = self.KH, self.KW, self.stride, self.pad
@@ -693,15 +709,24 @@
         srcs = [(s, 0) if isinstance(s, torch.Tensor) else s for s in sources]
         if len(srcs) != len(self.cpg):
             raise ValueError("expected %d sources, got %d" % (len(self.cpg), len(srcs)))
-        N, H, W, _ = srcs[0][0].shape
+        a_planes = is_planes(srcs[0][0])
+        N, H, W, _ = srcs[0][0].shape[1:] if a_planes else srcs[0][0].shape
         Ho, Wo = self.out_hw(H, W)
         dev = srcs[0][0].device
         if out is None:
             out = (torch.empty((N, self.Cout, Ho, Wo), dtype=torch.float32, device=dev) if out_nchw else
                    torch.empty((N, Ho, Wo, self.Cout), dtype=out_dtype, device=dev))
-        per_img = max(H * W * t.shape[3] * (4 if self.f32 else 2) for t, _ in srcs)
+        if a_planes and not self.x3:
+            best = self._decision(N, H, W, out, out_nchw)
+            if not (best and X3_BASE + APL_BASE < best < X3_BASE + APL_BASE + 100) or self._alt3() is None:
+                raise ValueError("%s: a source as bf16 planes needs an A-from-planes tile (table: %s)" % (self.name, best))
+            return self.alt3(srcs, out=out, out_dtype=out_dtype, out_coff=out_coff, residual=residual, res_coff=res_coff, act=act,
+                             slope=slope, out2=out2, tile=best - X3_BASE, out_nchw=out_nchw, planes=planes, split_from=split_from)
+        if not a_planes and self.x3 and APL_BASE < tile < APL_BASE + 100:
+            tile -= APL_BASE
+        per_img = max(H * W * t.shape[-1] * (4 if self.f32 else 2) for t, _ in srcs)
         if N > 1 and N * per_img >= (1 << 32) - 1:
-            if planes is not None:
+            if planes is not None or a_planes:
                 raise ValueError("split planes: the batch spans >= 4 GiB (call in chunks)")
             step = max(1, ((1 << 32) - 2) // per_img)
             for n0 in range(0, N, step):
@@ -716,8 +741,7 @@
         d.tile = tile
         x3 = self.try_x3 and X3_ENABLED and self.f32 and not self.x3
         if tile == 0 and self.tune and N * Ho * Wo >= 2048:
-            key = (("x3" if self.x3 else ("x32+3" if x3 else "x32")) if self.f32 else "x", self.Cout, tuple(self.cpg), self.KH, self.KW, self.stride, self.pad, self.groups,
-                   int(4.0 * math.log2(N * Ho * Wo)), _dt_key(out), out_nchw, self.taps)
+            key = self._key(N, H, W, out, out_nchw)
             best = _decision(key)
             if best is None and AUTOTUNE and not torch.cuda.is_current_stream_capturing() and (
                     residual is None or residual.data_ptr() != out.data_ptr()):
@@ -728,6 +752,8 @@
                     if res3 and (not res or min(res3.values()) < X3_MARGIN * min(res.values())):
                         best = X3_BASE + min(res3, key=res3.get)
                 best = _remember(key, best)
+            if best and X3_BASE + APL_BASE < best < X3_BASE + APL_BASE + 100:
+                best -= APL_BASE
             if best and best >= X3_BASE and self._alt3() is not None:
                 try:
                     return self.alt3(srcs, out=out, out_dtype=out_dtype, out_coff=out_coff, residual=residual, res_coff=res_coff, act=act,
@@ -754,6 +780,24 @@
             rc = self._fn(C.byref(d), _stream())
         _L.check(rc, "conv2d_x")
         return out
+
+    def _key(self, N, H, W, out, out_nchw):
+        Ho, Wo = self.out_hw(H, W)
+        x3 = self.try_x3 and X3_ENABLED and self.f32 and not self.x3
+        return ((("x3" if self.x3 else ("x32+3" if x3 else "x32")) if self.f32 else "x"), self.Cout, tuple(self.cpg), self.KH, self.KW,
+                self.stride, self.pad, self.groups, int(4.0 * math.log2(N * Ho * Wo)), _dt_key(out), out_nchw, self.taps)
+
+    def _decision(self, N, H, W, out, out_nchw=False):
+        Ho, Wo = self.out_hw(H, W)
+        if not (self.tune and N * Ho * Wo >= 2048):
+            return None
+        return _decision(self._key(N, H, W, out, out_nchw))
+
+    def wants_planes(self, N, H, W, out_dtype=torch.float32):
+        if not (self.f32 and not self.x3 and self.try_x3 and X3_ENABLED and len(self.cpg) == 1 and self.groups == 1):
+            return False
+        best = self._decision(N, H, W, torch.empty(0, dtype=out_dtype))
+        return bool(best) and X3_BASE + APL_BASE < best < X3_BASE + APL_BASE + 100
 
     def _time_tiles(self, d, reps=3, rounds=2):
         st = _stream()
@@ -1312,6 +1356,14 @@
     return out
 
 
+def ffn_fold_gelu_planes(hid, F_, fh, fw, H, W, Cc):
+    lib = _L.load()
+    _chk(hid, "hid")
+    out = torch.empty((3, F_, H, W, Cc), dtype=torch.bfloat16, device=hid.device)
+    _L.check(lib.e2fgvi_ffn_fold_gelu_x3(_ptr(hid), _ptr(out), F_, fh, fw, H, W, Cc, _stream()), "ffn_fold_gelu_x3")
+    return out
+
+
 def ffn_unfold(folded, fh, fw, out=None):
     lib = _L.load()
     _chk_any(folded, "folded")
diff --git a/e2fgvi_amd/tile_table.py b/e2fgvi_amd/tile_table.py
--- a/e2fgvi_amd/tile_table.py
+++ b/e2fgvi_amd/tile_table.py
@@ -148,7 +148,7 @@
     ('x', 64, (8,), 3, 3, 2, 1, 1, 84, 1, False, True): 2,
     ('x', 64, (8,), 3, 3, 2, 1, 1, 93, 1, False, True): 2,
     ('x32+3', 512, (40,), 7, 7, 3, 3, 1, 47, 0, False, True): 30005,
-    ('x32+3', 512, (40,), 7, 7, 3, 3, 1, 51, 0, False, True): 30004,
+    ('x32+3', 512, (40,), 7, 7, 3, 3, 1, 51, 0, False, True): 30204,
     ('x32+3', 512, (40,), 7, 7, 3, 3, 1, 54, 0, False, True): 30001,
     ('x32+3', 512, (40,), 7, 7, 3, 3, 1, 55, 0, False, True): 30001,
     ('x32+3', 512, (40,), 7, 7, 3, 3, 1, 63, 0, False, True): 30007,
diff --git a/include/e2fgvi_hip.h b/include/e2fgvi_hip.h
--- a/include/e2fgvi_hip.h
+++ b/include/e2fgvi_hip.h
@@ -274,6 +274,8 @@
                              int32_t W, int32_t C, void* stream);
 int e2fgvi_ffn_fold_gelu_x(const void* hid, void* folded, int32_t dtype, int32_t F, int32_t fh, int32_t fw, int32_t H, int32_t W,
                            int32_t C, void* stream);
+int e2fgvi_ffn_fold_gelu_x3(const float* hid, void* planes, int32_t F, int32_t fh, int32_t fw, int32_t H, int32_t W, int32_t C,
+                            void* stream);
 int e2fgvi_ffn_unfold_x(const void* folded, void* out, int32_t dtype, int32_t F, int32_t fh, int32_t fw, int32_t H, int32_t W,
                         int32_t C, void* stream);
 int e2fgvi_softcomp_fold_bf16(const void* emb, const float* bias_hwc, const void* residual, void* dst, int32_t F, int32_t fh,
```
